# IML-DKFZ/values

Measured on AMD Instinct MI355X. Metric: uncertainty-volumes/sec (64^3, T=10 MC-dropout), higher is better.
Workload: dtype f32; 1 GPU; C2: 64^3 1-channel volumes, UNet3D(initial_filter_size=8, 2 classes), T=10 MC-dropout passes + fused softmax/entropy/MI/variance/argmax reduction; dropout=hash bit generator, new seed every step, weights=torch default init, seed 123

## Files before the change

include/values_amd.h:

```cpp
#ifndef VALUES_AMD_H
#define VALUES_AMD_H

#include <stddef.h>
#include <stdint.h>

#ifdef __cplusplus
extern "C" {
#endif

typedef void* vx_stream_t;

enum {
  VX_OK = 0,
  VX_E_NULL = -1,
  VX_E_SHAPE = -2,
  VX_E_DTYPE = -3,
  VX_E_WORKSPACE = -4,
  VX_E_ALIGN = -5
};

enum { VX_F32 = 0, VX_F64 = 1 };
enum { VX_ACT_NONE = 0, VX_ACT_LRELU = 1 , VX_ACT_RELU = 2 };
enum { VX_DROP_NONE = 0, VX_DROP_HASH = 1, VX_DROP_MASK = 2 };

// ... 30 lines not shown
                  uint8_t* argmax, uint8_t* sample_argmax, vx_stream_t stream);

typedef struct vx_unc_outputs {
  float* mean_prob; float* pred_entropy; float* exp_entropy; float* mutual_info;
  float* variance;
  uint8_t* argmax; uint8_t* sample_argmax;
  const float* in_count; const float* out_count;
} vx_unc_outputs;
int vx_unc_reduce_ex(const void* x, int dtype, int from_logits, int B, int T, int C, int64_t nvox,
                     const vx_unc_outputs* outputs, vx_stream_t stream);

int vx_unc_stats_accumulate(const float* logits, int B, int T, int C, int64_t nvox, float* stats, vx_stream_t stream);
int vx_unc_stats_finalize(const float* stats, int B, int T_total, int C, int64_t nvox, float* mean_prob,
                          float* pred_entropy, float* exp_entropy, float* mutual_info, uint8_t* argmax,
                          vx_stream_t stream);

int vx_softmax_planar(const float* logits, int64_t R, int C, int64_t nvox, float* out, vx_stream_t stream);

int vx_one_minus_msr(const void* x, int dtype, int C, int64_t nvox, void* out, vx_stream_t stream);

#define VX_MSR_MAX_ITEMS 65536
#define VX_MSR_MAX_PLANES (1 << 22)
typedef struct vx_msr_item {
  void* out;
  int64_t n;
  int32_t first_plane;
  int32_t C;
  int32_t dtype;
  int32_t reserved;
} vx_msr_item;
int64_t vx_one_minus_msr_batched_workspace_bytes(int n_items, int n_planes);
int vx_one_minus_msr_batched(const vx_msr_item* items , int n_items,
                             const void* const* planes , int n_planes, void* workspace,
                             int64_t ws_bytes, vx_stream_t stream);

int64_t vx_conv3d_k3_packed_floats(int Cin, int Cout);
int vx_pack_conv3d_k3(const float* w_torch, float* w_packed, int Cin, int Cout, vx_stream_t stream);
int64_t vx_convT_k2s2_packed_floats(int Cin, int Cout);
int vx_pack_convT_k2s2(const float* w_torch, float* w_packed, int Cin, int Cout, vx_stream_t stream);

typedef struct vx_conv3d_args {
  const float* in;
  const float* w_packed;
  const float* bias;
  float* out;
  int32_t in_pitch, out_pitch, out_coff;
  int32_t N, D, H, W, Cin, Cout;
  int32_t act;
  int32_t drop_mode;
  uint32_t drop_seed, drop_layer;
  const uint8_t* drop_mask;
  float* stats_partial;
  int32_t in_xblk;
  int32_t w_family;
  float* head_out;
  const float* head_w;
  const float* head_b;
  const int32_t* head_dst;
  const int32_t* head_flip;
  int32_t head_C;
  const float* in_mean; const float* in_rstd;
  int32_t in_drop_mode; uint32_t in_drop_seed, in_drop_layer;
  int32_t in_repeat;
  int32_t out_xblk, out_half;
  uint32_t* range_flag;
  const uint32_t* seed_dev;
  const float* up_in;
  const float* up_w;
  const float* up_b;
  int32_t up_pitch;
  float* pool_out;
  uint32_t* pool_flags;
  int32_t in_split;
  int32_t out_f16, in_f16;
  int32_t out_split, up_split;
  const float* up_fused;
  const uint32_t* in_pool_flags;
  const float* acc_in;
  int32_t acc_pitch;
  int32_t out_planar, in_planar;
  int32_t products;
} vx_conv3d_args;
int64_t vx_conv3d_upfused_packed_floats(void);
int vx_pack_conv3d_upfused(const float* w1_torch, const float* b1, const float* up_w_torch, const float* up_b, float* packed,
                           vx_stream_t stream);
int vx_conv3d_k3_prologue_ok(int D, int H, int W, int Cin, int Cout);
int vx_conv3d_k3_upfuse_ok(int D, int H, int W, int Cin, int Cout);
int64_t vx_convT_zc16_packed_floats(void);
int64_t vx_conv3d_upfused_zc16_packed_floats(void);
int vx_pack_conv3d_upfused_zc16(const float* w1_torch, const float* up_w_torch, const float* up_b, float* packed, vx_stream_t stream);
int vx_pack_convT_zc16(const float* w_torch , float* packed, vx_stream_t stream);
int vx_conv3d_k3_skip_prologue_ok(int D, int H, int W, int Cin, int Cout, int xblk);
int vx_conv3d_k3_acc_ok(int D, int H, int W, int Cin, int Cout);
int vx_conv3d_k3_planar_ok(int D, int H, int W, int Cin, int Cout);
int vx_conv3d_k3_poolfuse_ok(int D, int H, int W, int Cin, int Cout);
int vx_conv3d_k3_presplit_ok(int D, int H, int W, int Cin, int Cout);
int vx_conv3d_k3_poolfin_ok(int Cin, int Cout);
int vx_prenorm_split(float* x, const float* mean, const float* rstd, int N, int64_t nvox, float scale, vx_stream_t stream);
int vx_pool_finish(const float* pool_raw, const uint32_t* pool_flags, const float* mean, const float* rstd, float* out,
                   int out_pitch, int N, int64_t voxels_per_sample, int drop_scale2, vx_stream_t stream);
int vx_pool_finish_z(const float* pool_raw, const uint32_t* pool_flags, const float* mean, const float* rstd, float* out,
                     int out_pitch, int N, int Dp, int64_t plane_voxels, int drop_scale2, vx_stream_t stream);
int vx_conv3d_k3_pool_layout(int D, int H, int W, int Cin, int Cout);
int vx_conv3d_k3_tiles(int D, int H, int W);
int vx_conv3d_k3_tiles_for(int D, int H, int W, int Cout);
int vx_conv3d_k3(const vx_conv3d_args* a, vx_stream_t stream);
int vx_conv3d_k3_head_fusable(int Cin, int Cout);
int vx_conv3d_k3_route(const vx_conv3d_args* a, char* kernel_name, int cap);

int vx_conv3d_k3_c1_tiles(int D, int H, int W);
int vx_conv3d_k3_c1(const float* in, const float* w_torch , const float* bias, float* out,
                    int out_pitch, int N, int D, int H, int W, int Cout, int repeat, const int32_t* src,
                    const int32_t* flip, float* stats_partial, vx_stream_t stream);

int vx_pack_input_cl8(const float* in, float* out, int N, int Cin, int D, int H, int W, int repeat, const int32_t* src,
                      const int32_t* flip, vx_stream_t stream);

int vx_instnorm_finalize(const float* stats_partial, int N, int ntiles, int C, int64_t nvox, float eps,
                         float* mean, float* rstd, vx_stream_t stream);

typedef struct vx_norm_args {
  const float* x; int32_t x_pitch;
  const float* mean; const float* rstd;
  float* out; int32_t out_pitch, out_coff;
  float* pool_out; int32_t pool_pitch;
  int32_t N, D, H, W, C;
  int32_t act, drop_mode; uint32_t drop_seed, drop_layer; const uint8_t* drop_mask;
  int32_t out_xblk, out_half;
  int32_t x_xblk, x_half;
  const uint32_t* seed_dev;
  uint32_t* range_flag;
} vx_norm_args;
int vx_norm_act_drop_pool(const vx_norm_args* a, vx_stream_t stream);
typedef struct vx_stat_src {
  const float* stats_partial; int32_t tiles; float eps; int64_t count;
  float* mean_out; float* rstd_out;
} vx_stat_src;
int vx_norm_act_drop_pool_stats(const vx_norm_args* a, const vx_stat_src* st, vx_stream_t stream);
int vx_prenorm_split_stats(float* x, const vx_stat_src* st, int N, int64_t nvox, float scale, vx_stream_t stream);
int vx_zero(void* p, int64_t bytes, vx_stream_t stream);
int vx_pool_finish_z_stats(const float* pool_raw, const uint32_t* pool_flags, const vx_stat_src* st, float* out, int out_pitch,
                           int N, int Dp, int64_t plane_voxels, int drop_scale2, vx_stream_t stream);
int vx_norm_act_drop_pool_bcast(const vx_norm_args* a, int x_repeat, vx_stream_t stream);

typedef struct vx_convT_args {
  const float* in; int32_t in_pitch;
  const float* w_packed; const float* bias;
  float* out; int32_t out_pitch, out_coff;
  int32_t N, D, H, W, Cin, Cout;
  int32_t act, drop_mode; uint32_t drop_seed, drop_layer; const uint8_t* drop_mask;
  int32_t out_xblk, out_half;
  uint32_t* range_flag;
  const uint32_t* seed_dev;
} vx_convT_args;
int vx_convT_k2s2(const vx_convT_args* a, vx_stream_t stream);

int vx_conv1x1_ncdhw(const float* in, int in_pitch, const float* w, const float* bias, float* out, int N, int D,
                     int H, int W, int F, int C, const int32_t* dst, const int32_t* flip, vx_stream_t stream);

typedef struct vx_unet3d_weights {
  const float* conv_w[18];
  const float* conv_b[18];
  const float* up_w[4];
  const float* up_b[4];
  const float* final_w;
  const float* final_b;
  int32_t F;
  int32_t num_classes;
  int32_t conv_family[18];
  int32_t in_channels;
  int32_t no_instancenorm;
  const float* up_fused;
  const float* split_w[2];
  int32_t split_family;
  const float* up3_zc16;
  const float* up3_fused;
} vx_unet3d_weights;

typedef struct vx_unet3d_run {
  const float* x;
  int32_t N, D, H, W;
  int32_t repeat;
  const int32_t* src;
  const int32_t* flip;
  const int32_t* dst;
  int32_t drop_mode;
  uint32_t seed;
  const uint8_t* masks[17];
  float* logits;
  void* workspace; size_t workspace_bytes;
  uint32_t* range_flag;
  const uint32_t* seed_dev;
} vx_unet3d_run;

size_t vx_unet3d_workspace_bytes(int N, int D, int H, int W, int F);
int vx_unet3d_forward(const vx_unet3d_weights* w, const vx_unet3d_run* r, vx_stream_t stream);
int vx_unet3d_forward_profiled(const vx_unet3d_weights* w, const vx_unet3d_run* r, vx_stream_t stream,
                               int max_launches, float* ms, const char** labels, int* n_launches);

typedef struct vx_conv2d_args {
  const float* in; int32_t in_pitch;
  const float* w_packed; const float* bias;
  float* out; int32_t out_pitch, out_coff;
  int32_t N, H, W, Cin, Cout, KS, S;
  float* stats_partial;
  int32_t w_family;
  const float* in_scale; const float* in_shift;
  int32_t in_cpitch, in_group_images, in_relu;
  const float* out_scale; const float* out_shift;
  const float* out_add; int32_t out_add_pitch;
  int32_t out_act;
} vx_conv2d_args;
int64_t vx_conv2d_packed_floats(int Cin, int Cout, int KS);
int vx_pack_conv2d(const float* w_torch , float* w_packed, int Cin, int Cout, int KS, vx_stream_t stream);
int vx_conv2d_tiles(int H, int W, int KS, int S);
int vx_conv2d(const vx_conv2d_args* a, vx_stream_t stream);
typedef struct vx_conv2d_route_info {
  int32_t nchunks;
  int32_t w_all;
  int32_t lds_bytes;
  int32_t grid_x, grid_y;
} vx_conv2d_route_info;
int vx_conv2d_route(const vx_conv2d_args* a, char* kernel_name, int cap, vx_conv2d_route_info* info);

int vx_bn_finalize(const float* stats_partial, int ntiles, int C, int64_t count, float eps, const float* gamma,
                   const float* beta, float* scale, float* shift, vx_stream_t stream);
int vx_bn_finalize_groups(const float* stats_partial, int ntiles_per_group, int G, int C, int cpitch, int64_t count_per_group,
                          float eps, const float* gamma, const float* beta, float* scale, float* shift, vx_stream_t stream);

typedef struct vx_bn_affine_item {
  const float* gamma; const float* beta; const float* running_mean; const float* running_var;
  float* scale; float* shift;
  int32_t C, cpitch;
} vx_bn_affine_item;
int vx_bn_running_affine(const vx_bn_affine_item* items, int n_items, float eps, vx_stream_t stream);

typedef struct vx_affine_args {
  const float* x; int32_t x_pitch;
  const float* scale; const float* shift;
  const float* add; int32_t add_pitch;
  float* out; int32_t out_pitch, out_coff;
  int32_t N, H, W, C, OH, OW;
  int32_t act;
  int32_t drop_mode; uint32_t drop_seed, drop_layer; const uint8_t* drop_mask;
  int32_t group_images;
} vx_affine_args;
int vx_affine_gather(const vx_affine_args* a, vx_stream_t stream);

typedef struct vx_fuse_term {
  const float* x; int32_t x_pitch, H, W;
  const float* scale; const float* shift;
} vx_fuse_term;
typedef struct vx_fuse_args {
  vx_fuse_term term[4]; int32_t nterms;
  float* out; int32_t out_pitch;
  int32_t N, OH, OW, C;
  int32_t act;
  int32_t group_images;
} vx_fuse_args;
int vx_fuse_sum(const vx_fuse_args* a, vx_stream_t stream);

int vx_bilinear_nchw(const float* x, int x_pitch, int N, int H, int W, int C, int OH, int OW, float* out,
                     const int32_t* dst, const int32_t* flip, vx_stream_t stream);
int vx_bilinear_softmax_nchw(const float* x, int x_pitch, int N, int H, int W, int C, int OH, int OW, float* out,
                             const int32_t* dst, const int32_t* flip, vx_stream_t stream);

int vx_softmax_accumulate(const float* logits, int B, int T, int C, int P0, int P1, int P2, const int32_t* crop,
                          float* sum, float* count, int X, int Y, int Z, int overlap, vx_stream_t stream);

int vx_aleatoric_sample(const float* mu_s, const float* eps, uint32_t seed, int N, int T, int C, int64_t nvox,
                        float* out, float* sigma, vx_stream_t stream);

int vx_softmax_variance(const float* x, int from_logits, int B, int T, int C, int64_t nvox, float* out, vx_stream_t stream);

int vx_ssn_sample(const float* head, const float* eps_w, const float* eps_d, uint32_t seed, int N, int S, int C, int R,
                  int64_t nvox, float epsilon, float* out, vx_stream_t stream);

int vx_tta_views_2d(const void* src, int src_u8, const float* noise0, const float* noise1, const float* mean, const float* std,
                    float max_pixel_value, int B, int H, int W, int G, const int32_t* view_code, float* out, vx_stream_t stream);

int vx_tta_views_2d_gen(const void* src, int src_u8, const float* noise0, const float* noise1, const float* mean,
                        const float* std, float max_pixel_value, int B, int H, int W, int G, const int32_t* view_code,
                        uint32_t seed, const uint32_t* seed_dev, int64_t image0, const float* var_limit, float* sigma_out,
                        float* out, vx_stream_t stream);

int vx_noise_view_3d(const float* x, float* out, int V, int64_t per, uint32_t seed, const uint32_t* seed_dev, int64_t index0,
                     float var_lo, float var_hi, int sigma_law, float* sigma_out, vx_stream_t stream);

int vx_colorize_u8(const uint8_t* labels, const uint8_t* ignore, int64_t n, const uint8_t* lut, int unlabeled, uint8_t* rgb,
                   vx_stream_t stream);

#define VX_SELECT_MAX_ITEMS 65536
enum { VX_COUNT_B1 = 0, VX_COUNT_B2 = 1, VX_COUNT_B4 = 2, VX_COUNT_B8 = 3, VX_COUNT_F32 = 4, VX_COUNT_F64 = 5 };
enum { VX_SELECT_OK = 0, VX_SELECT_NAN = 1 };
typedef struct vx_count_item {
  const void* ptr;
  int64_t n;
  int32_t kind;
  int32_t reserved;
} vx_count_item;
typedef struct vx_select_item {
  const void* ptr;
  int64_t n;
  int32_t dtype;
  int32_t reserved;
} vx_select_item;
int64_t vx_count_nonzero_batched_workspace_bytes(int n_items);
int vx_count_nonzero_batched(const vx_count_item* items , int n_items, uint64_t* counts ,
                             void* workspace, int64_t ws_bytes, vx_stream_t stream);
int64_t vx_select_segments_workspace_bytes(int n_items);
int vx_select_segments(const vx_select_item* items , int n_items, int64_t k, float* out ,
                       int32_t* status , void* workspace, int64_t ws_bytes, vx_stream_t stream);

enum { VX_PREP_U8 = 0, VX_PREP_I8 = 1, VX_PREP_U16 = 2, VX_PREP_I16 = 3, VX_PREP_U32 = 4, VX_PREP_I32 = 5, VX_PREP_F32 = 6, VX_PREP_F64 = 7 };
enum { VX_PREP_ZSCORE = 0, VX_PREP_COPY = 1 };
#define VX_PREP_OWN (-1)
typedef struct vx_prep_item {
  const void* ptr;
  int64_t n;
  int32_t kind;
  int32_t reserved;
} vx_prep_item;
typedef struct vx_prep_pad_item {
  const void* src;
  void* dst;
  int32_t dims[3];
  int32_t out_dims[3];
  int32_t pad_below[3];
  int32_t kind;
// ... 269 lines not shown
```

values_amd/_lib.py:

```python
from __future__ import annotations

import ctypes as C
import os

_HERE = os.path.dirname(os.path.abspath(__file__))
LIB_PATH = os.environ.get("VX_LIB_PATH") or os.path.join(_HERE, "libvalues_amd.so")

VX_F32, VX_F64 = 0, 1
VX_ACT_NONE, VX_ACT_LRELU, VX_ACT_RELU = 0, 1, 2
VX_DROP_NONE, VX_DROP_HASH, VX_DROP_MASK = 0, 1, 2

_p = C.c_void_p
_i = C.c_int
_i32 = C.c_int32
_u32 = C.c_uint32
_i64 = C.c_int64


class ConvArgs(C.Structure):
    _fields_ = [("in_", _p), ("w_packed", _p), ("bias", _p), ("out", _p),
                ("in_pitch", _i32), ("out_pitch", _i32), ("out_coff", _i32),
                ("N", _i32), ("D", _i32), ("H", _i32), ("W", _i32), ("Cin", _i32), ("Cout", _i32),
                ("act", _i32), ("drop_mode", _i32), ("drop_seed", _u32), ("drop_layer", _u32),
                ("drop_mask", _p), ("stats_partial", _p), ("in_xblk", _i32), ("w_family", _i32),
                ("head_out", _p), ("head_w", _p), ("head_b", _p), ("head_dst", _p), ("head_flip", _p),
                ("head_C", _i32),
                ("in_mean", _p), ("in_rstd", _p), ("in_drop_mode", _i32), ("in_drop_seed", _u32), ("in_drop_layer", _u32),
                ("in_repeat", _i32), ("out_xblk", _i32), ("out_half", _i32), ("range_flag", _p), ("seed_dev", _p),
                ("up_in", _p), ("up_w", _p), ("up_b", _p), ("up_pitch", _i32), ("pool_out", _p), ("pool_flags", _p),
                ("in_split", _i32), ("out_f16", _i32), ("in_f16", _i32),
                ("out_split", _i32), ("up_split", _i32), ("up_fused", _p), ("in_pool_flags", _p),
                ("acc_in", _p), ("acc_pitch", _i32), ("out_planar", _i32), ("in_planar", _i32), ("products", _i32)]


class NormArgs(C.Structure):
    _fields_ = [("x", _p), ("x_pitch", _i32), ("mean", _p), ("rstd", _p),
                ("out", _p), ("out_pitch", _i32), ("out_coff", _i32),
                ("pool_out", _p), ("pool_pitch", _i32),
                ("N", _i32), ("D", _i32), ("H", _i32), ("W", _i32), ("C", _i32),
                ("act", _i32), ("drop_mode", _i32), ("drop_seed", _u32), ("drop_layer", _u32), ("drop_mask", _p),
                ("out_xblk", _i32), ("out_half", _i32), ("x_xblk", _i32), ("x_half", _i32), ("seed_dev", _p),
                ("range_flag", _p)]


class StatSrc(C.Structure):
    _fields_ = [("stats_partial", _p), ("tiles", _i32), ("eps", C.c_float), ("count", _i64), ("mean_out", _p), ("rstd_out", _p)]


class ConvTArgs(C.Structure):
    _fields_ = [("in_", _p), ("in_pitch", _i32), ("w_packed", _p), ("bias", _p),
                ("out", _p), ("out_pitch", _i32), ("out_coff", _i32),
                ("N", _i32), ("D", _i32), ("H", _i32), ("W", _i32), ("Cin", _i32), ("Cout", _i32),
                ("act", _i32), ("drop_mode", _i32), ("drop_seed", _u32), ("drop_layer", _u32), ("drop_mask", _p),
                ("out_xblk", _i32), ("out_half", _i32), ("range_flag", _p), ("seed_dev", _p)]


class Conv2dArgs(C.Structure):
    _fields_ = [("in_", _p), ("in_pitch", _i32), ("w_packed", _p), ("bias", _p),
                ("out", _p), ("out_pitch", _i32), ("out_coff", _i32),
                ("N", _i32), ("H", _i32), ("W", _i32), ("Cin", _i32), ("Cout", _i32), ("KS", _i32), ("S", _i32),
                ("stats_partial", _p), ("w_family", _i32),
                ("in_scale", _p), ("in_shift", _p), ("in_cpitch", _i32), ("in_group_images", _i32), ("in_relu", _i32),
                ("out_scale", _p), ("out_shift", _p), ("out_add", _p), ("out_add_pitch", _i32), ("out_act", _i32)]


class Conv2dRouteInfo(C.Structure):
    _fields_ = [("nchunks", _i32), ("w_all", _i32), ("lds_bytes", _i32), ("grid_x", _i32), ("grid_y", _i32)]


class BnAffineItem(C.Structure):
    _fields_ = [("gamma", _p), ("beta", _p), ("running_mean", _p), ("running_var", _p), ("scale", _p), ("shift", _p),
                ("C", _i32), ("cpitch", _i32)]


class AffineArgs(C.Structure):
    _fields_ = [("x", _p), ("x_pitch", _i32), ("scale", _p), ("shift", _p), ("add", _p), ("add_pitch", _i32),
                ("out", _p), ("out_pitch", _i32), ("out_coff", _i32),
                ("N", _i32), ("H", _i32), ("W", _i32), ("C", _i32), ("OH", _i32), ("OW", _i32),
                ("act", _i32), ("drop_mode", _i32), ("drop_seed", _u32), ("drop_layer", _u32), ("drop_mask", _p),
                ("group_images", _i32)]


class FuseTerm(C.Structure):
    _fields_ = [("x", _p), ("x_pitch", _i32), ("H", _i32), ("W", _i32), ("scale", _p), ("shift", _p)]


class FuseArgs(C.Structure):
    _fields_ = [("term", FuseTerm * 4), ("nterms", _i32), ("out", _p), ("out_pitch", _i32),
                ("N", _i32), ("OH", _i32), ("OW", _i32), ("C", _i32), ("act", _i32), ("group_images", _i32)]


class Config(C.Structure):
    _fields_ = [(n, _i32) for n in (
        "conv_fp32", "s16_no_prenorm", "s16_no_xp8", "s16_skip_raw", "no_head_fusion", "s16_no_upfuse", "s16_no_poolfuse",
        "storage16", "s16_generic", "s16_no_zc16", "s16_no_halves", "s16_no_deep", "s16_no_l1dma", "c2s_no_wide", "c2s_no_oct")]
    RETIRED = ("s16_no_upcompose", "s16_no_upsplit", "s16_no_poolfin", "s16_no_presplit", "s16_no_dbplain")


def _retired_field(name):
    def put(self, v):
        if v:
            raise ValueError(f"vx_config.{name} was retired in 0.7.0: the default data flow is the only one")
    return property(lambda self: 0, put)


for _n in Config.RETIRED:
    setattr(Config, _n, _retired_field(_n))


class UncOutputs(C.Structure):
    _fields_ = [("mean_prob", _p), ("pred_entropy", _p), ("exp_entropy", _p), ("mutual_info", _p), ("variance", _p),
                ("argmax", _p), ("sample_argmax", _p), ("in_count", _p), ("out_count", _p)]


class UNet3DWeights(C.Structure):
    _fields_ = [("conv_w", _p * 18), ("conv_b", _p * 18), ("up_w", _p * 4), ("up_b", _p * 4),
                ("final_w", _p), ("final_b", _p), ("F", _i32), ("num_classes", _i32), ("conv_family", _i32 * 18),
                ("in_channels", _i32), ("no_instancenorm", _i32), ("up_fused", _p), ("split_w", _p * 2), ("split_family", _i32), ("up3_zc16", _p), ("up3_fused", _p)]


class UNet3DRun(C.Structure):
    _fields_ = [("x", _p), ("N", _i32), ("D", _i32), ("H", _i32), ("W", _i32), ("repeat", _i32),
                ("src", _p), ("flip", _p), ("dst", _p), ("drop_mode", _i32), ("seed", _u32),
                ("masks", _p * 17), ("logits", _p), ("workspace", _p), ("workspace_bytes", C.c_size_t),
                ("range_flag", _p), ("seed_dev", _p)]


VX_NIFTI_COPY, VX_NIFTI_PROB, VX_NIFTI_MEAN_PROB, VX_NIFTI_ARGMAX, VX_NIFTI_ARGMAX_MEAN = 0, 1, 2, 3, 4


class NiftiItem(C.Structure):
    _fields_ = [("src", _p), ("count", _p), ("dst_off", _i64), ("kind", _i32), ("src_dtype", _i32), ("esize", _i32),
                ("T", _i32), ("C", _i32), ("t", _i32), ("c", _i32), ("X", _i32), ("Y", _i32), ("Z", _i32),
                ("header", C.c_uint8 * 352)]


class GzItem(C.Structure):
    _fields_ = [("src", _p), ("n", _i64), ("dst_off", _i64), ("stride_hint", _i32 * 3), ("pad", _i32)]


class PngItem(C.Structure):
    _fields_ = [("labels", _p), ("ignore", _p), ("H", _i32), ("W", _i32)]


class PngRgbItem(C.Structure):
    _fields_ = [("rgb", _p), ("H", _i32), ("W", _i32)]


class InflateItem(C.Structure):
    _fields_ = [("src", _p), ("src_n", _i64), ("dst_off", _i64), ("dst_cap", _i64), ("format", _i32), ("pad", _i32)]


VX_INFLATE_GZIP, VX_INFLATE_ZLIB, VX_INFLATE_RAW = 0, 1, 2
INFLATE_STATUS = ("ok", "truncated", "bad header", "bad block type", "invalid code lengths", "bad symbol",
                  "distance beyond the output start", "output capacity reached", "checksum mismatch", "ISIZE mismatch",
                  "trailing bytes", "stored block length mismatch", "preset dictionary")
VX_INFLATE_CAPACITY = 7


class NiftiDecItem(C.Structure):
    _fields_ = [("src", _p), ("src_n", _i64), ("vox_offset", _i64), ("dst", _p), ("dst_n", _i64), ("ndim", _i32),
                ("dims", _i32 * 7), ("code", _i32), ("big_endian", _i32), ("out_dtype", _i32), ("pad", _i32),
                ("slope", C.c_double), ("inter", C.c_double)]


class PngUnfilterItem(C.Structure):
    _fields_ = [("src", _p), ("src_n", _i64), ("dst", _p), ("H", _i32), ("W", _i32), ("bpp", _i32), ("pad", _i32)]


VX_PNG_OK, VX_PNG_BAD_FILTER, VX_PNG_BAD_SIZE = 0, 1, 2
PNG_STATUS = ("ok", "filter byte above 4", "stream size is not H (1 + W bpp)")


class TiffLzwItem(C.Structure):
    _fields_ = [("src", _p), ("src_n", _i64), ("dst_off", _i64), ("dst_cap", _i64)]


class TiffUnpredictItem(C.Structure):
    _fields_ = [("src", _p), ("dst", _p), ("rows", _i32), ("W", _i32), ("predictor", _i32), ("pad", _i32)]


VX_LZW_OK, VX_LZW_TRUNCATED, VX_LZW_BAD_CODE = 0, 1, 2
LZW_STATUS = ("ok", "truncated", "bad code")
VX_LZW_NO_ROOM = 3


VX_AGG_IMAGE, VX_AGG_THRESHOLD, VX_AGG_PATCH = 0, 1, 2
VX_AGG_MAX_SPECS, VX_AGG_MAX_ITEMS = 8, 4096


class AggItem(C.Structure):
    _fields_ = [("map", _p), ("dtype", _i32), ("D", _i32), ("H", _i32), ("W", _i32)]


class AggSpec(C.Structure):
    _fields_ = [("kind", _i32), ("pd", _i32), ("ph", _i32), ("pw", _i32), ("thr", C.c_double)]


VX_EM_MAX_ITEMS = 4096


class EmItem(C.Structure):
    _fields_ = [("unc", _p), ("ref", _p), ("pred", _p), ("nvox", _i64), ("dtype", _i32), ("R", _i32)]


class NccItem(C.Structure):
    _fields_ = [("gt", _p), ("pred", _p), ("n_gt", _i64), ("n_pred", _i64), ("gt_dtype", _i32), ("pred_dtype", _i32),
                ("gt_R", _i32), ("reserved", _i32)]


VX_SELECT_MAX_ITEMS = 65536
VX_COUNT_B1, VX_COUNT_B2, VX_COUNT_B4, VX_COUNT_B8, VX_COUNT_F32, VX_COUNT_F64 = range(6)
VX_SELECT_OK, VX_SELECT_NAN = 0, 1


class CountItem(C.Structure):
    _fields_ = [("ptr", _p), ("n", _i64), ("kind", _i32), ("reserved", _i32)]


class SelectItem(C.Structure):
    _fields_ = [("ptr", _p), ("n", _i64), ("dtype", _i32), ("reserved", _i32)]


VX_PREP_U8, VX_PREP_I8, VX_PREP_U16, VX_PREP_I16, VX_PREP_U32, VX_PREP_I32, VX_PREP_F32, VX_PREP_F64 = range(8)
VX_PREP_ZSCORE, VX_PREP_COPY = 0, 1
VX_PREP_OWN = -1


class PrepItem(C.Structure):
    _fields_ = [("ptr", _p), ("n", _i64), ("kind", _i32), ("reserved", _i32)]


class PrepPadItem(C.Structure):
    _fields_ = [("src", _p), ("dst", _p), ("dims", _i32 * 3), ("out_dims", _i32 * 3), ("pad_below", _i32 * 3),
                ("kind", _i32), ("out_dtype", _i32), ("mode", _i32), ("stats_row", _i32), ("reserved", _i32)]


VX_P2D_IMAGE, VX_P2D_LABEL_IDS, VX_P2D_LABEL_COLOR = 0, 1, 2


class P2dItem(C.Structure):
    _fields_ = [("src", _p), ("palette", _p), ("H", _i32), ("W", _i32), ("bpp", _i32), ("y0", _i32), ("x0", _i32),
                ("crop_h", _i32), ("crop_w", _i32), ("factor", _i32), ("mode", _i32), ("reserved", _i32), ("out_rgb", _p),
                ("out_ids", _p)]


class P2dTables(C.Structure):
    _fields_ = [("id2trainid", _p), ("trainid2color", _p), ("color2trainid", _p), ("n_color", _i32), ("default_id", _i32)]


VX_MSR_MAX_ITEMS, VX_MSR_MAX_PLANES = 65536, 1 << 22


class MsrItem(C.Structure):
    _fields_ = [("out", _p), ("n", _i64), ("first_plane", _i32), ("C", _i32), ("dtype", _i32), ("reserved", _i32)]


SIGNATURES = {
    "vx_version": (_i, []),
    "vx_last_error_string": (C.c_char_p, []),
    "vx_last_kernel_name": (C.c_char_p, []),
    "vx_drop_hash_mask": (_i, [_u32, _u32, _i, _i64, _p, _p]),
    "vx_get_config": (_i, [C.POINTER(Config)]),
    "vx_set_config": (_i, [C.POINTER(Config)]),
    "vx_conv3d_k3_family": (_i, [_i, _i]),
    "vx_conv2d_family": (_i, [_i, _i, _i]),
    "vx_unc_reduce": (_i, [_p, _i, _i, _i, _i, _i, _i64, _p, _p, _p, _p, _p, _p, _p]),
    "vx_unc_reduce_ex": (_i, [_p, _i, _i, _i, _i, _i, _i64, C.POINTER(UncOutputs), _p]),
    "vx_unc_stats_accumulate": (_i, [_p, _i, _i, _i, _i64, _p, _p]),
    "vx_unc_stats_finalize": (_i, [_p, _i, _i, _i, _i64, _p, _p, _p, _p, _p, _p]),
    "vx_softmax_planar": (_i, [_p, _i64, _i, _i64, _p, _p]),
    "vx_one_minus_msr": (_i, [_p, _i, _i, _i64, _p, _p]),
    "vx_one_minus_msr_batched_workspace_bytes": (_i64, [_i, _i]),
    "vx_one_minus_msr_batched": (_i, [C.POINTER(MsrItem), _i, C.POINTER(_p), _i, _p, _i64, _p]),
    "vx_conv3d_k3_packed_floats": (_i64, [_i, _i]),
    "vx_pack_conv3d_k3": (_i, [_p, _p, _i, _i, _p]),
    "vx_convT_k2s2_packed_floats": (_i64, [_i, _i]),
    "vx_pack_convT_k2s2": (_i, [_p, _p, _i, _i, _p]),
    "vx_conv3d_k3_tiles": (_i, [_i, _i, _i]),
    "vx_conv3d_k3_tiles_for": (_i, [_i, _i, _i, _i]),
    "vx_conv3d_k3_head_fusable": (_i, [_i, _i]),
    "vx_conv3d_k3_route": (_i, [C.POINTER(ConvArgs), C.c_char_p, _i]),
    "vx_conv3d_k3_prologue_ok": (_i, [_i, _i, _i, _i, _i]),
    "vx_conv3d_k3_upfuse_ok": (_i, [_i, _i, _i, _i, _i]),
    "vx_conv3d_k3_poolfuse_ok": (_i, [_i, _i, _i, _i, _i]),
    "vx_conv3d_k3_presplit_ok": (_i, [_i, _i, _i, _i, _i]),
    "vx_conv3d_k3_poolfin_ok": (_i, [_i, _i]),
    "vx_conv3d_upfused_packed_floats": (_i64, []),
    "vx_pack_conv3d_upfused": (_i, [_p, _p, _p, _p, _p, _p]),
    "vx_pack_conv3d_upfused_zc16": (_i, [_p, _p, _p, _p, _p]),
    "vx_conv3d_upfused_zc16_packed_floats": (_i64, []),
    "vx_pool_finish": (_i, [_p, _p, _p, _p, _p, _i, _i, _i64, _i, _p]),
    "vx_pool_finish_z": (_i, [_p, _p, _p, _p, _p, _i, _i, _i, _i64, _i, _p]),
    "vx_conv3d_k3_pool_layout": (_i, [_i, _i, _i, _i, _i]),
    "vx_conv3d_k3_skip_prologue_ok": (_i, [_i, _i, _i, _i, _i, _i]),
    "vx_conv3d_k3_acc_ok": (_i, [_i, _i, _i, _i, _i]),
    "vx_conv3d_k3_planar_ok": (_i, [_i, _i, _i, _i, _i]),
    "vx_convT_zc16_packed_floats": (_i64, []),
    "vx_pack_convT_zc16": (_i, [_p, _p, _p]),
    "vx_prenorm_split": (_i, [_p, _p, _p, _i, _i64, C.c_float, _p]),
    "vx_zero": (_i, [_p, _i64, _p]),
    "vx_conv3d_k3": (_i, [C.POINTER(ConvArgs), _p]),
    "vx_conv3d_k3_c1_tiles": (_i, [_i, _i, _i]),
    "vx_conv3d_k3_c1": (_i, [_p, _p, _p, _p, _i, _i, _i, _i, _i, _i, _i, _p, _p, _p, _p]),
    "vx_pack_input_cl8": (_i, [_p, _p, _i, _i, _i, _i, _i, _i, _p, _p, _p]),
    "vx_instnorm_finalize": (_i, [_p, _i, _i, _i, _i64, C.c_float, _p, _p, _p]),
    "vx_norm_act_drop_pool": (_i, [C.POINTER(NormArgs), _p]),
    "vx_norm_act_drop_pool_bcast": (_i, [C.POINTER(NormArgs), _i, _p]),
    "vx_norm_act_drop_pool_stats": (_i, [C.POINTER(NormArgs), C.POINTER(StatSrc), _p]),
    "vx_prenorm_split_stats": (_i, [_p, C.POINTER(StatSrc), _i, _i64, C.c_float, _p]),
    "vx_pool_finish_z_stats": (_i, [_p, _p, C.POINTER(StatSrc), _p, _i, _i, _i, _i64, _i, _p]),
    "vx_convT_k2s2": (_i, [C.POINTER(ConvTArgs), _p]),
    "vx_conv1x1_ncdhw": (_i, [_p, _i, _p, _p, _p, _i, _i, _i, _i, _i, _i, _p, _p, _p]),
    "vx_unet3d_workspace_bytes": (C.c_size_t, [_i, _i, _i, _i, _i]),
    "vx_unet3d_forward": (_i, [C.POINTER(UNet3DWeights), C.POINTER(UNet3DRun), _p]),
    "vx_unet3d_forward_profiled": (_i, [C.POINTER(UNet3DWeights), C.POINTER(UNet3DRun), _p, _i, C.POINTER(C.c_float),
                                        C.POINTER(C.c_char_p), C.POINTER(_i)]),
    "vx_softmax_accumulate": (_i, [_p, _i, _i, _i, _i, _i, _i, _p, _p, _p, _i, _i, _i, _i, _p]),
    "vx_aleatoric_sample": (_i, [_p, _p, _u32, _i, _i, _i, _i64, _p, _p, _p]),
    "vx_colorize_u8": (_i, [_p, _p, _i64, _p, _i, _p, _p]),
    "vx_fuse_sum": (_i, [C.POINTER(FuseArgs), _p]),
    "vx_tta_views_2d": (_i, [_p, _i, _p, _p, C.POINTER(C.c_float), C.POINTER(C.c_float), C.c_float, _i, _i, _i, _i,
                             C.POINTER(C.c_int32), _p, _p]),
    "vx_tta_views_2d_gen": (_i, [_p, _i, _p, _p, C.POINTER(C.c_float), C.POINTER(C.c_float), C.c_float, _i, _i, _i, _i,
                                 C.POINTER(C.c_int32), _u32, _p, _i64, C.POINTER(C.c_float), _p, _p, _p]),
    "vx_noise_view_3d": (_i, [_p, _p, _i, _i64, _u32, _p, _i64, C.c_float, C.c_float, _i, _p, _p]),
    "vx_count_nonzero_batched_workspace_bytes": (_i64, [_i]),
    "vx_count_nonzero_batched": (_i, [C.POINTER(CountItem), _i, _p, _p, _i64, _p]),
    "vx_select_segments_workspace_bytes": (_i64, [_i]),
    "vx_select_segments": (_i, [C.POINTER(SelectItem), _i, _i64, _p, _p, _p, _i64, _p]),
    "vx_volume_stats_batched_workspace_bytes": (_i64, [C.POINTER(PrepItem), _i]),
    "vx_volume_stats_batched": (_i, [C.POINTER(PrepItem), _i, _p, _p, _i64, _p]),
    "vx_zscore_pad_batched_workspace_bytes": (_i64, [C.POINTER(PrepPadItem), _i]),
    "vx_zscore_pad_batched": (_i, [C.POINTER(PrepPadItem), _i, _p, _p, _i64, _p]),
    "vx_p2d_out_size": (_i, [_i, _i]),
    "vx_crop_resize_batched_workspace_bytes": (_i64, [C.POINTER(P2dItem), _i, C.POINTER(P2dTables)]),
    "vx_crop_resize_batched": (_i, [C.POINTER(P2dItem), _i, C.POINTER(P2dTables), _p, _p, _i64, _p]),
    "vx_toy_embed": (_i, [_p, C.POINTER(_i32), C.POINTER(_i32), C.c_double, _i, _i, _p, C.POINTER(_i32), _p]),
    "vx_gauss_blur_axis_f64": (_i, [_p, _p, C.POINTER(_i32), _i, _p, _i, _p]),
    "vx_count_ge_f64": (_i, [_p, _i64, C.c_double, _p, _p]),
    "vx_order_stats_f64_workspace_bytes": (_i64, [_i]),
    "vx_order_stats_f64_reads": (_i, [_i64, C.POINTER(_i64), _i]),
    "vx_order_stats_f64": (_i, [_p, _i64, C.POINTER(_i64), _i, _p, _p, _p, _i64, _p]),
    "vx_toy_segment": (_i, [_p, _i64, C.POINTER(C.c_double), _i, _p, _p]),
    "vx_toy_noise": (_i, [_p, _i64, _u32, _u32, C.c_double, _p]),
    "vx_voxelize_meshes": (_i, [_p, C.POINTER(_i64), _i, C.POINTER(C.c_double), C.c_double, C.POINTER(_i32), _p, _p, _p]),
    "vx_mask_agreement": (_i, [_p, _i, _i, _i64, _p, _p]),
    "vx_mask_agreement_batched": (_i, [_p, _i, _i, _i, _i64, _i, _p, _p]),
    "vx_soft_metric_workspace_bytes": (_i64, [_i, _i]),
    "vx_soft_metric_sums": (_i, [_p, _p, _i, _i, _i64, _p, _p, _p]),
    "vx_soft_metric_batched_workspace_bytes": (_i64, [_i, _i, _i, _i64]),
    "vx_soft_metric_sums_batched": (_i, [_p, _p, _i, _i, _i, _i64, _p, _p, _p]),
    "vx_ssn2d_lowres": (_i, [_p, _i, _p, _i, _p, _u32, _i, _i64, _i, _i, _i, _p, _p, _p]),
    "vx_ssn2d_add_diag": (_i, [_p, _p, _p, _u32, _i, _i, _i64, C.c_float, _p]),
    "vx_softmax_variance": (_i, [_p, _i, _i, _i, _i, _i64, _p, _p]),
    "vx_ssn_sample": (_i, [_p, _p, _p, _u32, _i, _i, _i, _i, _i64, C.c_float, _p, _p]),
    "vx_conv2d_packed_floats": (_i64, [_i, _i, _i]),
    "vx_pack_conv2d": (_i, [_p, _p, _i, _i, _i, _p]),
    "vx_conv2d_tiles": (_i, [_i, _i, _i, _i]),
    "vx_conv2d": (_i, [C.POINTER(Conv2dArgs), _p]),
    "vx_conv2d_route": (_i, [C.POINTER(Conv2dArgs), C.c_char_p, _i, C.POINTER(Conv2dRouteInfo)]),
    "vx_bn_finalize": (_i, [_p, _i, _i, _i64, C.c_float, _p, _p, _p, _p, _p]),
    "vx_bn_finalize_groups": (_i, [_p, _i, _i, _i, _i, _i64, C.c_float, _p, _p, _p, _p, _p]),
    "vx_bn_running_affine": (_i, [_p, _i, C.c_float, _p]),
    "vx_affine_gather": (_i, [C.POINTER(AffineArgs), _p]),
    "vx_bilinear_nchw": (_i, [_p, _i, _i, _i, _i, _i, _i, _i, _p, _p, _p, _p]),
    "vx_bilinear_softmax_nchw": (_i, [_p, _i, _i, _i, _i, _i, _i, _i, _p, _p, _p, _p]),
    "vx_ncc_batched_workspace_bytes": (C.c_size_t, [C.POINTER(NccItem), _i]),
    "vx_ncc_batched": (_i, [C.POINTER(NccItem), _i, _p, _p, C.c_size_t, _p]),
    "vx_rater_variance": (_i, [_p, _i, _i64, _p, _p]),
    "vx_platt_batched_workspace_bytes": (C.c_size_t, [C.POINTER(EmItem), _i]),
    "vx_platt_sums_batched": (_i, [C.POINTER(EmItem), _i, C.POINTER(C.c_double), _i, _p, _p, C.c_size_t, _p]),
    "vx_calib_batched_workspace_bytes": (C.c_size_t, [C.POINTER(EmItem), _i]),
    "vx_calib_bins_batched": (_i, [C.POINTER(EmItem), _i, C.POINTER(C.c_double), C.POINTER(C.c_double), _i, _p, _p,
                                   C.c_size_t, _p]),
    "vx_aggregate_workspace_bytes": (C.c_size_t, [C.POINTER(AggItem), _i, C.POINTER(AggSpec), _i]),
    "vx_aggregate_batched": (_i, [C.POINTER(AggItem), _i, C.POINTER(AggSpec), _i, _p, _p, C.c_size_t, _p]),
    "vx_nifti_workspace_bytes": (C.c_size_t, [_i]),
    "vx_nifti_payload_bytes": (_i64, [C.POINTER(NiftiItem)]),
    "vx_nifti_payload": (_i, [C.POINTER(NiftiItem), _i, _p, _i64, _p, C.c_size_t, _p]),
    "vx_gzip_bound": (_i64, [_i64]),
    "vx_gzip_workspace_bytes": (C.c_size_t, [C.POINTER(_i64), _i]),
    "vx_gzip_encode": (_i, [C.POINTER(GzItem), _i, _p, _i64, _p, _p, C.c_size_t, _p]),
    "vx_crc32": (_i, [_p, _i64, _p, _p]),
    "vx_png_bound": (_i64, [_i, _i]),
    "vx_png_workspace_bytes": (C.c_size_t, [C.POINTER(PngItem), _i]),
    "vx_png_encode": (_i, [C.POINTER(PngItem), _i, _p, _i, _p, _i64, _p, _p, _p, C.c_size_t, _p]),
    "vx_png_encode_rgb_workspace_bytes": (C.c_size_t, [C.POINTER(PngRgbItem), _i]),
    "vx_png_encode_rgb": (_i, [C.POINTER(PngRgbItem), _i, _p, _i64, _p, _p, _p, C.c_size_t, _p]),
    "vx_inflate_workspace_bytes": (_i64, [_i]),
    "vx_inflate": (_i, [C.POINTER(InflateItem), _i, _p, _i64, _p, _p, _p, _i64, _p]),
    "vx_nifti_decode_workspace_bytes": (_i64, [_i]),
    "vx_nifti_decode": (_i, [C.POINTER(NiftiDecItem), _i, _p, _i64, _p]),
    "vx_png_unfilter_workspace_bytes": (_i64, [_i]),
    "vx_png_unfilter": (_i, [C.POINTER(PngUnfilterItem), _i, _p, _p, _i64, _p]),
    "vx_rgb_to_trainid": (_i, [_p, _i64, _p, _i, _i, _p, _p]),
    "vx_tiff_lzw_workspace_bytes": (_i64, [_i]),
    "vx_tiff_lzw": (_i, [C.POINTER(TiffLzwItem), _i, _p, _i64, _p, _p, _p, _i64, _p]),
    "vx_tiff_unpredict_workspace_bytes": (_i64, [_i]),
    "vx_tiff_unpredict": (_i, [C.POINTER(TiffUnpredictItem), _i, _p, _p, _i64, _p]),
    "vx_tiff_predict_workspace_bytes": (_i64, [_i]),
    "vx_tiff_predict": (_i, [C.POINTER(TiffUnpredictItem), _i, _p, _p, _i64, _p]),
    "vx_tiff_lzw_bound": (_i64, [_i64]),
    "vx_tiff_lzw_encode_workspace_bytes": (_i64, [_i]),
    "vx_tiff_lzw_encode": (_i, [C.POINTER(TiffLzwItem), _i, _p, _i64, _p, _p, _p, _i64, _p]),
    "vx_tiff_lzw_pack_workspace_bytes": (_i64, [_i]),
    "vx_tiff_lzw_pack": (_i, [C.POINTER(TiffLzwItem), _i, _p, _i64, _p, _p, _i64, _p, _p, _i64, _p]),
}

_lib = None


class VxError(RuntimeError):
    pass


def load():
    global _lib
    if _lib is not None:
        return _lib
    if not os.path.exists(LIB_PATH):
        raise VxError(
            f"{LIB_PATH} is missing: build it with `python -c 'import __graft_entry__ as g; g.build()'` "
            "(or `make -C values_amd/csrc`). values_amd has no CPU fallback.")
    import torch
    lib = C.CDLL(LIB_PATH, mode=C.RTLD_GLOBAL)
    for name, (res, args) in SIGNATURES.items():
        if os.environ.get("VX_LIB_PATH") and not hasattr(lib, name):
            continue
        fn = getattr(lib, name)
        fn.restype = res
        fn.argtypes = args
    _lib = lib
    return lib


def get_config() -> "Config":
    c = Config()
    check(load().vx_get_config(C.byref(c)), "vx_get_config")
    return c


class config:

# ... 73 lines not shown
```

values_amd/csrc/conv3d_deep.hip:

```cpp
#include "s16_common.h"
#include "conv3d_internal.h"

struct DeepArgs {
  vx_conv3d_args a;
  const float* w;
  int tx, ty, tz, ts;
  int ltx, lty, ltz;
  int tiles_x, tiles_y, tiles_z;
  int npos;
  int nchunks, ncg;
  int npairs;
  unsigned m_cg, m_tx, m_ty, m_tz;
  int stat_epc;
  unsigned long long* stamps;
  int abl;
};

#define DP_STAMP VX_STAMP
#define DP_WAIT_LOADS VX_STAMP_WAIT_LOADS
#define DP_ABL VX_DIAG(ka.abl)

constexpr int DEEP_PREC_B = DEEP_NPOS * 16;
constexpr int DEEP_IMG_B = 2 * DEEP_PREC_B;

// ... 176 lines not shown
      }
#pragma unroll
      for (int it = 0; it < IN_IT; ++it) {
        if (!((ibad_always >> it) & 1u)) {
          f32x4 v = ibuf[it];
          if constexpr (PRE == 1) {
            uint32_t bits = 0xFu;
            if (hashed) bits = vx_drop_bits4(p_key, p_e0 + (voff[it] >> 2));
            if ((p_bad >> it) & 1u) bits = 0u;
#pragma unroll
            for (int j = 0; j < 4; ++j) {
              const int keep = __builtin_amdgcn_sbfe((int)bits, j, 1);
              const float scj = __int_as_float(__float_as_int(sc[j]) & keep);
              const float tt = vx_mul1(vx_sub1(v[j], p_mean[j]), scj);
              v[j] = vx_max1(tt, vx_mul1(tt, 0.01f));
            }
          }
          f16x4 hi, lo;
          vx_split4_s(v, hi, lo);
          if (!(DP_ABL & 16)) {
            *reinterpret_cast<f16x4*>(img + ldst[it]) = hi;
            *reinterpret_cast<f16x4*>(img + ldst[it] + DEEP_PREC_B) = lo;
          } else {
            asm volatile("" :: "v"(hi), "v"(lo));
          }
        }
      }
    };

    Cur cx = {0, 0}, cc = {0, 0}, cp = {0, 0};
    prefetch(cp); advance(cp);
    dma_w(cc, 0);
    commit(0);    advance(cc);
    asm volatile("s_waitcnt vmcnt(0)" ::: "memory");
    prefetch(cp); advance(cp);
    int j = 0;
    while (cx.ci < npair_wg) {
      __syncthreads();
      DP_STAMP(0);
      DP_WAIT_LOADS();
      DP_STAMP(3);
      dma_w(cc, (j + 1) & 1);
      if (cc.ci < npair_wg && !(DP_ABL & 4)) commit((j + 1) & 1);
      DP_STAMP(4);
      if (!(DP_ABL & 8)) prefetch(cp);
      if constexpr (IN_IT == 9) asm volatile("s_waitcnt vmcnt(9)" ::: "memory");
      else asm volatile("s_waitcnt vmcnt(7)" ::: "memory");
      DP_STAMP(5);
#ifdef VX_CONV_STAMPS
      ++st_iters;
#endif
      advance(cx); advance(cc); advance(cp);
      ++j;
    }
    if (STATS) __syncthreads();
  } else {
    int vbase[R];
    const int out_voxf = a.out_pitch;
    const size_t out_sample = (size_t)a.D * a.H * a.W * out_voxf;
    auto vox_of = [&](int v, int& cx_, int& ly, int& lz, int& smp) {
      cx_ = v & (TX - 1); v >>= ka.ltx;
      ly = v & (TY - 1); v >>= ka.lty;
      lz = v & (TZ - 1); smp = v >> ka.ltz;
    };
#pragma unroll
    for (int r = 0; r < R; ++r) {
      int cx_, ly, lz, smp;
      vox_of((wave * R + r) * 16 + m, cx_, ly, lz, smp);
      vbase[r] = (((smp * HZ + lz) * HY + ly) * HX + cx_) * 16;
    }
    int toff[NSTEP];
#pragma unroll
    for (int s = 0; s < NSTEP; ++s) {
      int tap = 4 * s + g;
      if (DP_ABL & 64) tap = 4 * s;
      if (tap > 26) tap = 26;
      toff[s] = (((tap / 9) * HY + (tap / 3) % 3) * HX + tap % 3) * 16;
    }
    const unsigned char* wlane = s_w + lane * 16;
    const bool f_lrelu = EPI == 3 ? a.act == VX_ACT_LRELU : EPI == 1;
    const bool f_relu = EPI == 3 && a.act == VX_ACT_RELU;
    const uint32_t seed_out = EPI == 1 ? vx_seed_of(a, a.drop_seed) : 0u;

    f32x4 acc[R][NT], accx[R][NT];

    auto multiply = [&](int buf) {
      const unsigned char* img = s_img + buf * DEEP_IMG_B;
      const unsigned char* wb = wlane + buf * DEEP_W_B;
      f16x8 wh[NT], wl[NT], bh[2][R], bl[R];
      int vb_[R];
#pragma unroll
      for (int r = 0; r < R; ++r) { vb_[r] = vbase[r]; asm volatile("" : "+v"(vb_[r])); }
      auto ldA = [&](int s, int nt) {
        wh[nt] = *reinterpret_cast<const f16x8*>(wb + ((s * NT + nt) * 2) * 1024);
        wl[nt] = *reinterpret_cast<const f16x8*>(wb + ((s * NT + nt) * 2 + 1) * 1024);
      };
      auto ldBh = [&](int s, int r) { bh[s & 1][r] = *reinterpret_cast<const f16x8*>(img + vb_[r] + toff[s]); };
      auto ldBl = [&](int s, int r) { bl[r] = *reinterpret_cast<const f16x8*>(img + vb_[r] + toff[s] + DEEP_PREC_B); };
#pragma unroll
      for (int nt = 0; nt < NT; ++nt) ldA(0, nt);
#pragma unroll
      for (int r = 0; r < R; ++r) { ldBh(0, r); ldBl(0, r); }
      __builtin_amdgcn_sched_group_barrier(0x100, 2 * NT + 2 * R, 0);
#pragma unroll
      for (int s = 0; s < NSTEP; ++s) {
        const bool more = s + 1 < NSTEP;
        const int set = s & 1;
#pragma unroll
        for (int nt = 0; nt < NT; ++nt) {
#pragma unroll
          for (int r = 0; r < R; ++r) {
            acc[r][nt] = __builtin_amdgcn_mfma_f32_16x16x32_f16(wh[nt], bh[set][r], acc[r][nt], 0, 0, 0);
            accx[r][nt] = __builtin_amdgcn_mfma_f32_16x16x32_f16(wh[nt], bl[r], accx[r][nt], 0, 0, 0);
            if (more && nt == 0) ldBh(s + 1, r);
            if (more && nt == NT - 1) ldBl(s + 1, r);
          }
#pragma unroll
          for (int r = 0; r < R; ++r) accx[r][nt] = __builtin_amdgcn_mfma_f32_16x16x32_f16(wl[nt], bh[set][r], accx[r][nt], 0, 0, 0);
          if (more) ldA(s + 1, nt);
        }
#ifndef DEEP_NO_PIPE
#pragma unroll
        for (int nt = 0; nt < NT; ++nt) {
#pragma unroll
          for (int r = 0; r < R; ++r) {
            __builtin_amdgcn_sched_group_barrier(0x008, 2, 0);
            if (more) __builtin_amdgcn_sched_group_barrier(0x100, 1, 0);
          }
          __builtin_amdgcn_sched_group_barrier(0x008, R, 0);
          if (more) __builtin_amdgcn_sched_group_barrier(0x100, 2, 0);
        }
#endif
      }
    };

    auto epilogue = [&](int ci) {
      float* red = s_red + (ci & 1) * (NW * 32 * 2);
      int n0, tzi, tyi, txi, cg;
      pair_of(ci, n0, tzi, tyi, txi, cg);
      const auto kp = kernarg();
      const unsigned vox0 = (unsigned)(((tzi * TZ) * a.H + tyi * TY) * a.W + txi * TX);
      const unsigned osoff = (vox0 * (unsigned)out_voxf + (unsigned)(cg * 32)) * 4u;
      const __amdgpu_buffer_rsrc_t osrd = __builtin_amdgcn_make_buffer_rsrc(
          (void*)(reinterpret_cast<char*>(kp->a.out) + (size_t)n0 * out_sample * 4), 0, VX_NUMREC, 0x00020000);
      float ssum[NT][4], ssq[NT][4];
      if (STATS) {
#pragma unroll
        for (int nt = 0; nt < NT; ++nt)
#pragma unroll
          for (int j = 0; j < 4; ++j) { ssum[nt][j] = 0.f; ssq[nt][j] = 0.f; }
      }
      int m_ = m;
      asm volatile("" : "+v"(m_));
#pragma unroll
      for (int r = 0; r < R; ++r) {
        int cx_, ly, lz, smp;
        vox_of((wave * R + r) * 16 + m_, cx_, ly, lz, smp);
        const int ovox = (lz * a.H + ly) * a.W + cx_;
        unsigned ovoff_r = ((unsigned)smp * (unsigned)out_sample + (unsigned)ovox * (unsigned)out_voxf + (unsigned)kp->a.out_coff + 4u * g) * 4u;
        if constexpr (R == 2) {
          if (n0 + smp >= a.N) ovoff_r = VX_OOB;
        }
        uint32_t hword = 0;
        if (EPI == 1) {
          const vx_dkey key = vx_drop_key(seed_out, kp->a.drop_layer, (uint32_t)(n0 + smp));
          hword = vx_drop_word(key, (vox0 + (unsigned)ovox) * (unsigned)ka.ncg + (unsigned)cg) >> (4 * g);
        }
#pragma unroll
        for (int nt = 0; nt < NT; ++nt) {
          f32x4 v;
#pragma unroll
          for (int j = 0; j < 4; ++j) v[j] = fmaf(accx[r][nt][j], 1.0f / 2048.f, acc[r][nt][j]);
          if (STATS) {
#pragma unroll
            for (int j = 0; j < 4; ++j) { ssum[nt][j] += v[j]; ssq[nt][j] = fmaf(v[j], v[j], ssq[nt][j]); }
          }
          if (f_lrelu) {
#pragma unroll
            for (int j = 0; j < 4; ++j) v[j] = fmaxf(v[j], 0.01f * v[j]);
          } else if (f_relu) {
#pragma unroll
            for (int j = 0; j < 4; ++j) v[j] = fmaxf(v[j], 0.f);
          }
          if (EPI == 1) {
            const uint32_t bits = hword >> (16 * nt);
#pragma unroll
            for (int j = 0; j < 4; ++j) v[j] *= __uint_as_float((bits << (30 - j)) & 0x40000000u);
          }
          if (!STATS) rmax = vx_max3abs(vx_max3abs(rmax, v[0], v[1]), v[2], v[3]);
          u32x4 sv = __builtin_bit_cast(u32x4, v);
          if (EPI == 1 || EPI == 3) {
            if (a.out_split) {
              typedef unsigned u32x2 __attribute__((ext_vector_type(2)));
              f16x4 hi, lo;
              vx_split4_s(v, hi, lo);
              const u32x2 h2 = __builtin_bit_cast(u32x2, hi), l2 = __builtin_bit_cast(u32x2, lo);
              sv = (u32x4){h2[0], h2[1], l2[0], l2[1]};
            }
          }
          __builtin_amdgcn_raw_buffer_store_b128(sv, osrd, (int)ovoff_r, (int)(osoff + (unsigned)(nt * 64)), 0);
          __builtin_amdgcn_sched_barrier(0);
          asm volatile("s_nop 3" ::: "memory");
          __builtin_amdgcn_sched_barrier(0);
        }
      }
      if (STATS) {
#pragma unroll
        for (int nt = 0; nt < NT; ++nt)
#pragma unroll
          for (int j = 0; j < 4; ++j) {
            float s = ssum[nt][j], qq = ssq[nt][j];
#pragma unroll
            for (int rot = 8; rot >= 1; rot >>= 1) { s += vx_row_ror(s, rot); qq += vx_row_ror(qq, rot); }
            if (m == 0) {
              red[(wave * 32 + nt * 16 + g * 4 + j) * 2 + 0] = s;
              red[(wave * 32 + nt * 16 + g * 4 + j) * 2 + 1] = qq;
            }
          }
      }
    };

    auto flush_tile = [&](int ci) {
      const float* red = s_red + (ci & 1) * (NW * 32 * 2);
      int n0, tzi, tyi, txi, cg;
      pair_of(ci, n0, tzi, tyi, txi, cg);
      const auto kp = kernarg();
      const int epc = kp->stat_epc;
      const int tps = ka.tiles_x * ka.tiles_y * ka.tiles_z;
      const int tile = (tzi * ka.tiles_y + tyi) * ka.tiles_x + txi;
      float* dst = kp->a.stats_partial + (((size_t)n0 * tps + tile) * epc * a.Cout + cg * 32) * 2;
      if (tid < 32) {
        float s = 0.f, qq = 0.f;
#pragma unroll
        for (int w = 0; w < NW; ++w) {
          s += red[(w * 32 + tid) * 2 + 0];
          qq += red[(w * 32 + tid) * 2 + 1];
        }
        dst[tid * 2 + 0] = s;
        dst[tid * 2 + 1] = qq;
      }
      for (int e = 1; e < epc; ++e)
        if (tid < 64) dst[(size_t)e * a.Cout * 2 + tid] = 0.f;
    };

    const bool late = wave >= NW / 2;
    Cur cx = {0, 0};
    int j = 0;
    int prev_ci = -1;
    int fl_ci = -1, fl_at = 0;
    while (cx.ci < npair_wg) {
      __syncthreads();
      DP_STAMP(0);
      if (STATS && fl_ci >= 0 && j >= fl_at && !late) { flush_tile(fl_ci); fl_ci = -1; }
      if (late && prev_ci >= 0) {
        if (!(DP_ABL & 2)) epilogue(prev_ci);
        prev_ci = -1;
      }
      DP_STAMP(2);
      if (cx.c == 0) {
        int n0, tzi, tyi, txi, cg;
        pair_of(cx.ci, n0, tzi, tyi, txi, cg);
        const f32x4 zero = {0.f, 0.f, 0.f, 0.f};
#pragma unroll
        for (int nt = 0; nt < NT; ++nt) {
          const f32x4 b4 = *reinterpret_cast<const f32x4*>(s_bias + cg * 32 + nt * 16 + 4 * g);
#pragma unroll
          for (int r = 0; r < R; ++r) { acc[r][nt] = b4; accx[r][nt] = zero; }
        }
      }
      if (!(DP_ABL & 1)) multiply(j & 1);
      DP_STAMP(1);
      if (cx.c == NCH - 1) {
        if (late) prev_ci = cx.ci;
        else if (!(DP_ABL & 2)) epilogue(cx.ci);
        if (STATS) { fl_ci = cx.ci; fl_at = j + 2; }
      }
      DP_STAMP(2);
#ifdef VX_CONV_STAMPS
      ++st_iters;
#endif
      advance(cx);
      ++j;
    }
    if (late && prev_ci >= 0) epilogue(prev_ci);
    if (STATS) {
      __syncthreads();
      if (fl_ci >= 0 && !late) flush_tile(fl_ci);
    }
  }
  if (!STATS && a.range_flag) {
    float mx = rmax;
#pragma unroll
    for (int off = 32; off >= 1; off >>= 1) mx = fmaxf(mx, __shfl_xor(mx, off, 64));
    if (lane == 0 && !(mx < 32768.f)) atomicMax(a.range_flag, __float_as_uint(mx));
  }
#ifdef VX_CONV_STAMPS
  if (ka.stamps && lane == 0) {
    unsigned long long* d = ka.stamps + ((size_t)blockIdx.x * 16 + wave) * 8;
    for (int i = 0; i < 6; ++i) d[i] = st_sum[i];
    d[6] = st_iters;
  }
#endif
}

__global__ void pack_conv3d_deep_kernel(const float* __restrict__ w, _Float16* __restrict__ out, int Cin, int64_t total) {
  const int nch = Cin / 8;
  for (int64_t i = (int64_t)blockIdx.x * blockDim.x + threadIdx.x; i < total; i += (int64_t)gridDim.x * blockDim.x) {
    const int j = (int)(i & 7), lane = (int)((i >> 3) & 63), hl = (int)((i >> 9) & 1), nt = (int)((i >> 10) & 1);
    const int64_t sb = i >> 11;
    const int step = (int)(sb % 7);
    const int64_t blk = sb / 7;
    const int chunk = (int)(blk % nch), cg = (int)(blk / nch);
    const int row = cg * 32 + nt * 16 + (lane & 15), tap = 4 * step + (lane >> 4);
    const float v = tap > 26 ? 0.f : w[((size_t)row * Cin + 8 * chunk + j) * 27 + tap];
    const float c = fminf(fmaxf(v, -65504.f), 65504.f);
    const _Float16 h = (_Float16)c;
    out[i] = hl == 0 ? h : (_Float16)((v - (float)h) * 2048.f);
  }
}

int vx_pack_conv3d_deep(const float* w_torch, float* w_packed, int Cin, int Cout, hipStream_t s) {
  const int64_t total = conv3d_deep_packed_floats(Cin, Cout) * 2;
  if (total <= 0) return VX_OK;
  int blocks = (int)((total + 255) / 256);
  if (blocks > 4096) blocks = 4096;
  hipLaunchKernelGGL(pack_conv3d_deep_kernel, dim3(blocks), dim3(256), 0, s, w_torch, reinterpret_cast<_Float16*>(w_packed), Cin, total);
  VX_CHECK_LAUNCH("vx_pack_conv3d_k3(deep)");
  return VX_OK;
// ... 44 lines not shown
```

values_amd/csrc/conv3d_k3.hip:

```cpp
#include <string.h>

#include "conv3d_internal.h"

extern "C" int vx_conv3d_k3_route(const vx_conv3d_args* ap, char* kernel_name, int cap) {
  if (!ap) VX_FAIL(VX_E_NULL, "vx_conv3d_k3: null args");
  Conv3dRoute r;
  const int rc = conv3d_route(*ap, vx_cfg(), &r);
  if (rc != VX_OK) VX_FAIL(rc, "%s", r.err);
  if (kernel_name && cap > 0) conv3d_route_name(r, kernel_name, cap);
  return VX_OK;
}

extern "C" int vx_conv3d_k3(const vx_conv3d_args* ap, vx_stream_t stream) {
  if (!ap) VX_FAIL(VX_E_NULL, "vx_conv3d_k3: null args");
  const vx_conv3d_args& a = *ap;
  Conv3dRoute r;
  const int rc = conv3d_route(a, vx_cfg(), &r);
  if (rc != VX_OK) VX_FAIL(rc, "%s", r.err);
  hipStream_t s = (hipStream_t)stream;
  switch (r.kernel) {
    case CONV3D_C8: return vx_conv3d_c8_launch(r, a, s);
    case CONV3D_XP8W: return vx_conv3d_xp8w_launch(r, a, s);
    case CONV3D_ZC16: return vx_conv3d_zc16_launch(r, a, a.w_packed + r.w_off, s);
    case CONV3D_DEEP: return vx_conv3d_deep_launch(r, a, a.w_packed + r.w_off, s);
    case CONV3D_S16: return vx_conv3d_s16_launch(r, a, s);
    default: return vx_conv3d_mfma_launch(r, a, s);
  }
}

extern "C" int vx_conv3d_k3_family(int Cin, int Cout) { return conv3d_family(Cin, Cout, vx_cfg()); }
extern "C" int64_t vx_conv3d_k3_packed_floats(int Cin, int Cout) { return conv3d_packed_floats(Cin, Cout, vx_cfg()); }

extern "C" int vx_pack_conv3d_k3(const float* w_torch, float* w_packed, int Cin, int Cout, vx_stream_t stream) {
  if (!w_torch || !w_packed) VX_FAIL(VX_E_NULL, "vx_pack_conv3d_k3: null pointer");
  const int64_t total = vx_conv3d_k3_packed_floats(Cin, Cout);
  if (total < 0) VX_FAIL(VX_E_SHAPE, "vx_pack_conv3d_k3: Cin=%d Cout=%d must be positive multiples of 8", Cin, Cout);
  const ConvCfg c = conv_config(Cin, Cout, vx_cfg());
  hipStream_t s = (hipStream_t)stream;
  if (c.C8) return vx_pack_conv3d_k3_c8(w_torch, w_packed, Cin, s);
  if (!c.S16) return vx_pack_conv3d_k3_mfma(w_torch, w_packed, Cin, Cout, total, s);
  const int rc = vx_pack_conv3d_k3_s16(w_torch, w_packed, Cin, Cout, s);
  if (rc != VX_OK) return rc;
  float* w_block = w_packed + conv3d_s16_packed_floats(Cin, Cout);
  if (conv3d_deep_packs(Cin, Cout)) return vx_pack_conv3d_deep(w_torch, w_block, Cin, Cout, s);
  return vx_pack_conv3d_zc16(w_torch, w_block, Cin, Cout, s);
}

extern "C" int vx_conv3d_k3_tiles(int D, int H, int W) { return conv3d_tiles_max(D, H, W); }
extern "C" int vx_conv3d_k3_tiles_for(int D, int H, int W, int Cout) { return conv3d_tiles_for(D, H, W, Cout, vx_cfg()); }
extern "C" int vx_conv3d_k3_head_fusable(int Cin, int Cout) { return conv3d_head_fusable(Cin, Cout, vx_cfg()); }
extern "C" int vx_conv3d_k3_prologue_ok(int D, int H, int W, int Cin, int Cout) { return conv3d_prologue_ok(D, H, W, Cin, Cout, vx_cfg()); }
extern "C" int vx_conv3d_k3_skip_prologue_ok(int D, int H, int W, int Cin, int Cout, int xblk) {
  return conv3d_skip_prologue_ok(D, H, W, Cin, Cout, xblk, vx_cfg());
}
extern "C" int vx_conv3d_k3_acc_ok(int D, int H, int W, int Cin, int Cout) { return conv3d_zc16_16to16(D, H, W, Cin, Cout, vx_cfg()) ? 1 : 0; }
extern "C" int vx_conv3d_k3_planar_ok(int D, int H, int W, int Cin, int Cout) { return conv3d_zc16_16to16(D, H, W, Cin, Cout, vx_cfg()) ? 1 : 0; }
extern "C" int vx_conv3d_k3_upfuse_ok(int D, int H, int W, int Cin, int Cout) { return conv3d_upfuse_ok(D, H, W, Cin, Cout, vx_cfg()); }
extern "C" int vx_conv3d_k3_pool_layout(int D, int H, int W, int Cin, int Cout) { return conv3d_pool_layout(D, H, W, Cin, Cout, vx_cfg()); }
extern "C" int vx_conv3d_k3_poolfuse_ok(int D, int H, int W, int Cin, int Cout) { return conv3d_pool_layout(D, H, W, Cin, Cout, vx_cfg()) != 0 ? 1 : 0; }
extern "C" int vx_conv3d_k3_presplit_ok(int D, int H, int W, int Cin, int Cout) { return conv3d_presplit_ok(D, H, W, Cin, Cout, vx_cfg()); }
extern "C" int vx_conv3d_k3_poolfin_ok(int Cin, int Cout) { return conv3d_poolfin_ok(Cin, Cout, vx_cfg()); }
```

values_amd/csrc/conv3d_route.h:

```cpp
#pragma once
#include <stdint.h>
#include <stdio.h>

#include "../../include/values_amd.h"

constexpr int DEEP_NPOS = 1080;
constexpr int DEEP_NPOS_R2 = 896;
constexpr int DEEP_W_B = 7 * 2 * 2 * 1024;
constexpr int DEEP_MAXC = 512;
constexpr int DEEP_MAXDIM = 32;
constexpr int S16_HEAD_MAXC = 4;

enum Conv3dKernel { CONV3D_MFMA = 0, CONV3D_C8, CONV3D_S16, CONV3D_XP8W, CONV3D_ZC16, CONV3D_DEEP, CONV3D_NKERNELS };

#define MFMA_TILES(X, CB, NT, XP) X(CB, NT, 16, 4, 4, 8, XP) X(CB, NT, 8, 8, 4, 8, XP) X(CB, NT, 4, 4, 4, 4, XP)
#define MFMA_INSTANCES(X) MFMA_TILES(X, 8, 1, 1) MFMA_TILES(X, 16, 1, 0) MFMA_TILES(X, 16, 2, 0) MFMA_TILES(X, 8, 1, 0) MFMA_TILES(X, 8, 2, 0)
#define C8_INSTANCES(X) X(1, 32, 4, 4) X(2, 32, 4, 4) X(1, 16, 8, 4) X(2, 16, 8, 4) X(1, 8, 4, 4) X(2, 8, 4, 4)
#define S16_SMALL(X, CB, NT, XP)                                                                                       \
  X(CB, NT, 16, 4, 4, 8, XP, 0, 0) X(CB, NT, 16, 4, 4, 8, XP, 0, 1) X(CB, NT, 16, 4, 4, 8, XP, 0, 3)                     \
  X(CB, NT, 8, 8, 4, 8, XP, 0, 0) X(CB, NT, 8, 8, 4, 8, XP, 0, 1) X(CB, NT, 8, 8, 4, 8, XP, 0, 3) X(CB, NT, 4, 4, 4, 4, XP, 0, 3)
#define S16_LARGE(X, CB, XP) X(CB, 1, 16, 8, 4, 8, XP, 0, 0) X(CB, 1, 16, 8, 4, 8, XP, 0, 1) X(CB, 1, 16, 8, 4, 8, XP, 0, 3)
#define S16_DB_PLAIN(X, CB, NT) X(CB, NT, 16, 4, 4, 8, 0, 2, 0) X(CB, NT, 16, 4, 4, 8, 0, 2, 1) X(CB, NT, 16, 4, 4, 8, 0, 2, 3)
#define S16_DB_XP(X)                                                                                                   \
  X(8, 1, 16, 8, 4, 8, 1, 2, 0) X(8, 1, 16, 8, 4, 8, 1, 2, 1) X(8, 1, 16, 8, 4, 8, 1, 2, 2) X(8, 1, 16, 8, 4, 8, 1, 2, 3) \
// ... 226 lines not shown
}
static inline bool conv3d_tile_prologue(int Cin, int Cout, const vx_config& cfg) {
  return conv_config(Cin, Cout, cfg).S16 && conv3d_s16_prologue_ok(Cin, Cout);
}
static inline bool conv3d_tile_xblk_prologue(int Cin, int Cout, int xblk) {
  const int csrc = Cin / 2;
  return s16_config(Cin, Cout).CB == 16 && csrc % 16 == 0 && conv3d_pow2((int64_t)xblk * csrc);
}
static inline int conv3d_prologue_ok(int D, int H, int W, int Cin, int Cout, const vx_config& cfg) {
  if (!conv3d_channels_ok(Cin, Cout)) return 0;
  return conv3d_xp8_applies(D, H, W, Cin, Cout, cfg) || conv3d_tile_prologue(Cin, Cout, cfg) ? 1 : 0;
}
static inline int conv3d_skip_prologue_ok(int D, int H, int W, int Cin, int Cout, int xblk, const vx_config& cfg) {
  if (Cin <= 0 || Cout <= 0 || Cin % 16 || Cout % 8 || (xblk != 1 && xblk != 2 && xblk != 4)) return 0;
  if (Cin == 16 && conv3d_xp8_applies(D, H, W, Cin, Cout, cfg)) return 1;
  return conv3d_tile_prologue(Cin, Cout, cfg) && conv3d_tile_xblk_prologue(Cin, Cout, xblk) ? 1 : 0;
}
static inline int conv3d_upfuse_ok(int D, int H, int W, int Cin, int Cout, const vx_config& cfg) {
  if (cfg.s16_no_upfuse) return 0;
  if (Cin == 16 && conv3d_xp8_applies(D, H, W, Cin, Cout, cfg)) return 1;
  return conv3d_zc16_16to16(D, H, W, Cin, Cout, cfg) ? 2 : 0;
}
static inline int conv3d_pool_layout(int D, int H, int W, int Cin, int Cout, const vx_config& cfg) {
  if (cfg.s16_no_poolfuse) return 0;
  if (Cin == 8 && conv3d_xp8_applies(D, H, W, Cin, Cout, cfg)) return 1;
  return conv3d_zc16_16to16(D, H, W, Cin, Cout, cfg) ? 2 : 0;
}
static inline int conv3d_presplit_ok(int D, int H, int W, int Cin, int Cout, const vx_config& cfg) {
  return Cin == 8 && conv3d_xp8_applies(D, H, W, Cin, Cout, cfg) ? 1 : 0;
}
static inline int conv3d_poolfin_ok(int Cin, int Cout, const vx_config& cfg) {
  if (Cin != 8 || Cout <= 0 || Cout % 8 || Cout % 32 == 0) return 0;
  return conv3d_tile_prologue(Cin, Cout, cfg) ? 1 : 0;
}

#define ROUTE_FAIL(code, ...)                          \
  do {                                                 \
    snprintf(r->err, sizeof(r->err), __VA_ARGS__);     \
    return (code);                                     \
  } while (0)
constexpr int ROUTE_DECLINED = 1;

static inline void route_instance(Conv3dRoute* r, int kernel, int np, int a = 0, int b = 0, int c = 0, int d = 0, int e = 0, int f = 0,
                                  int g = 0, int h = 0, int i = 0) {
  const int p[9] = {a, b, c, d, e, f, g, h, i};
  r->kernel = kernel; r->np = np;
  for (int k = 0; k < 9; ++k) r->p[k] = p[k];
}
static inline void route_tiles(Conv3dRoute* r, const vx_conv3d_args& a, int txv, int ty, int tz) {
  r->tiles_x = conv3d_tiles_along(a.W, txv); r->tiles_y = conv3d_tiles_along(a.H, ty); r->tiles_z = conv3d_tiles_along(a.D, tz);
  r->mx = conv3d_magic(r->tiles_x); r->my = conv3d_magic(r->tiles_y); r->mz = conv3d_magic(r->tiles_z);
}
static inline void route_columns(Conv3dRoute* r, const vx_conv3d_args& a, int tz, int stat_tiles) {
  r->tiles_x = a.W / 32; r->tiles_y = a.H / 8; r->tiles_z = 1; r->kz = a.D / tz;
  const int cps = r->tiles_x * r->tiles_y;
  r->nitems = (int)((int64_t)a.N * cps);
  r->mcps = conv3d_magic(cps); r->mx = conv3d_magic(r->tiles_x);
  r->stat_epc = stat_tiles / cps;
}

static inline int route_xp8w(const vx_conv3d_args& a, int stat_tiles, Conv3dRoute* r) {
  const int nch = a.Cin / 8;
  route_columns(r, a, 4 / nch, stat_tiles);
  const int cps = r->tiles_x * r->tiles_y;
  r->rep = (a.in_mean && a.in_repeat > 1 && a.N % a.in_repeat == 0) ? a.in_repeat : 1;
  r->mrep = conv3d_magic(r->rep);
  if ((int64_t)a.N * cps >= (1ll << 31)) ROUTE_FAIL(VX_E_SHAPE, "vx_conv3d_k3(xp8w): too many columns");
  if (a.stats_partial && (stat_tiles % cps || a.act != VX_ACT_NONE || (a.drop_mode != VX_DROP_NONE && !a.pool_out) || a.head_out))
    ROUTE_FAIL(VX_E_SHAPE, "vx_conv3d_k3(xp8w): statistics go with a plain epilogue");
  const int pre = a.in_split ? 2 : (a.in_mean ? 1 : 0);
  if (a.in_split && (a.Cin != 8 || a.in_xblk || a.in_pitch != 8 || a.up_in || !a.stats_partial))
    ROUTE_FAIL(VX_E_SHAPE, "vx_conv3d_k3(xp8w): a pre-split input (vx_prenorm_split) goes with a dense 8-channel tensor and the "
               "statistics epilogue (contr_1_2)");
  int epi;
  if (a.stats_partial) epi = a.pool_out ? 4 : 0;
  else if (a.head_out) epi = 2;
  else if (a.drop_mode == VX_DROP_HASH) epi = 1;
  else epi = 3;
  if (epi == 2 && a.act == VX_ACT_LRELU && a.drop_mode == VX_DROP_NONE) epi = 5;
  if (epi == 2 && !(a.act == VX_ACT_LRELU && a.drop_mode == VX_DROP_HASH)) return ROUTE_DECLINED;
  if (epi == 1 && a.act != VX_ACT_LRELU) return ROUTE_DECLINED;
  const int up = a.up_in ? (a.up_fused ? 2 : 1) : 0;
  if (a.pool_out && nch != 1) ROUTE_FAIL(VX_E_SHAPE, "vx_conv3d_k3(xp8w): the pooled output goes with Cin = 8");
  if (a.out_split) ROUTE_FAIL(VX_E_SHAPE, "vx_conv3d_k3(xp8w): out_split is an epilogue of the tile kernel");
  if (a.up_split && !up) ROUTE_FAIL(VX_E_SHAPE, "vx_conv3d_k3(xp8w): up_split without up_in");
  if (a.out_f16 && (epi != 1 || a.out_xblk || a.out_coff))
    ROUTE_FAIL(VX_E_SHAPE, "vx_conv3d_k3(xp8w): fp16 output goes with the LeakyReLU + dropout epilogue and a dense output tensor");
  if (a.in_f16 && !(nch == 1 && epi == 2 && pre == 0 && !up && !a.in_xblk))
    ROUTE_FAIL(VX_E_SHAPE, "vx_conv3d_k3(xp8w): fp16 input goes with the dense 8-channel layer that carries the fused head");
  const int in16 = (a.in_f16 ? 1 : 0) | (a.products == 1 ? 2 : 0);
  route_instance(r, CONV3D_XP8W, 6, nch, epi, pre, up, nch == 2 ? 8 : 4, in16);
  if (conv3d_instance_exists(CONV3D_XP8W, r->p, 6)) return VX_OK;
  if (a.products == 1 && !a.in_f16)
    ROUTE_FAIL(VX_E_SHAPE, "vx_conv3d_k3(xp8w): products = 1 exists for the MC-dropout forward's contr_1_2, upscale2 + expand_1_1 and "
               "expand_1_2 + head (nch %d, epilogue %d, prologue %d, up %d)", nch, epi, pre, up);
  if (up) ROUTE_FAIL(VX_E_SHAPE, "vx_conv3d_k3(xp8w): no fused up-convolution for this epilogue (act=%d, drop_mode=%d, statistics=%d)",
                     a.act, a.drop_mode, a.stats_partial ? 1 : 0);
  if (a.pool_out) ROUTE_FAIL(VX_E_SHAPE, "vx_conv3d_k3(xp8w): no pooled output for this epilogue");
  return ROUTE_DECLINED;
}

static inline int route_zc16(const vx_conv3d_args& a, int stat_tiles, Conv3dRoute* r) {
  if (a.in_xblk || a.head_out || a.in_split || a.in_f16 || a.out_f16 || (a.in_repeat > 1)) return ROUTE_DECLINED;
  if ((a.in_planar || a.out_planar) && (a.drop_mode == VX_DROP_MASK || !a.out || a.in_pitch != a.Cin || a.Cout != 16))
    ROUTE_FAIL(VX_E_SHAPE, "vx_conv3d_k3(zc16): the planar pre-split hand-over needs hash or no dropout and dense 16-channel tensors");
  if (a.up_in && (a.Cin != 16 || a.in_mean || a.stats_partial || a.up_pitch < 32 || a.up_pitch % 4 || (a.up_fused && (!a.acc_in || a.out_xblk || a.out_split))))
    ROUTE_FAIL(VX_E_SHAPE, "vx_conv3d_k3(zc16): the fused up-convolution (32 coarse channels -> the conv's 16 input channels) goes with an "
               "activation epilogue, no prologue, up_pitch >= 32 (got %d), up_w packed by vx_pack_convT_zc16; composed weights "
               "(up_fused: vx_pack_conv3d_upfused_zc16) only together with partial sums (acc_in) and a dense float or planar output", a.up_pitch);
  if (a.drop_mode == VX_DROP_MASK || !a.out) return ROUTE_DECLINED;
  route_columns(r, a, 2, stat_tiles);
  const int cps = r->tiles_x * r->tiles_y;
  if ((int64_t)a.N * cps >= (1ll << 31)) ROUTE_FAIL(VX_E_SHAPE, "vx_conv3d_k3(zc16): too many columns");
  if (a.in_pitch != a.Cin) return ROUTE_DECLINED;
  if (a.stats_partial && (stat_tiles % cps || a.act != VX_ACT_NONE || (a.drop_mode != VX_DROP_NONE && !a.pool_out)))
    ROUTE_FAIL(VX_E_SHAPE, "vx_conv3d_k3(zc16): statistics go with a plain epilogue");
  if (a.pool_out && (!a.stats_partial || a.Cin != 16)) ROUTE_FAIL(VX_E_SHAPE, "vx_conv3d_k3(zc16): the pooled output goes with statistics, 16 -> 16");
  int pre = 0;
  if (a.in_pool_flags) pre = 3;
  else if (a.in_mean) pre = 1;
  if ((pre == 1 && a.Cin != 16) || (pre == 3 && a.Cin != 8)) return ROUTE_DECLINED;
  if (a.in_planar) {
    if (a.Cin != 16 || pre != 0 || a.up_in || a.acc_in || a.stats_partial || !conv3d_aligned16(a.in) ||
        (conv3d_bytes)a.D * a.H * a.W * 64 >= CONV3D_2GIB)
      ROUTE_FAIL(VX_E_SHAPE, "vx_conv3d_k3(zc16): a planar pre-split input (in_planar) goes with 16 -> 16, an activation epilogue, no "
                 "prologue / up-convolution / partial sums, a 16-byte aligned tensor, one sample below 2 GiB");
    pre = 4;
  }
  if (a.out_planar && (a.stats_partial || a.out_pitch != 16 || a.out_coff != 0 || a.out_xblk || a.out_split || a.out == a.acc_in ||
                       (conv3d_bytes)a.D * a.H * a.W * 64 >= CONV3D_2GIB))
    ROUTE_FAIL(VX_E_SHAPE, "vx_conv3d_k3(zc16): a planar pre-split output (out_planar) goes with an activation epilogue into a dense "
               "16-channel tensor that is not the partial sums' (another layout), one sample below 2 GiB");
  int epi;
  if (a.stats_partial) epi = a.pool_out ? 4 : 0;
  else if (a.drop_mode == VX_DROP_HASH) { if (a.act != VX_ACT_LRELU) return ROUTE_DECLINED; epi = 1; }
  else epi = 3;
  if (a.out_split && a.stats_partial) ROUTE_FAIL(VX_E_SHAPE, "vx_conv3d_k3(zc16): out_split goes with the activation epilogues");
  if (a.out_planar) {
    if (a.Cin != 16 || pre != 0 || (epi != 1 && epi != 3) || ((a.acc_in != nullptr) != (a.up_in != nullptr)))
      ROUTE_FAIL(VX_E_SHAPE, "vx_conv3d_k3(zc16): out_planar goes with 16 -> 16, an activation epilogue, no prologue, and either partial "
                 "sums + the fused up-convolution together or neither");
    epi = epi == 1 ? 5 : 6;
  }
  if (a.acc_in && (a.Cin != 16 || pre != 0 || a.stats_partial || a.acc_pitch < 16 || a.acc_pitch % 4 || !conv3d_aligned16(a.acc_in) ||
                   (conv3d_bytes)a.D * a.H * a.W * a.acc_pitch * 4 >= CONV3D_2GIB))
    ROUTE_FAIL(VX_E_SHAPE, "vx_conv3d_k3(zc16): partial sums (acc_in) go with 16 -> 16, no prologue, an activation epilogue, a "
               "16-byte aligned tensor of pitch >= 16 (pitch %d), one sample below 2 GiB", a.acc_pitch);
  route_instance(r, CONV3D_ZC16, 5, a.Cin, epi, pre, a.acc_in ? 1 : 0, a.up_in ? 1 : 0);
  if (conv3d_instance_exists(CONV3D_ZC16, r->p, 5)) return VX_OK;
  if (a.up_in && !a.acc_in) ROUTE_FAIL(VX_E_SHAPE, "vx_conv3d_k3(zc16): no fused up-convolution for this epilogue");
  return ROUTE_DECLINED;
}

static inline int route_deep(const vx_conv3d_args& a, int stat_tiles, Conv3dRoute* r) {
  if (a.head_out || a.in_split || a.in_f16 || a.out_f16 || (a.in_repeat > 1) || a.out_xblk || a.up_in || a.pool_out ||
      a.in_pool_flags || a.acc_in)
    return ROUTE_DECLINED;
  if (a.drop_mode == VX_DROP_MASK || !a.out) return ROUTE_DECLINED;
  DeepGeo g;
  const int R = deep_pick(a.D, a.H, a.W, &g);
  if (!R) return ROUTE_DECLINED;
  if (a.in_xblk) {
    const int csrc = a.Cin / 2;
    if (a.in_mean || csrc % 8 || a.W % a.in_xblk) return ROUTE_DECLINED;
  } else if (a.in_pitch % 4) {
    return ROUTE_DECLINED;
  }
  if (a.in_mean && (a.in_pitch != a.Cin || g.ts != 1)) return ROUTE_DECLINED;
  if (a.stats_partial && g.ts != 1) return ROUTE_DECLINED;
  r->tx = g.tx; r->ty = g.ty; r->tz = g.tz; r->ts = g.ts; r->npos = g.npos;
  r->tiles_x = g.tiles_x; r->tiles_y = g.tiles_y; r->tiles_z = g.tiles_z;
  r->nchunks = a.Cin / 8;
  r->ncg = a.Cout / 32;
  const int tps = g.tiles_x * g.tiles_y * g.tiles_z;
  const int64_t npairs = (((int64_t)a.N + g.ts - 1) / g.ts) * tps * r->ncg;
  if (npairs >= (1ll << 31)) ROUTE_FAIL(VX_E_SHAPE, "vx_conv3d_k3(deep): too many tiles");
  r->nitems = (int)npairs;
  r->m_cg = conv3d_magic(r->ncg); r->mx = conv3d_magic(g.tiles_x); r->my = conv3d_magic(g.tiles_y); r->mz = conv3d_magic(g.tiles_z);
  r->stat_epc = 0;
  if (a.stats_partial) {
    if (stat_tiles % tps) return ROUTE_DECLINED;
    if (a.act != VX_ACT_NONE || a.drop_mode != VX_DROP_NONE) ROUTE_FAIL(VX_E_SHAPE, "vx_conv3d_k3(deep): statistics go with a plain epilogue");
    r->stat_epc = stat_tiles / tps;
  }
  if ((conv3d_bytes)g.ts * a.D * a.H * a.W * a.out_pitch * 4 >= CONV3D_2GIB)
    ROUTE_FAIL(VX_E_SHAPE, "vx_conv3d_k3(deep): one tile's samples must stay below 2 GiB");
  int epi;
  if (a.stats_partial) epi = 0;
  else if (a.drop_mode == VX_DROP_HASH) { if (a.act != VX_ACT_LRELU) return ROUTE_DECLINED; epi = 1; }
  else epi = 3;
  if (a.out_split && a.stats_partial) ROUTE_FAIL(VX_E_SHAPE, "vx_conv3d_k3(deep): out_split goes with the activation epilogues");
  route_instance(r, CONV3D_DEEP, 3, R, epi, a.in_mean ? 1 : 0);
  return conv3d_instance_exists(CONV3D_DEEP, r->p, 3) ? VX_OK : ROUTE_DECLINED;
}

static inline int route_s16(const vx_conv3d_args& a, const vx_config& cfg, Conv3dRoute* r) {
  const S16Cfg c = s16_config(a.Cin, a.Cout);
  int txv, ty, tz;
  vx_conv3d_s16_tile(a.H, a.W, a.Cout, &txv, &ty, &tz);
  const int tx = c.XP ? txv / 2 : txv;
  route_tiles(r, a, txv, ty, tz);
  r->nchunks = a.Cin / c.CB;
  r->ty8 = (tx == 16 && ty == 8) ? 1 : 0;
  const bool generic = cfg.s16_generic != 0;
  int epi = 3;
  if (generic) epi = 3;
  else if (a.act == VX_ACT_NONE && a.drop_mode == VX_DROP_NONE && !a.head_out && a.out) epi = 0;
  else if (a.act == VX_ACT_LRELU && a.drop_mode == VX_DROP_HASH && !a.head_out && a.out) epi = 1;
  else if (a.act == VX_ACT_LRELU && a.drop_mode == VX_DROP_HASH && a.head_out && c.XP) epi = 2;
  int db = 0;
  if (!generic && tx == 16 && c.XP && r->ty8 && r->nchunks <= 2) db = r->nchunks == 1 ? 2 : 3;
  if (!generic && tx == 16 && !c.XP && !r->ty8 && r->nchunks == 1) db = 2;
  if (epi == 2 && db != 2) epi = 3;
  if (db == 3 && epi == 0) epi = 3;
  if (tx == 4) epi = 3;
  route_instance(r, CONV3D_S16, 9, c.CB, c.NT, tx, ty, tz, tx == 4 ? 4 : 8, c.XP, db, epi);
  if (!conv3d_instance_exists(CONV3D_S16, r->p, 9)) ROUTE_FAIL(VX_E_SHAPE, "vx_conv3d_k3(s16): no instance for this tile");
  return VX_OK;
}

static inline int conv3d_route(const vx_conv3d_args& a, const vx_config& cfg, Conv3dRoute* r) {
  r->err[0] = 0;
  r->w_off = 0;
  if (!a.in || !a.w_packed || !a.bias || (!a.out && !a.head_out)) ROUTE_FAIL(VX_E_NULL, "vx_conv3d_k3: null tensor pointer");
  const ConvCfg c = conv_config(a.Cin, a.Cout, cfg);
  if (a.head_out) {
    if (!a.head_w || !a.head_b) ROUTE_FAIL(VX_E_NULL, "vx_conv3d_k3: fused head without weights");
    if (a.head_C < 1 || a.head_C > 8) ROUTE_FAIL(VX_E_SHAPE, "vx_conv3d_k3: fused head takes 1..8 classes, got %d", a.head_C);
    if (c.S16 && a.head_C > S16_HEAD_MAXC)
      ROUTE_FAIL(VX_E_SHAPE, "vx_conv3d_k3: the split-fp16 kernel fuses heads of up to 4 classes, got %d", a.head_C);
    if (!conv3d_head_fusable(a.Cin, a.Cout, cfg))
      ROUTE_FAIL(VX_E_SHAPE, "vx_conv3d_k3: no fused head for Cin=%d Cout=%d (see vx_conv3d_k3_head_fusable)", a.Cin, a.Cout);
    if (a.stats_partial) ROUTE_FAIL(VX_E_SHAPE, "vx_conv3d_k3: fused head on a layer with InstanceNorm statistics");
  }
  if (!conv3d_channels_ok(a.Cin, a.Cout))
    ROUTE_FAIL(VX_E_SHAPE, "vx_conv3d_k3: Cin=%d Cout=%d must be positive multiples of 8", a.Cin, a.Cout);
  if (a.N <= 0 || a.D <= 0 || a.H <= 0 || a.W <= 0) ROUTE_FAIL(VX_E_SHAPE, "vx_conv3d_k3: empty tensor");
  if (a.w_family != conv3d_family(a.Cin, a.Cout, cfg))
    ROUTE_FAIL(VX_E_DTYPE, "vx_conv3d_k3: weights packed for kernel family %d, the library is configured for family %d "
               "(vx_conv3d_k3_family(%d, %d)): re-pack them", a.w_family, conv3d_family(a.Cin, a.Cout, cfg), a.Cin, a.Cout);
  if (a.out_xblk && ((a.out_xblk != 1 && a.out_xblk != 2 && a.out_xblk != 4) || a.W % a.out_xblk || (a.out_half != 0 && a.out_half != 1)))
    ROUTE_FAIL(VX_E_SHAPE, "vx_conv3d_k3: bad concat output (xblk=%d, half=%d, W=%d)", a.out_xblk, a.out_half, a.W);
  if ((a.in_mean == nullptr) != (a.in_rstd == nullptr)) ROUTE_FAIL(VX_E_NULL, "vx_conv3d_k3: in_mean / in_rstd must come together");
  if (a.products != 0 && a.products != 1 && a.products != 3)
    ROUTE_FAIL(VX_E_SHAPE, "vx_conv3d_k3: products = %d (0 / 3: the default split scheme, 1: one fp16 product)", a.products);
  const bool xp8 = c.S16 && conv3d_xp8_applies(a.D, a.H, a.W, a.Cin, a.Cout, cfg) && a.drop_mode != VX_DROP_MASK;
  if (a.products == 1 && !(xp8 && a.in_drop_mode != VX_DROP_MASK))
    ROUTE_FAIL(VX_E_SHAPE, "vx_conv3d_k3: products = 1 is taken by the full-resolution z-column kernel only (got %dx%dx%d, %d -> %d)",
               a.D, a.H, a.W, a.Cin, a.Cout);
  if ((a.in_planar || a.out_planar) && !conv3d_zc16_16to16(a.D, a.H, a.W, a.Cin, a.Cout, cfg))
    ROUTE_FAIL(VX_E_SHAPE, "vx_conv3d_k3: the planar pre-split hand-over (in_planar / out_planar) is taken where vx_conv3d_k3_planar_ok "
               "(got %dx%dx%d, %d -> %d)", a.D, a.H, a.W, a.Cin, a.Cout);
  if (a.up_in) {
    if (!a.up_w || !a.up_b) ROUTE_FAIL(VX_E_NULL, "vx_conv3d_k3: fused up-convolution without weights");
    if (!conv3d_upfuse_ok(a.D, a.H, a.W, a.Cin, a.Cout, cfg) || a.drop_mode == VX_DROP_MASK || a.stats_partial || a.head_out)
      ROUTE_FAIL(VX_E_SHAPE, "vx_conv3d_k3: no fused up-convolution for this layer (see vx_conv3d_k3_upfuse_ok; hash or no "
                 "dropout, no statistics, no head): %dx%dx%d, %d -> %d", a.D, a.H, a.W, a.Cin, a.Cout);
    if (a.up_pitch < 16 || a.up_pitch % 4 || !conv3d_aligned16(a.up_in) || !conv3d_aligned16(a.up_b))
      ROUTE_FAIL(VX_E_ALIGN, "vx_conv3d_k3: up_in pitch %d (>= 16, multiple of 4 floats) / alignment", a.up_pitch);
    if ((conv3d_bytes)(a.D / 2 + 2) * (a.H / 2) * (a.W / 2) * a.up_pitch * 4 >= CONV3D_2GIB)
      ROUTE_FAIL(VX_E_SHAPE, "vx_conv3d_k3: one coarse sample must stay below 2 GiB");
    if (a.up_fused && !conv3d_aligned16(a.up_fused)) ROUTE_FAIL(VX_E_ALIGN, "vx_conv3d_k3: up_fused alignment");
  } else if (a.up_fused) {
    ROUTE_FAIL(VX_E_SHAPE, "vx_conv3d_k3: up_fused (composed up-convolution weights) without up_in");
  }
  if (a.pool_out) {
    if (!a.pool_flags || !a.stats_partial) ROUTE_FAIL(VX_E_NULL, "vx_conv3d_k3: pool_out goes with pool_flags and stats_partial");
    if (!conv3d_pool_layout(a.D, a.H, a.W, a.Cin, a.Cout, cfg) || a.drop_mode == VX_DROP_MASK || a.act != VX_ACT_NONE || a.head_out)
      ROUTE_FAIL(VX_E_SHAPE, "vx_conv3d_k3: no pooled output for this layer (see vx_conv3d_k3_poolfuse_ok; hash or no dropout, "
                 "no activation): %dx%dx%d, %d -> %d", a.D, a.H, a.W, a.Cin, a.Cout);
    if (!conv3d_aligned16(a.pool_out)) ROUTE_FAIL(VX_E_ALIGN, "vx_conv3d_k3: pool_out alignment");
  }
  if (a.in_drop_mode != VX_DROP_NONE && a.in_drop_mode != VX_DROP_HASH) ROUTE_FAIL(VX_E_DTYPE, "vx_conv3d_k3: in_drop_mode %d", a.in_drop_mode);
  if (a.in_pool_flags) {
    if (!a.in_mean) ROUTE_FAIL(VX_E_NULL, "vx_conv3d_k3: in_pool_flags goes with in_mean / in_rstd");
    if (!conv3d_poolfin_ok(a.Cin, a.Cout, cfg) || a.in_xblk || a.in_pitch != 8 || a.in_split || a.up_in || a.in_repeat > 1)
      ROUTE_FAIL(VX_E_SHAPE, "vx_conv3d_k3: pool-finish on load takes a dense 8-channel tensor of window maxima (see "
                 "vx_conv3d_k3_poolfin_ok): %d -> %d, pitch %d", a.Cin, a.Cout, a.in_pitch);
    if (a.act != VX_ACT_NONE || a.drop_mode != VX_DROP_NONE || a.head_out || !a.out)
      ROUTE_FAIL(VX_E_SHAPE, "vx_conv3d_k3: pool-finish on load goes with the plain epilogue (no activation, no dropout, no head): "
                 "act=%d drop_mode=%d", a.act, a.drop_mode);
  }
  if (a.out && !a.out_xblk && (a.out_pitch < (int64_t)a.out_coff + a.Cout || a.out_pitch % 4 || a.out_coff % 4))
    ROUTE_FAIL(VX_E_ALIGN, "vx_conv3d_k3: output pitch/offset must be multiples of 4 floats and cover the channels");
  if (a.in_xblk) {
    if (a.in_xblk != 1 && a.in_xblk != 2 && a.in_xblk != 4) ROUTE_FAIL(VX_E_SHAPE, "vx_conv3d_k3: in_xblk must be 0, 1, 2 or 4");
    if (a.W % a.in_xblk) ROUTE_FAIL(VX_E_SHAPE, "vx_conv3d_k3: W=%d not a multiple of in_xblk=%d", a.W, a.in_xblk);
    if (a.Cin % 16) ROUTE_FAIL(VX_E_SHAPE, "vx_conv3d_k3: concat input needs Cin %% 16 == 0 (two halves of Cin/2)");
  } else if (a.in_pitch < (a.up_in ? a.Cin / 2 : a.Cin) || a.in_pitch % 4) {
    ROUTE_FAIL(VX_E_ALIGN, "vx_conv3d_k3: input pitch must be a multiple of 4 floats and cover the channels");
  }
  if (!conv3d_aligned16(a.in) || !conv3d_aligned16(a.out) || !conv3d_aligned16(a.w_packed) || !conv3d_aligned16(a.bias))
    ROUTE_FAIL(VX_E_ALIGN, "vx_conv3d_k3: pointers must be 16-byte aligned");
  if (a.act < 0 || a.act > 2 || a.drop_mode < 0 || a.drop_mode > 2) ROUTE_FAIL(VX_E_DTYPE, "vx_conv3d_k3: bad act/drop enum");
  if (a.drop_mode == VX_DROP_MASK && !a.drop_mask) ROUTE_FAIL(VX_E_NULL, "vx_conv3d_k3: VX_DROP_MASK without mask");
  const int64_t inrow = a.in_xblk ? (int64_t)a.Cin : (int64_t)a.in_pitch;
  if ((conv3d_bytes)a.D * a.H * a.W * a.out_pitch * 4 >= CONV3D_2GIB || ((conv3d_bytes)a.D + 2) * a.H * a.W * inrow * 4 >= CONV3D_2GIB)
    ROUTE_FAIL(VX_E_SHAPE, "vx_conv3d_k3: one sample must stay below 2 GiB (32-bit buffer offsets)");

  const TileCfg t = tile_config(a.W, c.XP);
  if (c.C8 && !a.in_mean && !a.out_xblk) {
    route_tiles(r, a, t.TXV, t.TY, t.TZ);
    route_instance(r, CONV3D_C8, 4, a.Cin / 8, t.TXV, t.TY, t.TZ);
    return VX_OK;
  }
  const int stat_tiles = conv3d_tiles_for(a.D, a.H, a.W, a.Cout, cfg);
  r->w_off = conv3d_s16_packed_floats(a.Cin, a.Cout);
  if (xp8) {
    r->w_off = 0;
    const int rc = route_xp8w(a, stat_tiles, r);
    if (rc != ROUTE_DECLINED) return rc;
// ... 40 lines not shown
```

values_amd/csrc/convtranspose.hip:

```cpp
#include "common.h"
#include <stdlib.h>

constexpr int CT_CO = 8;

__device__ __forceinline__ float* convT_out_ptr(const vx_convT_args& a, size_t orow, int ox, int OW, int c) {
  if (a.out_xblk) {
    const int xb = a.out_xblk;
    return a.out + orow * (2 * (size_t)OW * a.Cout) + ((ox / xb) * 2 + a.out_half) * xb * a.Cout + (ox % xb) * a.Cout + c;
  }
  return a.out + (orow * OW + ox) * a.out_pitch + a.out_coff + c;
}

__global__ __launch_bounds__(256) void convT_k2s2_kernel(vx_convT_args a, int64_t nvox_in) {
  const int ngroups = a.Cout / CT_CO;
  const int cgp = blockIdx.y % ngroups;
  const int dzy = blockIdx.y / ngroups;
  const int dz = dzy >> 1, dy = dzy & 1;
  const int co0 = cgp * CT_CO;
  const float* __restrict__ wp = a.w_packed + (size_t)dzy * a.Cin * 2 * a.Cout;
  const int OD = a.D * 2, OH = a.H * 2, OW = a.W * 2;

  for (int64_t i = blockIdx.x * (int64_t)blockDim.x + threadIdx.x; i < nvox_in; i += (int64_t)gridDim.x * blockDim.x) {
    int64_t r = i;
    const int x = r % a.W; r /= a.W;
// ... 68 lines not shown
    const int n = (int)r;
    const int ox = p / C4, x = ox >> 1;
    const float* __restrict__ xin = a.in + (((size_t)(n * a.D + z) * a.H + y) * a.W + x) * a.in_pitch;
    f32x4 xv[CIN / 4];
#pragma unroll
    for (int k = 0; k < CIN / 4; ++k) xv[k] = *reinterpret_cast<const f32x4*>(xin + 4 * k);
    f32x4 acc = b4;
#pragma unroll
    for (int ci = 0; ci < CIN; ++ci) {
      const float xs = xv[ci >> 2][ci & 3];
#pragma unroll
      for (int j = 0; j < 4; ++j) acc[j] = fmaf(wreg[ci][j], xs, acc[j]);
    }
    const int oz = 2 * z + dz, oy = 2 * y + dy;
    const size_t ovox = ((size_t)(n * OD + oz) * OH + oy) * OW + ox;
    if (a.act == VX_ACT_RELU) {
#pragma unroll
      for (int j = 0; j < 4; ++j) acc[j] = fmaxf(acc[j], 0.f);
    } else if (a.act == VX_ACT_LRELU) {
#pragma unroll
      for (int j = 0; j < 4; ++j) acc[j] = fmaxf(acc[j], 0.01f * acc[j]);
    }
    if (a.drop_mode == VX_DROP_HASH) {
      const uint32_t e = (uint32_t)(((oz * OH + oy) * OW + ox) * a.Cout + cq * 4);
      const uint32_t bits = vx_drop_bits4(vx_drop_key(vx_seed_of(a, a.drop_seed), a.drop_layer, (uint32_t)n), e);
#pragma unroll
      for (int j = 0; j < 4; ++j) acc[j] *= __uint_as_float((bits << (30 - j)) & 0x40000000u);
    } else if (a.drop_mode == VX_DROP_MASK) {
      const uint32_t mk = *reinterpret_cast<const uint32_t*>(a.drop_mask + ovox * a.Cout + cq * 4);
#pragma unroll
      for (int j = 0; j < 4; ++j) acc[j] = ((mk >> (8 * j)) & 0xFFu) ? 2.f * acc[j] : 0.f;
    }
    *reinterpret_cast<f32x4*>(convT_out_ptr(a, (size_t)(n * OD + oz) * OH + oy, ox, OW, cq * 4)) = acc;
  }
}

struct ConvTDecode { unsigned mW, mH, mD; };
__device__ __forceinline__ unsigned ct_div(unsigned n, unsigned m) { return m ? __umulhi(n, m) : n; }

template <int CIN, int RT, bool MASK = false>
__global__ __launch_bounds__(256) void convT_k2s2_mfma_kernel(vx_convT_args a, int ncoltiles, int nvox_in, ConvTDecode dc) {
  constexpr int Q = CIN / 16;
  const int tid = threadIdx.x, lane = tid & 63, wave = tid >> 6;
  const int m = lane & 15, g = lane >> 4;
  const int OW = a.W * 2, OH = a.H * 2, OD = a.D * 2;
  const int rt0 = blockIdx.y * RT;
  f32x4 wreg[RT][Q];
#pragma unroll
  for (int rt = 0; rt < RT; ++rt) {
    const int row = 16 * (rt0 + rt) + m;
    const int pos = row / a.Cout, co = row % a.Cout;
    const float* wp = a.w_packed + (size_t)(pos >> 1) * CIN * 2 * a.Cout + (pos & 1) * a.Cout + co;
#pragma unroll
    for (int q = 0; q < Q; ++q)
#pragma unroll
      for (int j = 0; j < 4; ++j) wreg[rt][q][j] = wp[(size_t)(16 * q + 4 * g + j) * 2 * a.Cout];
  }
  int opos[RT], oco[RT];
#pragma unroll
  for (int rt = 0; rt < RT; ++rt) {
    const int row = 16 * (rt0 + rt) + 4 * g;
    opos[rt] = row / a.Cout;
    oco[rt] = row % a.Cout;
  }
  const int xs = a.out_xblk ? __builtin_ctz((unsigned)a.out_xblk) : 0;
  const int wstride = (int)gridDim.x * 4;
  float rmax = 0.f;
  auto load_x = [&](int ct, f32x4* dst) {
    int v = ct * 16 + m;
    if (v >= nvox_in) v = nvox_in - 1;
    const float* __restrict__ xin = a.in + (size_t)v * a.in_pitch + 4 * g;
#pragma unroll
    for (int q = 0; q < Q; ++q) dst[q] = *reinterpret_cast<const f32x4*>(xin + 16 * q);
  };
  constexpr bool PF = CIN <= 32;
  constexpr bool HB = PF || RT <= 4;
  f32x4 biasr[HB ? RT : 1];
  if constexpr (HB) {
#pragma unroll
    for (int rt = 0; rt < RT; ++rt) biasr[rt] = *reinterpret_cast<const f32x4*>(a.bias + oco[rt]);
  }
  f32x4 xnext[Q];
  if constexpr (PF) {
    const int ct0 = blockIdx.x * 4 + wave;
    load_x(ct0 < ncoltiles ? ct0 : ncoltiles - 1, xnext);
  }
  const uint32_t seed0 = vx_seed_of(a, a.drop_seed);
  for (int ct = blockIdx.x * 4 + wave; ct < ncoltiles; ct += wstride) {
    const int v = ct * 16 + m;
    const bool ok = v < nvox_in;
    const int vc = ok ? v : nvox_in - 1;
    f32x4 xv[Q];
    if constexpr (PF) {
#pragma unroll
      for (int q = 0; q < Q; ++q) xv[q] = xnext[q];
      const int ctn = ct + wstride;
      load_x(ctn < ncoltiles ? ctn : ncoltiles - 1, xnext);
    } else {
      load_x(ct, xv);
    }
    unsigned r = (unsigned)vc, q;
    q = ct_div(r, dc.mW); const int x = (int)(r - q * (unsigned)a.W); r = q;
    q = ct_div(r, dc.mH); const int y = (int)(r - q * (unsigned)a.H); r = q;
    q = ct_div(r, dc.mD); const int z = (int)(r - q * (unsigned)a.D);
    const int n = (int)q;
    const vx_dkey dkey = vx_drop_key(seed0, a.drop_layer, (uint32_t)n);
#pragma unroll
    for (int rt = 0; rt < RT; ++rt) {
      f32x4 acc;
      if constexpr (HB) acc = biasr[rt];
      else acc = *reinterpret_cast<const f32x4*>(a.bias + oco[rt]);
#pragma unroll
      for (int q = 0; q < Q; ++q)
#pragma unroll
        for (int j = 0; j < 4; ++j) acc = __builtin_amdgcn_mfma_f32_16x16x4f32(wreg[rt][q][j], xv[q][j], acc, 0, 0, 0);
      const int pos = opos[rt];
      const int oz = 2 * z + (pos >> 2), oy = 2 * y + ((pos >> 1) & 1), ox = 2 * x + (pos & 1);
      const size_t orow = ((size_t)n * OD + oz) * OH + oy;
      if (a.act == VX_ACT_RELU) {
#pragma unroll
        for (int j = 0; j < 4; ++j) acc[j] = fmaxf(acc[j], 0.f);
      } else if (a.act == VX_ACT_LRELU) {
#pragma unroll
        for (int j = 0; j < 4; ++j) acc[j] = fmaxf(acc[j], 0.01f * acc[j]);
      }
      if (a.drop_mode == VX_DROP_HASH) {
        const uint32_t bits = vx_drop_bits4(dkey, (uint32_t)(((oz * OH + oy) * OW + ox) * a.Cout + oco[rt]));
#pragma unroll
        for (int j = 0; j < 4; ++j) acc[j] *= __uint_as_float((bits << (30 - j)) & 0x40000000u);
      }
      if constexpr (MASK) {
        const uint32_t mk = *reinterpret_cast<const uint32_t*>(a.drop_mask + (orow * OW + ox) * a.Cout + oco[rt]);
#pragma unroll
        for (int j = 0; j < 4; ++j) acc[j] = ((mk >> (8 * j)) & 0xFFu) ? 2.f * acc[j] : 0.f;
      }
      float* op;
      if (a.out_xblk)
        op = a.out + orow * (2 * (size_t)OW * a.Cout) +
             ((((ox >> xs) * 2 + a.out_half) << xs) + (ox & (a.out_xblk - 1))) * a.Cout + oco[rt];
      else
        op = a.out + (orow * OW + ox) * a.out_pitch + a.out_coff + oco[rt];
      *reinterpret_cast<f32x4*>(op) = acc;
      rmax = fmaxf(fmaxf(rmax, fmaxf(fabsf(acc[0]), fabsf(acc[1]))), fmaxf(fabsf(acc[2]), fabsf(acc[3])));
    }
  }
  if (a.range_flag) {
#pragma unroll
    for (int off = 32; off >= 1; off >>= 1) rmax = fmaxf(rmax, __shfl_xor(rmax, off, 64));
    if (lane == 0 && !(rmax < 32768.f)) atomicMax(a.range_flag, __float_as_uint(rmax));
  }
}

#include "s16_common.h"
template <int CIN, int RT, bool MASK = false>
__global__ __launch_bounds__(256) void convT_k2s2_s16_kernel(vx_convT_args a, int ncoltiles, int nvox_in, ConvTDecode dc) {
  constexpr int Q = CIN / 32;
  const int tid = threadIdx.x, lane = tid & 63, wave = tid >> 6;
  const int m = lane & 15, g = lane >> 4;
  const int OW = a.W * 2, OH = a.H * 2, OD = a.D * 2;
  const int rt0 = blockIdx.y * RT;
  f16x8 wh[RT][Q], wl[RT][Q];
  float rmax = 0.f;
#pragma unroll
  for (int rt = 0; rt < RT; ++rt) {
    const int row = 16 * (rt0 + rt) + m;
    const int pos = row / a.Cout, co = row % a.Cout;
    const float* wp = a.w_packed + (size_t)(pos >> 1) * CIN * 2 * a.Cout + (pos & 1) * a.Cout + co;
#pragma unroll
    for (int q = 0; q < Q; ++q)
#pragma unroll
      for (int j = 0; j < 8; ++j) {
        const float w = wp[(size_t)(32 * q + 8 * g + j) * 2 * a.Cout];
        const float c = fminf(fmaxf(w, -65504.f), 65504.f);
        if (!(fabsf(w) <= 65504.f)) rmax = __builtin_inff();
        const _Float16 h = (_Float16)c;
        wh[rt][q][j] = h;
        wl[rt][q][j] = (_Float16)((c - (float)h) * 2048.f);
      }
  }
  int opos[RT], oco[RT];
#pragma unroll
  for (int rt = 0; rt < RT; ++rt) {
    const int row = 16 * (rt0 + rt) + 4 * g;
    opos[rt] = row / a.Cout;
    oco[rt] = row % a.Cout;
  }
  const int xs = a.out_xblk ? __builtin_ctz((unsigned)a.out_xblk) : 0;
  const int wstride = (int)gridDim.x * 4;
  auto load_x = [&](int ct, f32x4* dst) {
    int v = ct * 16 + m;
    if (v >= nvox_in) v = nvox_in - 1;
    const float* __restrict__ xin = a.in + (size_t)v * a.in_pitch + 8 * g;
#pragma unroll
    for (int q = 0; q < Q; ++q) {
      dst[2 * q] = *reinterpret_cast<const f32x4*>(xin + 32 * q);
      dst[2 * q + 1] = *reinterpret_cast<const f32x4*>(xin + 32 * q + 4);
    }
  };
  f32x4 xnext[2 * Q];
  {
    const int ct0 = blockIdx.x * 4 + wave;
    load_x(ct0 < ncoltiles ? ct0 : ncoltiles - 1, xnext);
  }
  const uint32_t seed0 = vx_seed_of(a, a.drop_seed);
  const f32x4 zero = {0.f, 0.f, 0.f, 0.f};
  for (int ct = blockIdx.x * 4 + wave; ct < ncoltiles; ct += wstride) {
    const int v = ct * 16 + m;
    const int vc = v < nvox_in ? v : nvox_in - 1;
    f16x8 bh[Q], bl[Q];
#pragma unroll
    for (int q = 0; q < Q; ++q) {
      typedef unsigned u32x2 __attribute__((ext_vector_type(2)));
      f16x4 h0, l0, h1, l1;
      vx_split4(xnext[2 * q], h0, l0);
      vx_split4(xnext[2 * q + 1], h1, l1);
      const u32x2 a0 = __builtin_bit_cast(u32x2, h0), a1 = __builtin_bit_cast(u32x2, h1);
      const u32x2 c0 = __builtin_bit_cast(u32x2, l0), c1 = __builtin_bit_cast(u32x2, l1);
      bh[q] = __builtin_bit_cast(f16x8, (u32x4){a0[0], a0[1], a1[0], a1[1]});
      bl[q] = __builtin_bit_cast(f16x8, (u32x4){c0[0], c0[1], c1[0], c1[1]});
    }
    {
      const int ctn = ct + wstride;
      load_x(ctn < ncoltiles ? ctn : ncoltiles - 1, xnext);
    }
    __builtin_amdgcn_sched_barrier(0);
    asm volatile("s_nop 7" ::: "memory");
    __builtin_amdgcn_sched_barrier(0);
    unsigned r = (unsigned)vc, qq;
    qq = ct_div(r, dc.mW); const int x = (int)(r - qq * (unsigned)a.W); r = qq;
    qq = ct_div(r, dc.mH); const int y = (int)(r - qq * (unsigned)a.H); r = qq;
    qq = ct_div(r, dc.mD); const int z = (int)(r - qq * (unsigned)a.D);
    const int n = (int)qq;
    const vx_dkey dkey = vx_drop_key(seed0, a.drop_layer, (uint32_t)n);
#pragma unroll
    for (int rt = 0; rt < RT; ++rt) {
      f32x4 acc = *reinterpret_cast<const f32x4*>(a.bias + oco[rt]);
      f32x4 accx = zero;
#pragma unroll
      for (int q = 0; q < Q; ++q) {
        acc = __builtin_amdgcn_mfma_f32_16x16x32_f16(wh[rt][q], bh[q], acc, 0, 0, 0);
        accx = __builtin_amdgcn_mfma_f32_16x16x32_f16(wh[rt][q], bl[q], accx, 0, 0, 0);
        accx = __builtin_amdgcn_mfma_f32_16x16x32_f16(wl[rt][q], bh[q], accx, 0, 0, 0);
      }
#pragma unroll
      for (int j = 0; j < 4; ++j) acc[j] = fmaf(accx[j], 1.0f / 2048.f, acc[j]);
      const int pos = opos[rt];
      const int oz = 2 * z + (pos >> 2), oy = 2 * y + ((pos >> 1) & 1), ox = 2 * x + (pos & 1);
      const size_t orow = ((size_t)n * OD + oz) * OH + oy;
      if (a.act == VX_ACT_RELU) {
#pragma unroll
        for (int j = 0; j < 4; ++j) acc[j] = fmaxf(acc[j], 0.f);
      } else if (a.act == VX_ACT_LRELU) {
#pragma unroll
        for (int j = 0; j < 4; ++j) acc[j] = fmaxf(acc[j], 0.01f * acc[j]);
      }
      if (a.drop_mode == VX_DROP_HASH) {
        const uint32_t bits = vx_drop_bits4(dkey, (uint32_t)(((oz * OH + oy) * OW + ox) * a.Cout + oco[rt]));
#pragma unroll
        for (int j = 0; j < 4; ++j) acc[j] *= __uint_as_float((bits << (30 - j)) & 0x40000000u);
      }
      if constexpr (MASK) {
        const uint32_t mk = *reinterpret_cast<const uint32_t*>(a.drop_mask + (orow * OW + ox) * a.Cout + oco[rt]);
#pragma unroll
        for (int j = 0; j < 4; ++j) acc[j] = ((mk >> (8 * j)) & 0xFFu) ? 2.f * acc[j] : 0.f;
      }
      float* op;
      if (a.out_xblk)
        op = a.out + orow * (2 * (size_t)OW * a.Cout) +
             ((((ox >> xs) * 2 + a.out_half) << xs) + (ox & (a.out_xblk - 1))) * a.Cout + oco[rt];
      else
        op = a.out + (orow * OW + ox) * a.out_pitch + a.out_coff + oco[rt];
      *reinterpret_cast<f32x4*>(op) = acc;
      rmax = fmaxf(fmaxf(rmax, fmaxf(fabsf(acc[0]), fabsf(acc[1]))), fmaxf(fabsf(acc[2]), fabsf(acc[3])));
    }
  }
  if (a.range_flag) {
#pragma unroll
    for (int off = 32; off >= 1; off >>= 1) rmax = fmaxf(rmax, __shfl_xor(rmax, off, 64));
    if (lane == 0 && !(rmax < 32768.f)) atomicMax(a.range_flag, __float_as_uint(rmax));
  }
}

template <int CIN, int RT>
static int launch_convT_s16(const vx_convT_args& a, hipStream_t s) {
  const int64_t nvox = (int64_t)a.N * a.D * a.H * a.W;
  const int ncoltiles = (int)((nvox + 15) / 16);
  const int groups = (a.Cout / 2) / RT;
  int bx = (ncoltiles + 3) / 4;
  const int cap = (512 + groups - 1) / groups;
  if (bx > cap) bx = cap;
  auto magic = [](int d) { return d == 1 ? 0u : (unsigned)((1ull << 32) / (unsigned)d) + 1u; };
  ConvTDecode dc;
  dc.mW = magic(a.W); dc.mH = magic(a.H); dc.mD = magic(a.D);
  static const char* kname = vx_kname("convT_k2s2_s16_kernel<%d,%d,false>", CIN, RT);
  static const char* kname_m = vx_kname("convT_k2s2_s16_kernel<%d,%d,true>", CIN, RT);
  vx_note_kernel(a.drop_mode == VX_DROP_MASK ? kname_m : kname);
  if (a.drop_mode == VX_DROP_MASK)
    hipLaunchKernelGGL((convT_k2s2_s16_kernel<CIN, RT, true>), dim3((unsigned)bx, (unsigned)groups), dim3(256), 0, s, a, ncoltiles,
                       (int)nvox, dc);
  else
    hipLaunchKernelGGL((convT_k2s2_s16_kernel<CIN, RT, false>), dim3((unsigned)bx, (unsigned)groups), dim3(256), 0, s, a, ncoltiles,
                       (int)nvox, dc);
  VX_CHECK_LAUNCH("vx_convT_k2s2(s16)");
  return VX_OK;
}

template <int CIN, int RT>
static int launch_convT_mfma(const vx_convT_args& a, hipStream_t s) {
  const int64_t nvox = (int64_t)a.N * a.D * a.H * a.W;
  const int ncoltiles = (int)((nvox + 15) / 16);
  const int groups = (a.Cout / 2) / RT;
  int bx = (ncoltiles + 3) / 4;
  int per = 32;
  const int cap = (256 * per + groups - 1) / groups;
  if (bx > cap) bx = cap;
  auto magic = [](int d) { return d == 1 ? 0u : (unsigned)((1ull << 32) / (unsigned)d) + 1u; };
  ConvTDecode dc;
  dc.mW = magic(a.W); dc.mH = magic(a.H); dc.mD = magic(a.D);
  static const char* kname = vx_kname("convT_k2s2_mfma_kernel<%d,%d,false>", CIN, RT);
  static const char* kname_m = vx_kname("convT_k2s2_mfma_kernel<%d,%d,true>", CIN, RT);
  vx_note_kernel(a.drop_mode == VX_DROP_MASK ? kname_m : kname);
  if (a.drop_mode == VX_DROP_MASK)
    hipLaunchKernelGGL((convT_k2s2_mfma_kernel<CIN, RT, true>), dim3((unsigned)bx, (unsigned)groups), dim3(256), 0, s, a,
                       ncoltiles, (int)nvox, dc);
  else
    hipLaunchKernelGGL((convT_k2s2_mfma_kernel<CIN, RT, false>), dim3((unsigned)bx, (unsigned)groups), dim3(256), 0, s, a,
                       ncoltiles, (int)nvox, dc);
  VX_CHECK_LAUNCH("vx_convT_k2s2(mfma)");
  return VX_OK;
}

__global__ void pack_convT_kernel(const float* __restrict__ w, float* __restrict__ out, int Cin, int Cout, int64_t total) {
  for (int64_t i = blockIdx.x * (int64_t)blockDim.x + threadIdx.x; i < total; i += (int64_t)gridDim.x * blockDim.x) {
    int64_t r = i;
    const int co = r % Cout; r /= Cout;
    const int dx = r % 2; r /= 2;
    const int ci = r % Cin; r /= Cin;
    const int dy = r % 2; r /= 2;
    const int dz = (int)r;
    out[i] = w[(((size_t)ci * Cout + co) * 2 + dz) * 4 + dy * 2 + dx];
  }
}

extern "C" int64_t vx_convT_k2s2_packed_floats(int Cin, int Cout) {
  if (Cin <= 0 || Cout <= 0 || Cin % 4 || Cout % 8) return -1;
  return (int64_t)Cin * Cout * 8;
}

extern "C" int vx_pack_convT_k2s2(const float* w_torch, float* w_packed, int Cin, int Cout, vx_stream_t stream) {
  if (!w_torch || !w_packed) VX_FAIL(VX_E_NULL, "vx_pack_convT_k2s2: null pointer");
  const int64_t total = vx_convT_k2s2_packed_floats(Cin, Cout);
  if (total < 0) VX_FAIL(VX_E_SHAPE, "vx_pack_convT_k2s2: Cin=%d (mult of 4) Cout=%d (mult of 8)", Cin, Cout);
  int blocks = (int)((total + 255) / 256);
  if (blocks > 4096) blocks = 4096;
  hipLaunchKernelGGL(pack_convT_kernel, dim3(blocks), dim3(256), 0, (hipStream_t)stream, w_torch, w_packed, Cin, Cout,
                     total);
  VX_CHECK_LAUNCH("vx_pack_convT_k2s2");
  return VX_OK;
}

extern "C" int vx_convT_k2s2(const vx_convT_args* ap, vx_stream_t stream) {
  if (!ap) VX_FAIL(VX_E_NULL, "vx_convT_k2s2: null args");
  const vx_convT_args& a = *ap;
  if (!a.in || !a.w_packed || !a.bias || !a.out) VX_FAIL(VX_E_NULL, "vx_convT_k2s2: null tensor");
  if (a.Cin <= 0 || a.Cout <= 0 || a.Cin % 4 || a.Cout % 8)
    VX_FAIL(VX_E_SHAPE, "vx_convT_k2s2: Cin=%d (mult of 4) Cout=%d (mult of 8)", a.Cin, a.Cout);
  if (a.N <= 0 || a.D <= 0 || a.H <= 0 || a.W <= 0) VX_FAIL(VX_E_SHAPE, "vx_convT_k2s2: empty tensor");
  if (a.in_pitch % 4 || a.in_pitch < a.Cin) VX_FAIL(VX_E_ALIGN, "vx_convT_k2s2: input pitch");
  if (a.out_xblk) {
    if ((a.out_xblk != 1 && a.out_xblk != 2 && a.out_xblk != 4) || (2 * a.W) % a.out_xblk || (a.out_half != 0 && a.out_half != 1))
      VX_FAIL(VX_E_SHAPE, "vx_convT_k2s2: bad concat layout (xblk=%d, half=%d)", a.out_xblk, a.out_half);
  } else if (a.out_pitch % 4 || a.out_coff % 4 || a.out_pitch < a.out_coff + a.Cout) {
    VX_FAIL(VX_E_ALIGN, "vx_convT_k2s2: pitches/offsets must be multiples of 4 floats");
  }
  if (a.drop_mode == VX_DROP_MASK && !a.drop_mask) VX_FAIL(VX_E_NULL, "vx_convT_k2s2: mask mode without mask");
  if ((int64_t)a.D * a.H * a.W * 8 * a.Cout >= (1ll << 32)) VX_FAIL(VX_E_SHAPE, "vx_convT_k2s2: sample too large");
  const int64_t dmax = a.W > a.H ? (a.W > a.D ? a.W : a.D) : (a.H > a.D ? a.H : a.D);
  if ((int64_t)a.N * a.D * a.H * a.W < (1ll << 27) && (int64_t)a.N * a.D * a.H * a.W * dmax < (1ll << 32)) {
    hipStream_t s = (hipStream_t)stream;
    const int tiles = a.Cout / 2;
    if (a.Cin == 16 && tiles % 4 == 0) return tiles % 8 ? launch_convT_mfma<16, 4>(a, s) : launch_convT_mfma<16, 8>(a, s);
    if (a.Cin == 32 && tiles % 4 == 0) return tiles % 8 ? launch_convT_mfma<32, 4>(a, s) : launch_convT_mfma<32, 8>(a, s);
    if (vx_cfg().conv_fp32 == 0) {
      if (a.Cin == 64 && tiles % 4 == 0) return launch_convT_s16<64, 4>(a, s);
      if (a.Cin == 128 && tiles % 2 == 0) return launch_convT_s16<128, 2>(a, s);
    }
    if (a.Cin == 64 && tiles % 4 == 0) return tiles % 8 ? launch_convT_mfma<64, 4>(a, s) : launch_convT_mfma<64, 8>(a, s);
    if (a.Cin == 128 && tiles % 4 == 0) return launch_convT_mfma<128, 4>(a, s);
  }
  if ((a.Cin == 16 || a.Cin == 32) && a.Cout <= 128 && 256 % (2 * (a.Cout / 4)) == 0) {
    const int64_t total = (int64_t)a.N * a.D * a.H * (2 * a.W) * (a.Cout / 4);
    int bx = (int)((total + 255) / 256);
    if (bx > 4096) bx = 4096;
    dim3 grid((unsigned)bx, 4);
    vx_note_kernel("convT_k2s2_rows_kernel");
    if (a.Cin == 16)
      hipLaunchKernelGGL(convT_k2s2_rows_kernel<16>, grid, dim3(256), 0, (hipStream_t)stream, a, total);
    else
      hipLaunchKernelGGL(convT_k2s2_rows_kernel<32>, grid, dim3(256), 0, (hipStream_t)stream, a, total);
    VX_CHECK_LAUNCH("vx_convT_k2s2");
    return VX_OK;
  }
  const int64_t nvox = (int64_t)a.N * a.D * a.H * a.W;
  int bx = (int)((nvox + 255) / 256);
  if (bx > 8192) bx = 8192;
  dim3 grid((unsigned)bx, (unsigned)(4 * (a.Cout / CT_CO)));
  vx_note_kernel("convT_k2s2_kernel");
  hipLaunchKernelGGL(convT_k2s2_kernel, grid, dim3(256), 0, (hipStream_t)stream, a, nvox);
  VX_CHECK_LAUNCH("vx_convT_k2s2");
  return VX_OK;
}
```

values_amd/csrc/lib.cpp:

```cpp
#include <stdarg.h>
#include <stdio.h>
#include <stdlib.h>
#include <string.h>

#include "../../include/values_amd.h"

static thread_local char g_err[512] = "";

void vx_set_error(const char* fmt, ...) {
  va_list ap;
  va_start(ap, fmt);
  vsnprintf(g_err, sizeof(g_err), fmt, ap);
  va_end(ap);
}

static thread_local const char* g_last_kernel = nullptr;
void vx_note_kernel(const char* name) { g_last_kernel = name; }
const char* vx_last_kernel() { return g_last_kernel; }
const char* vx_kname(const char* fmt, ...) {
  char buf[256];
  va_list ap;
  va_start(ap, fmt);
  vsnprintf(buf, sizeof(buf), fmt, ap);
  va_end(ap);
  char* p = (char*)malloc(strlen(buf) + 1);
  strcpy(p, buf);
  return p;
}

#include <mutex>
#include <stdlib.h>
#include <string.h>

static vx_config g_cfg;
static std::once_flag g_cfg_once;

static int env_int(const char* name, int dflt) {
  const char* e = getenv(name);
  if (!e || !*e) return dflt;
  char* end = nullptr;
  const long v = strtol(e, &end, 0);
  return end == e ? 1 : (int)v;
}

static void cfg_from_env() {
  memset(&g_cfg, 0, sizeof(g_cfg));
  g_cfg.conv_fp32 = env_int("VX_CONV_FP32", 0);
  g_cfg.s16_no_prenorm = env_int("VX_S16_NO_PRENORM", 0);
  g_cfg.s16_no_xp8 = env_int("VX_S16_NO_XP8", 0);
  g_cfg.s16_skip_raw = env_int("VX_S16_SKIP_RAW", 1);
  g_cfg.no_head_fusion = env_int("VX_NO_HEAD_FUSION", 0);
  g_cfg.s16_no_upfuse = env_int("VX_S16_NO_UPFUSE", 0);
  g_cfg.s16_no_poolfuse = env_int("VX_S16_NO_POOLFUSE", 0);
  g_cfg.storage16 = env_int("VX_STORAGE16", 0);
  g_cfg.s16_generic = env_int("VX_S16_GENERIC", 0);
  g_cfg.s16_no_zc16 = env_int("VX_S16_NO_ZC16", 0);
  g_cfg.s16_no_halves = env_int("VX_S16_NO_HALVES", 0);
  g_cfg.s16_no_deep = env_int("VX_S16_NO_DEEP", 0);
  g_cfg.s16_no_l1dma = env_int("VX_S16_NO_L1DMA", 0);
  g_cfg.c2s_no_wide = env_int("VX_C2S_NO_WIDE", 0);
  g_cfg.c2s_no_oct = env_int("VX_C2S_NO_OCT", 0);
}

const vx_config& vx_cfg() {
  std::call_once(g_cfg_once, cfg_from_env);
  return g_cfg;
}

extern "C" int vx_get_config(vx_config* out) {
  if (!out) { vx_set_error("vx_get_config: null"); return VX_E_NULL; }
  *out = vx_cfg();
  return VX_OK;
}

extern "C" int vx_set_config(const vx_config* cfg) {
  if (!cfg) { vx_set_error("vx_set_config: null"); return VX_E_NULL; }
  if (cfg->conv_fp32 < 0 || cfg->conv_fp32 > 2) { vx_set_error("vx_set_config: conv_fp32 %d", cfg->conv_fp32); return VX_E_DTYPE; }
  (void)vx_cfg();
  g_cfg = *cfg;
  return VX_OK;
}

extern "C" const char* vx_last_kernel_name(void) { return g_last_kernel ? g_last_kernel : ""; }
extern "C" int vx_version(void) { return 903;  }
extern "C" const char* vx_last_error_string(void) { return g_err; }
```

values_amd/csrc/unet3d_forward.hip:

```cpp
#include "conv3d_internal.h"

namespace {
struct Level { int D, H, W, C; int64_t nvox; };

struct Plan {
  Level lv[5];
  float *A[4], *B[4], *CAT[4], *P[5], *C0, *C1;
  float *stats, *mean, *rstd;
  float *mean0, *rstd0;
  float *meanS[4], *rstdS[4];
  size_t bytes;
};

static size_t align_up(size_t v) { return (v + 255) & ~(size_t)255; }

static void make_plan(Plan& p, int N, int D, int H, int W, int F, char* base) {
  size_t off = 0;
  auto carve = [&](size_t floats) {
    float* q = base ? (float*)(base + off) : nullptr;
    off += align_up(floats * sizeof(float));
    return q;
  };
  for (int l = 0; l < 5; ++l) {
    p.lv[l].D = D >> l; p.lv[l].H = H >> l; p.lv[l].W = W >> l; p.lv[l].C = F << l;
    p.lv[l].nvox = (int64_t)p.lv[l].D * p.lv[l].H * p.lv[l].W;
  }
  for (int l = 0; l < 4; ++l) {
    const size_t e = (size_t)N * p.lv[l].nvox * p.lv[l].C;
    p.A[l] = carve(e);
    p.B[l] = carve(e);
    p.CAT[l] = carve(2 * e);
  }
  p.P[0] = nullptr;
  for (int l = 1; l < 5; ++l) p.P[l] = carve((size_t)N * p.lv[l].nvox * p.lv[l - 1].C);
  p.C0 = carve((size_t)N * p.lv[4].nvox * p.lv[4].C);
  p.C1 = carve((size_t)N * p.lv[4].nvox * p.lv[4].C);
  size_t smax = 0;
  for (int l = 0; l < 4; ++l) {
    size_t t = (size_t)vx_conv3d_k3_tiles(p.lv[l].D, p.lv[l].H, p.lv[l].W);
    if (l == 0) {
      size_t t1 = (size_t)vx_conv3d_k3_c1_tiles(p.lv[0].D, p.lv[0].H, p.lv[0].W);
      if (t1 > t) t = t1;
    }
    const size_t e = (size_t)N * t * p.lv[l].C * 2;
    if (e > smax) smax = e;
  }
  p.stats = carve(smax);
  p.mean = carve((size_t)N * p.lv[3].C);
  p.rstd = carve((size_t)N * p.lv[3].C);
  p.mean0 = carve((size_t)N * p.lv[0].C);
  p.rstd0 = carve((size_t)N * p.lv[0].C);
  for (int l = 0; l < 4; ++l) {
    p.meanS[l] = l == 0 ? p.mean0 : carve((size_t)N * p.lv[l].C);
    p.rstdS[l] = l == 0 ? p.rstd0 : carve((size_t)N * p.lv[l].C);
  }
  p.bytes = off;
}
}

extern "C" size_t vx_unet3d_workspace_bytes(int N, int D, int H, int W, int F) {
  if (N <= 0 || D <= 0 || H <= 0 || W <= 0 || F <= 0) return 0;
  Plan p;
  make_plan(p, N, D, H, W, F, nullptr);
  return p.bytes;
}

namespace {
struct Prof {
  static constexpr int MAXL = 96;
  hipEvent_t ev[2 * MAXL];
  const char* name[MAXL];
  const char* kernel[MAXL];
  int n = 0;
  hipStream_t s;
};
thread_local Prof* g_prof = nullptr;
thread_local char g_prof_labels[Prof::MAXL][192];
}

#define VX_TRY(expr)            \
  do {                          \
    int rc_ = (expr);           \
    if (rc_ != VX_OK) return rc_; \
  } while (0)

#define VX_STEP(label, expr)                                                       \
  do {                                                                             \
    Prof* pf_ = g_prof;                                                            \
    if (pf_ && pf_->n < Prof::MAXL) { vx_note_kernel(nullptr); (void)hipEventRecord(pf_->ev[2 * pf_->n], pf_->s); }  \
    int rc_ = (expr);                                                              \
    if (rc_ != VX_OK) return rc_;                                                  \
    if (pf_ && pf_->n < Prof::MAXL) {                                              \
      (void)hipEventRecord(pf_->ev[2 * pf_->n + 1], pf_->s);                             \
      pf_->kernel[pf_->n] = vx_last_kernel();                                      \
      pf_->name[pf_->n++] = (label);                                               \
    }                                                                              \
  } while (0)

namespace {
int xblk_of(int W) { return W % 4 == 0 ? 4 : (W % 2 == 0 ? 2 : 1); }

struct Flow {
  bool inorm;
  int ich;
  int rep;
  bool shared;
  bool fuse_head;
  bool pre[4];
  bool presplit;
  bool skip_raw[4];
  bool pooled[4];
  bool poolfin1;
  bool halves[4];
  bool fuse_up;
  bool fuse_up1;
  bool split_out[4];
  bool planar1;
  bool st16;
  int products_c12, products_e11, products_e12;
};

Flow decide_flow(const vx_unet3d_weights* w, const vx_unet3d_run* r, const Plan& p) {
  const vx_config& cfg = vx_cfg();
  const int F = w->F, dm = r->drop_mode;
  const Level* lv = p.lv;
  const bool hashed = dm != VX_DROP_MASK;
  Flow f = {};
  f.inorm = !w->no_instancenorm;
  f.ich = w->in_channels > 1 ? w->in_channels : 1;
  f.rep = r->repeat > 0 ? r->repeat : 1;
  f.shared = !r->src && !r->flip && f.rep > 1 && r->N % f.rep == 0;
  f.fuse_head = w->num_classes <= 4 && vx_conv3d_k3_head_fusable(F, F) && !cfg.no_head_fusion;
  f.pre[0] = hashed && !cfg.s16_no_prenorm && F == 8 && f.inorm && vx_conv3d_k3_prologue_ok(lv[0].D, lv[0].H, lv[0].W, F, F);
  for (int l = 1; l < 4; ++l)
    f.pre[l] = f.inorm && hashed && !cfg.s16_no_prenorm && vx_conv3d_k3_prologue_ok(lv[l].D, lv[l].H, lv[l].W, lv[l].C, lv[l].C);
  f.presplit = f.shared && f.pre[0] && vx_conv3d_k3_presplit_ok(lv[0].D, lv[0].H, lv[0].W, F, F);
  f.skip_raw[0] = f.pre[0] && cfg.s16_skip_raw && vx_conv3d_k3_prologue_ok(lv[0].D, lv[0].H, lv[0].W, 2 * F, F);
  f.pooled[0] = f.skip_raw[0] && vx_conv3d_k3_poolfuse_ok(lv[0].D, lv[0].H, lv[0].W, F, F);
  f.poolfin1 = f.pooled[0] && vx_conv3d_k3_poolfin_ok(F, 2 * F);
  for (int l = 1; l < 4; ++l) {
    const Level& L = lv[l];
    f.skip_raw[l] = f.pooled[l] = f.inorm && hashed && !cfg.s16_no_prenorm && cfg.s16_skip_raw &&
                                  vx_conv3d_k3_pool_layout(L.D, L.H, L.W, L.C, L.C) == 2 &&
                                  vx_conv3d_k3_skip_prologue_ok(L.D, L.H, L.W, 2 * L.C, L.C, xblk_of(L.W));
  }
  f.halves[1] = f.skip_raw[1] && lv[1].C == 16 && w->split_w[0] && w->split_w[1] && !cfg.s16_no_halves &&
                w->split_family == vx_conv3d_k3_family(16, 16) && vx_conv3d_k3_acc_ok(lv[1].D, lv[1].H, lv[1].W, 16, 16);
  f.fuse_up = hashed && F == 8 && vx_conv3d_k3_upfuse_ok(lv[0].D, lv[0].H, lv[0].W, 2 * F, F);
  f.fuse_up1 = f.halves[1] && w->up3_zc16 && hashed && vx_conv3d_k3_upfuse_ok(lv[1].D, lv[1].H, lv[1].W, 16, 16) == 2;
  f.split_out[1] = f.fuse_up;
  f.split_out[2] = f.fuse_up1;
  f.planar1 = f.fuse_up1 && !cfg.s16_no_l1dma && vx_conv3d_k3_planar_ok(lv[1].D, lv[1].H, lv[1].W, 16, 16);
  f.st16 = cfg.storage16 && dm == VX_DROP_HASH && F == 8 && f.fuse_head && cfg.conv_fp32 == 0 &&
           vx_conv3d_k3_prologue_ok(lv[0].D, lv[0].H, lv[0].W, F, F);
  const bool one = f.st16 && cfg.storage16 == 2;
  f.products_c12 = one && f.presplit && f.pooled[0];
  f.products_e11 = one && f.skip_raw[0] && f.fuse_up && w->up_fused;
  f.products_e12 = one;
  return f;
}
}

extern "C" int vx_unet3d_forward(const vx_unet3d_weights* w, const vx_unet3d_run* r, vx_stream_t stream) {
  if (!w || !r) VX_FAIL(VX_E_NULL, "vx_unet3d_forward: null argument");
  if (!r->x || !r->logits || !r->workspace) VX_FAIL(VX_E_NULL, "vx_unet3d_forward: null tensor/workspace");
  const int N = r->N, D = r->D, H = r->H, W = r->W, F = w->F, NC = w->num_classes;
  if (N <= 0 || D <= 0 || H <= 0 || W <= 0) VX_FAIL(VX_E_SHAPE, "vx_unet3d_forward: empty batch");
  if (D % 16 || H % 16 || W % 16)
    VX_FAIL(VX_E_SHAPE, "vx_unet3d_forward: spatial size (%d,%d,%d) must be divisible by 16 (4 poolings; InstanceNorm "
            "needs > 1 voxel at the 8x level)", D, H, W);
  if (F != 8 && F != 16 && F != 32) VX_FAIL(VX_E_SHAPE, "vx_unet3d_forward: initial_filter_size %d unsupported (8,16,32)", F);
  if (NC <= 0) VX_FAIL(VX_E_SHAPE, "vx_unet3d_forward: num_classes %d", NC);
  if (r->drop_mode < 0 || r->drop_mode > 2) VX_FAIL(VX_E_DTYPE, "vx_unet3d_forward: drop_mode %d", r->drop_mode);
  if ((((uintptr_t)r->workspace) & 255u) != 0) VX_FAIL(VX_E_ALIGN, "vx_unet3d_forward: workspace must be 256-byte aligned");
  for (int i = 0; i < 18; ++i)
    if (!w->conv_w[i] || !w->conv_b[i]) VX_FAIL(VX_E_NULL, "vx_unet3d_forward: conv weight %d missing", i);
  if (w->in_channels < 0 || w->in_channels > 8) VX_FAIL(VX_E_SHAPE, "vx_unet3d_forward: in_channels %d (1 .. 8)", w->in_channels);
  for (int i = 0; i < 4; ++i)
    if (!w->up_w[i] || !w->up_b[i]) VX_FAIL(VX_E_NULL, "vx_unet3d_forward: transposed-conv weight %d missing", i);
  if (!w->final_w || !w->final_b) VX_FAIL(VX_E_NULL, "vx_unet3d_forward: final weights missing");
  if (r->drop_mode == VX_DROP_MASK)
    for (int i = 0; i < 17; ++i)
      if (!r->masks[i]) VX_FAIL(VX_E_NULL, "vx_unet3d_forward: mask %d missing", i);

  Plan p;
  make_plan(p, N, D, H, W, F, (char*)r->workspace);
  if (p.bytes > r->workspace_bytes)
    VX_FAIL(VX_E_WORKSPACE, "vx_unet3d_forward: workspace %zu B < required %zu B", r->workspace_bytes, p.bytes);
  const Flow f = decide_flow(w, r, p);

  const int dm = r->drop_mode;
  auto mask = [&](int i) { return dm == VX_DROP_MASK ? r->masks[i] : (const uint8_t*)nullptr; };
  auto conv_args = [&](int wi, const Level& L, int Cin, int Cout, float* stats) {
    vx_conv3d_args a = {};
    a.w_packed = w->conv_w[wi]; a.bias = w->conv_b[wi]; a.w_family = w->conv_family[wi];
    a.N = N; a.D = L.D; a.H = L.H; a.W = L.W; a.Cin = Cin; a.Cout = Cout;
    a.drop_seed = r->seed; a.seed_dev = r->seed_dev;
    a.stats_partial = stats; a.range_flag = stats ? nullptr : r->range_flag;
    a.out_half = 1;
    return a;
  };
  auto set_drop = [&](vx_conv3d_args& a, int act, int layer) {
    a.act = act; a.drop_mode = dm; a.drop_layer = (uint32_t)layer; a.drop_mask = mask(layer);
  };
  auto set_pre = [&](vx_conv3d_args& a, int layer, int rep, const float* mean, const float* rstd) {
    a.in_mean = mean; a.in_rstd = rstd; a.in_repeat = rep;
    a.in_drop_mode = dm; a.in_drop_seed = r->seed; a.in_drop_layer = (uint32_t)layer;
  };
  auto norm_args = [&](const float* x, int C, const Level& L, int drop_layer, bool normalise) {
    vx_norm_args a = {};
    a.x = x; a.x_pitch = C; a.x_half = 1; a.out_half = 1; a.pool_pitch = C;
    a.mean = normalise ? p.mean : nullptr; a.rstd = normalise ? p.rstd : nullptr;
    a.range_flag = normalise ? nullptr : r->range_flag;
    a.N = N; a.D = L.D; a.H = L.H; a.W = L.W; a.C = C;
    a.act = VX_ACT_LRELU;
    a.drop_mode = drop_layer >= 0 ? dm : VX_DROP_NONE; a.drop_seed = r->seed; a.drop_layer = (uint32_t)(drop_layer >= 0 ? drop_layer : 0);
    a.drop_mask = drop_layer >= 0 ? mask(drop_layer) : nullptr;
    a.seed_dev = r->seed_dev;
    return a;
  };
  auto convT = [&](const float* in, int ui, float* out, int out_pitch, const Level& Lin, int Cin, int Cout, int act,
                   int drop_layer, bool dense) {
    vx_convT_args a = {};
    a.range_flag = r->range_flag;
    a.seed_dev = r->seed_dev;
    a.out_xblk = dense ? 0 : xblk_of(2 * Lin.W); a.out_half = 0;
    a.in = in; a.in_pitch = Cin; a.w_packed = w->up_w[ui]; a.bias = w->up_b[ui];
    a.out = out; a.out_pitch = out_pitch; a.out_coff = 0;
    a.N = N; a.D = Lin.D; a.H = Lin.H; a.W = Lin.W; a.Cin = Cin; a.Cout = Cout;
    a.act = act;
    a.drop_mode = drop_layer >= 0 ? dm : VX_DROP_NONE;
    a.drop_seed = r->seed; a.drop_layer = (uint32_t)(drop_layer >= 0 ? drop_layer : 0);
    a.drop_mask = drop_layer >= 0 ? mask(drop_layer) : nullptr;
    return vx_convT_k2s2(&a, stream);
  };
  auto pool_flags = [&](int l) {
    const size_t maxima = l == 0 ? (size_t)N * p.lv[1].nvox * 8 : (size_t)N * (p.lv[l].nvox / 4) * p.lv[l].C;
    return reinterpret_cast<uint32_t*>(p.B[l] + maxima);
  };
  auto first_conv = [&](float* out, int n_out, int rep, float* stats) -> int {
    const Level& L = p.lv[0];
    if (f.ich == 1)
      return vx_conv3d_k3_c1(r->x, w->conv_w[0], w->conv_b[0], out, L.C, n_out, L.D, L.H, L.W, L.C, rep, r->src, r->flip, stats, stream);
    VX_TRY(vx_pack_input_cl8(r->x, p.B[0], n_out, f.ich, L.D, L.H, L.W, rep, r->src, r->flip, stream));
    vx_conv3d_args a = conv_args(0, L, 8, L.C, stats);
    a.N = n_out; a.in = p.B[0]; a.in_pitch = 8; a.out = out; a.out_pitch = L.C;
    return vx_conv3d_k3(&a, stream);
  };

  static const char* kConv[18] = {"contr_1_1", "contr_1_2", "contr_2_1", "contr_2_2", "contr_3_1", "contr_3_2",
                                  "contr_4_1", "contr_4_2", "center.0", "center.2", "expand_4_1", "expand_4_2",
                                  "expand_3_1", "expand_3_2", "expand_2_1", "expand_2_2", "expand_1_1", "expand_1_2"};
  static const char* kNorm[8] = {"norm:contr_1_1", "norm:contr_1_2", "norm:contr_2_1", "norm:contr_2_2",
                                 "norm:contr_3_1", "norm:contr_3_2", "norm:contr_4_1", "norm:contr_4_2"};
  static const char* kFin[8] = {"finalize:contr_1_1", "finalize:contr_1_2", "finalize:contr_2_1", "finalize:contr_2_2",
                                "finalize:contr_3_1", "finalize:contr_3_2", "finalize:contr_4_1", "finalize:contr_4_2"};
  static const char* kPoolFin[4] = {"poolfin:contr_1_2", "poolfin:contr_2_2", "poolfin:contr_3_2", "poolfin:contr_4_2"};
  static const char* kUp[4] = {"center.4", "upscale4", "upscale3", "upscale2"};
  float* const out1 = f.shared && !f.skip_raw[0] ? p.CAT[0] : p.A[0];
  const int fan = f.shared ? f.rep : 1;
  for (int l = 0; l < 4; ++l) {
    const Level& L = p.lv[l];
    const int C = L.C;
    const int ntiles = vx_conv3d_k3_tiles_for(L.D, L.H, L.W, C);
    if (l == 0) {
      const int n1 = N / fan;
      const int ntiles1 = f.ich == 1 ? vx_conv3d_k3_c1_tiles(L.D, L.H, L.W) : ntiles;
      VX_STEP(kConv[0], first_conv(out1, n1, f.shared ? 1 : f.rep, f.inorm ? p.stats : nullptr));
      if (f.inorm) VX_STEP(kFin[0], vx_instnorm_finalize(p.stats, n1, ntiles1, C, L.nvox, 1e-5f, p.mean, p.rstd, stream));
      if (f.presplit)
        VX_STEP("presplit:contr_1_1", vx_prenorm_split(out1, p.mean, p.rstd, n1, L.nvox, dm == VX_DROP_HASH ? 2.f : 1.f, stream));
      if (!f.pre[0]) {
        vx_norm_args n = norm_args(out1, C, L, 0, f.inorm);
        n.out = p.A[0]; n.out_pitch = C;
        VX_STEP(kNorm[0], vx_norm_act_drop_pool_bcast(&n, fan, stream));
      }
    } else {
      vx_conv3d_args a = conv_args(2 * l, L, C / 2, C, f.inorm ? p.stats : nullptr);
      a.in = p.P[l]; a.in_pitch = C / 2; a.out = p.A[l]; a.out_pitch = C;
      if (!f.inorm) set_drop(a, VX_ACT_LRELU, 2 * l);
      if (l == 1 && f.poolfin1) {
        a.in = p.B[0]; a.in_pool_flags = pool_flags(0);
        set_pre(a, 1, 1, p.mean0, p.rstd0);
      }
      VX_STEP(l == 1 && f.poolfin1 ? "poolfin+contr_2_1" : kConv[2 * l], vx_conv3d_k3(&a, stream));
      if (f.inorm) {
        VX_STEP(kFin[2 * l], vx_instnorm_finalize(p.stats, N, ntiles, C, L.nvox, 1e-5f, p.mean, p.rstd, stream));
        if (!f.pre[l]) {
          vx_norm_args n = norm_args(p.A[l], C, L, 2 * l, true);
          n.out = p.A[l]; n.out_pitch = C;
          VX_STEP(kNorm[2 * l], vx_norm_act_drop_pool_bcast(&n, 1, stream));
        }
      }
    }
    if (!f.inorm) {
      vx_conv3d_args a = conv_args(2 * l + 1, L, C, C, nullptr);
      a.in = p.A[l]; a.in_pitch = C; a.out = p.B[l]; a.out_pitch = C;
      set_drop(a, VX_ACT_LRELU, 2 * l + 1);
      VX_STEP(kConv[2 * l + 1], vx_conv3d_k3(&a, stream));
      vx_norm_args n = norm_args(p.B[l], C, L, -1, false);
      n.act = VX_ACT_NONE;
      n.out = p.CAT[l]; n.out_pitch = 2 * C; n.out_coff = C; n.out_xblk = xblk_of(L.W); n.pool_out = p.P[l + 1];
      VX_STEP(kNorm[2 * l + 1], vx_norm_act_drop_pool_bcast(&n, 1, stream));
      continue;
    }
    vx_conv3d_args a = conv_args(2 * l + 1, L, C, C, p.stats);
    a.in = p.A[l]; a.in_pitch = C; a.out = p.B[l]; a.out_pitch = C;
    if (f.pre[l]) {
      if (l == 0) a.in = out1;
      set_pre(a, 2 * l, l == 0 ? fan : 1, p.mean, p.rstd);
    }
    a.in_split = l == 0 && f.presplit;
    if (l == 0) a.products = f.products_c12;
    if (f.skip_raw[l]) {
      if (f.halves[l]) a.out = p.CAT[l] + (size_t)N * L.nvox * C;
      else { a.out = p.CAT[l]; a.out_xblk = xblk_of(L.W); }
    }
    if (f.pooled[l]) {
      a.pool_out = p.B[l]; a.pool_flags = pool_flags(l);
      set_drop(a, VX_ACT_NONE, 2 * l + 1);
    }
    VX_STEP(kConv[2 * l + 1], vx_conv3d_k3(&a, stream));
    if (l == 0 && f.skip_raw[0]) {
      VX_STEP(kFin[1], vx_instnorm_finalize(p.stats, N, ntiles, C, L.nvox, 1e-5f, p.mean0, p.rstd0, stream));
      if (!f.pooled[0]) {
        vx_norm_args n = norm_args(p.CAT[0], C, L, 1, true);
        n.mean = p.mean0; n.rstd = p.rstd0; n.x_xblk = xblk_of(L.W); n.pool_out = p.P[1];
        VX_STEP("pool:contr_1_2", vx_norm_act_drop_pool_bcast(&n, 1, stream));
      } else if (!f.poolfin1) {
        VX_STEP(kPoolFin[0], vx_pool_finish(p.B[0], pool_flags(0), p.mean0, p.rstd0, p.P[1], C, N, p.lv[1].nvox, dm == VX_DROP_HASH, stream));
      }
    } else if (f.skip_raw[l]) {
      const vx_stat_src st = {p.stats, ntiles, 1e-5f, (int64_t)L.nvox, p.meanS[l], p.rstdS[l]};
      VX_STEP(kPoolFin[l], vx_pool_finish_z_stats(p.B[l], pool_flags(l), &st, p.P[l + 1], C, N, L.D / 2, (int64_t)(L.H / 2) * (L.W / 2),
                                                  dm == VX_DROP_HASH, stream));
    } else {
      vx_norm_args n = norm_args(p.B[l], C, L, 2 * l + 1, true);
      n.out = p.CAT[l]; n.out_pitch = 2 * C; n.out_coff = C; n.out_xblk = xblk_of(L.W); n.pool_out = p.P[l + 1];
      if (C <= 512) {
        n.mean = nullptr; n.rstd = nullptr;
        const vx_stat_src st = {p.stats, ntiles, 1e-5f, (int64_t)L.nvox, p.mean, p.rstd};
        VX_STEP(kNorm[2 * l + 1], vx_norm_act_drop_pool_stats(&n, &st, stream));
      } else {
        VX_STEP(kFin[2 * l + 1], vx_instnorm_finalize(p.stats, N, ntiles, C, L.nvox, 1e-5f, p.mean, p.rstd, stream));
        VX_STEP(kNorm[2 * l + 1], vx_norm_act_drop_pool_bcast(&n, 1, stream));
      }
    }
  }
  {
    const Level& L4 = p.lv[4];
    const int C3 = p.lv[3].C, C4 = L4.C;
    vx_conv3d_args a = conv_args(8, L4, C3, C4, nullptr);
    a.in = p.P[4]; a.in_pitch = C3; a.out = p.C0; a.out_pitch = C4; a.act = VX_ACT_RELU;
    VX_STEP(kConv[8], vx_conv3d_k3(&a, stream));
    vx_conv3d_args b = conv_args(9, L4, C4, C4, nullptr);
    b.in = p.C0; b.in_pitch = C4; b.out = p.C1; b.out_pitch = C4; b.act = VX_ACT_RELU;
    VX_STEP(kConv[9], vx_conv3d_k3(&b, stream));
    VX_STEP(kUp[0], convT(p.C1, 0, p.CAT[3], 2 * C3, L4, C4, C3, VX_ACT_RELU, 8, false));
  }
  for (int l = 3; l >= 0; --l) {
    const Level& L = p.lv[l];
    const int C = L.C;
    const int wi = 10 + 2 * (3 - l);
    const int dl = 9 + 2 * (3 - l);
    if (f.halves[l]) {
      vx_conv3d_args a = conv_args(wi, L, C, C, nullptr);
      a.w_packed = w->split_w[1]; a.w_family = w->split_family;
      a.in = p.CAT[l] + (size_t)N * L.nvox * C; a.in_pitch = C; a.out = p.A[l]; a.out_pitch = C;
      set_pre(a, 2 * l + 1, 1, p.meanS[l], p.rstdS[l]);
      a.range_flag = nullptr;
      VX_STEP("expand_2_1(skip half)", vx_conv3d_k3(&a, stream));
      vx_conv3d_args b = conv_args(wi, L, C, C, nullptr);
      b.w_packed = w->split_w[0]; b.w_family = w->split_family;
      b.in = p.CAT[l]; b.in_pitch = C; b.out = p.A[l]; b.out_pitch = C; b.acc_in = p.A[l]; b.acc_pitch = C;
      set_drop(b, VX_ACT_LRELU, dl);
      if (f.fuse_up1) {
        b.in = p.B[l + 1]; b.up_in = p.B[l + 1]; b.up_pitch = 2 * C; b.up_w = w->up3_zc16; b.up_b = w->up_b[2];
        b.up_split = 1;
        b.up_fused = w->up3_fused;
      }
      if (f.planar1) { b.out = p.CAT[l]; b.out_planar = 1; }
      VX_STEP(f.fuse_up1 ? "upscale3+expand_2_1(up half)" : "expand_2_1(up half)", vx_conv3d_k3(&b, stream));
    } else {
      vx_conv3d_args a = conv_args(wi, L, 2 * C, C, nullptr);
      a.in = p.CAT[l]; a.in_pitch = 2 * C; a.in_xblk = xblk_of(L.W); a.out = p.A[l]; a.out_pitch = C;
      set_drop(a, VX_ACT_LRELU, dl);
      if (f.skip_raw[l]) set_pre(a, 2 * l + 1, 1, p.meanS[l], p.rstdS[l]);
      if (l == 0 && f.fuse_up) {
        a.up_in = p.B[1]; a.up_w = w->up_w[3]; a.up_b = w->up_b[3]; a.up_pitch = 2 * C;
        a.up_fused = w->up_fused;
        a.up_split = 1;
      }
      if (l == 0) { a.out_f16 = f.st16; a.products = f.products_e11; }
      VX_STEP(l == 0 && f.fuse_up ? "upscale2+expand_1_1" : kConv[wi], vx_conv3d_k3(&a, stream));
    }
    vx_conv3d_args a = conv_args(wi + 1, L, C, C, nullptr);
    a.in = p.A[l]; a.in_pitch = C; a.out = p.B[l]; a.out_pitch = C;
    set_drop(a, VX_ACT_LRELU, dl + 1);
    if (l == 1 && f.planar1) { a.in = p.CAT[l]; a.in_planar = 1; }
    a.out_split = f.split_out[l];
    if (l == 0) { a.in_f16 = f.st16; a.products = f.products_e12; }
    if (l == 0 && f.fuse_head) {
      a.out = nullptr;
      a.head_out = r->logits; a.head_w = w->final_w; a.head_b = w->final_b; a.head_C = NC; a.head_dst = r->dst; a.head_flip = r->flip;
    }
    VX_STEP(l == 0 && f.fuse_head ? "expand_1_2+final" : kConv[wi + 1], vx_conv3d_k3(&a, stream));
    if (l > 0 && !(l == 1 && f.fuse_up) && !(l == 2 && f.fuse_up1))
      VX_STEP(kUp[4 - l], convT(p.B[l], 4 - l, p.CAT[l - 1], f.halves[l - 1] ? C / 2 : C, L, C, C / 2, VX_ACT_NONE, -1, f.halves[l - 1]));
  }
  if (!f.fuse_head)
    VX_STEP("final", vx_conv1x1_ncdhw(p.B[0], F, w->final_w, w->final_b, r->logits, N, D, H, W, F, NC, r->dst, r->flip, stream));
  return VX_OK;
}

extern "C" int vx_unet3d_forward_profiled(const vx_unet3d_weights* w, const vx_unet3d_run* r, vx_stream_t stream,
                                          int max_launches, float* ms, const char** labels, int* n_launches) {
  if (!ms || !labels || !n_launches) VX_FAIL(VX_E_NULL, "vx_unet3d_forward_profiled: null output");
  Prof pf;
  pf.s = (hipStream_t)stream;
  for (int i = 0; i < 2 * Prof::MAXL; ++i) {
    hipError_t e = hipEventCreate(&pf.ev[i]);
    if (e != hipSuccess) VX_FAIL((int)e, "hipEventCreate: %s", hipGetErrorString(e));
  }
  g_prof = &pf;
  int rc = vx_unet3d_forward(w, r, stream);
  g_prof = nullptr;
  if (rc == VX_OK) {
    hipError_t e = hipStreamSynchronize(pf.s);
    if (e != hipSuccess) { vx_set_error("hipStreamSynchronize: %s", hipGetErrorString(e)); rc = (int)e; }
  }
  int n = 0;
  if (rc == VX_OK) {
    for (; n < pf.n && n < max_launches; ++n) {
      float t = 0.f;
      (void)hipEventElapsedTime(&t, pf.ev[2 * n], pf.ev[2 * n + 1]);
      ms[n] = t;
      snprintf(g_prof_labels[n], sizeof(g_prof_labels[n]), "%s|%s", pf.name[n], pf.kernel[n] ? pf.kernel[n] : "?");
      labels[n] = g_prof_labels[n];
    }
  }
  *n_launches = n;
  for (int i = 0; i < 2 * Prof::MAXL; ++i) (void)hipEventDestroy(pf.ev[i]);
  return rc;
}
```

values_amd/unet3d.py:

```python
from __future__ import annotations

import ctypes as C
from typing import List, Optional, Sequence

import torch
import torch.nn as nn

from . import _lib

CONV_ORDER = ["contr_1_1.0", "contr_1_2.0", "contr_2_1.0", "contr_2_2.0", "contr_3_1.0", "contr_3_2.0",
              "contr_4_1.0", "contr_4_2.0", "center.0", "center.2", "expand_4_1.0", "expand_4_2.0",
              "expand_3_1.0", "expand_3_2.0", "expand_2_1.0", "expand_2_2.0", "expand_1_1.0", "expand_1_2.0"]
UP_ORDER = ["center.4", "upscale4", "upscale3", "upscale2"]
DROPOUT_ORDER = ["contr_1_1", "contr_1_2", "contr_2_1", "contr_2_2", "contr_3_1", "contr_3_2", "contr_4_1",
                 "contr_4_2", "center", "expand_4_1", "expand_4_2", "expand_3_1", "expand_3_2", "expand_2_1",
                 "expand_2_2", "expand_1_1", "expand_1_2"]


def _block(cin, cout, k, norm, p):
    layers = [nn.Conv3d(cin, cout, k, padding=1)]
    if norm:
        layers.append(nn.InstanceNorm3d(cout))
    layers += [nn.LeakyReLU(inplace=True), nn.Dropout(p=p)]
    return nn.Sequential(*layers)


class UNet3D(nn.Module):
    def __init__(self, num_classes: int, in_channels: int = 1, initial_filter_size: int = 8, kernel_size: int = 3,
                 do_instancenorm: bool = True, do_dropout: bool = False, aleatoric_loss: bool = False):
        super().__init__()
        if kernel_size != 3:
            raise NotImplementedError("values_amd.UNet3D: only kernel_size=3 (every shipped config) has a HIP kernel")
        if not 1 <= in_channels <= 8:
            raise NotImplementedError("values_amd.UNet3D: in_channels must be 1 .. 8")
        if initial_filter_size not in (8, 16, 32):
            raise NotImplementedError("values_amd.UNet3D: initial_filter_size must be 8, 16 or 32")
        self.num_classes = num_classes
        self.aleatoric_loss = aleatoric_loss
        self.in_channels = in_channels
        self.do_instancenorm = bool(do_instancenorm)
        self.initial_filter_size = initial_filter_size
        self.dropout_prob = 0.5 if do_dropout else 0.0
        f, p = initial_filter_size, self.dropout_prob
        chans = [f, 2 * f, 4 * f, 8 * f]
        prev = in_channels
        for lvl, c in enumerate(chans, start=1):
            setattr(self, f"contr_{lvl}_1", _block(prev, c, 3, do_instancenorm, p))
            setattr(self, f"contr_{lvl}_2", _block(c, c, 3, do_instancenorm, p))
            prev = c
        center = [nn.Conv3d(8 * f, 16 * f, 3, padding=1), nn.ReLU(inplace=True),
                  nn.Conv3d(16 * f, 16 * f, 3, padding=1), nn.ReLU(inplace=True),
                  nn.ConvTranspose3d(16 * f, 8 * f, 2, stride=2), nn.ReLU(inplace=True)]
        if do_dropout:
            center.append(nn.Dropout(p=p))
        self.center = nn.Sequential(*center)
        for lvl in (4, 3, 2, 1):
            c = chans[lvl - 1]
            setattr(self, f"expand_{lvl}_1", _block(2 * c, c, 3, False, p))
            setattr(self, f"expand_{lvl}_2", _block(c, c, 3, False, p))
            if lvl > 1:
                setattr(self, f"upscale{lvl}", nn.ConvTranspose3d(c, c // 2, kernel_size=2, stride=2))
        self.final = nn.Conv3d(f, num_classes, kernel_size=1)
        if aleatoric_loss:
            self.final_aleatoric = nn.Conv3d(f, num_classes * 2, kernel_size=1)
        self.output_reconstruction_map = nn.Conv3d(f, out_channels=1, kernel_size=1)
        self._packed = None
        self._packed_key = None
        self._packed_by_mode = {}
        self._range = {}
        self._ws = {}
        self._calls = 0
        self.seed = 123

    def _param_key(self):
        return tuple((p.data_ptr(), p._version, p.dtype, str(p.device)) for p in self.parameters()) + (_lib.pack_mode(),)

    def _ensure_packed(self, device):
        key = self._param_key()
        mode = (key[-1], str(device))
        hit = self._packed_by_mode.get(mode)
        if hit is not None and hit[0] == key:
            self._packed, self._packed_key = hit[1], key
            return self._packed
        lib = _lib.load()
        sd = {k: v.detach().to(device=device, dtype=torch.float32).contiguous() for k, v in self.state_dict().items()}
        keep = []
        w = _lib.UNet3DWeights()
        st = _lib.stream_ptr()
        for i, name in enumerate(CONV_ORDER):
            wt, b = sd[name + ".weight"], sd[name + ".bias"]
            cout, cin = wt.shape[0], wt.shape[1]
            if i == 0 and cin > 1:
                wt8 = torch.zeros((cout, 8) + tuple(wt.shape[2:]), dtype=torch.float32, device=device)
                wt8[:, :cin] = wt
                wt, cin = wt8.contiguous(), 8
                n = lib.vx_conv3d_k3_packed_floats(cin, cout)
                packed = torch.empty(n, dtype=torch.float32, device=device)
                _lib.check(lib.vx_pack_conv3d_k3(_lib.ptr(wt), _lib.ptr(packed), cin, cout, st), "vx_pack_conv3d_k3")
            elif i == 0:
                packed = wt
            else:
                n = lib.vx_conv3d_k3_packed_floats(cin, cout)
                if n < 0:
                    raise _lib.VxError(f"conv {name}: Cin={cin} Cout={cout} unsupported")
                packed = torch.empty(n, dtype=torch.float32, device=device)
                _lib.check(lib.vx_pack_conv3d_k3(_lib.ptr(wt), _lib.ptr(packed), cin, cout, st), "vx_pack_conv3d_k3")
            keep += [packed, b, wt]
            w.conv_w[i] = packed.data_ptr()
            w.conv_b[i] = b.data_ptr()
            w.conv_family[i] = 0 if (i == 0 and cin == 1) else lib.vx_conv3d_k3_family(cin, cout)
        for i, name in enumerate(UP_ORDER):
            wt, b = sd[name + ".weight"], sd[name + ".bias"]
            cin, cout = wt.shape[0], wt.shape[1]
            n = lib.vx_convT_k2s2_packed_floats(cin, cout)
            packed = torch.empty(n, dtype=torch.float32, device=device)
            _lib.check(lib.vx_pack_convT_k2s2(_lib.ptr(wt), _lib.ptr(packed), cin, cout, st), "vx_pack_convT_k2s2")
            keep += [packed, b, wt]
            w.up_w[i] = packed.data_ptr()
            w.up_b[i] = b.data_ptr()
        if self.initial_filter_size == 8 and _lib.get_config().conv_fp32 == 0:
            uf = torch.empty(lib.vx_conv3d_upfused_packed_floats(), dtype=torch.float32, device=device)
            _lib.check(lib.vx_pack_conv3d_upfused(_lib.ptr(sd["expand_1_1.0.weight"]), _lib.ptr(sd["expand_1_1.0.bias"]),
                                                  _lib.ptr(sd["upscale2.weight"]), _lib.ptr(sd["upscale2.bias"]), _lib.ptr(uf), st),
                       "vx_pack_conv3d_upfused")
            keep.append(uf)
            w.up_fused = uf.data_ptr()
            w2 = sd["expand_2_1.0.weight"]
            for hidx in range(2):
                part = w2[:, 16 * hidx:16 * (hidx + 1)].contiguous()
                pk = torch.empty(lib.vx_conv3d_k3_packed_floats(16, 16), dtype=torch.float32, device=device)
                _lib.check(lib.vx_pack_conv3d_k3(_lib.ptr(part), _lib.ptr(pk), 16, 16, st), "vx_pack_conv3d_k3 (expand_2_1 half)")
                keep += [part, pk]
                w.split_w[hidx] = pk.data_ptr()
            w.split_family = lib.vx_conv3d_k3_family(16, 16)
            u3 = torch.empty(lib.vx_convT_zc16_packed_floats(), dtype=torch.float32, device=device)
            _lib.check(lib.vx_pack_convT_zc16(_lib.ptr(sd["upscale3.weight"]), _lib.ptr(u3), st), "vx_pack_convT_zc16")
            keep.append(u3)
            w.up3_zc16 = u3.data_ptr()
            if hasattr(lib, "vx_pack_conv3d_upfused_zc16"):
                u3f = torch.empty(lib.vx_conv3d_upfused_zc16_packed_floats(), dtype=torch.float32, device=device)
                _lib.check(lib.vx_pack_conv3d_upfused_zc16(_lib.ptr(w2), _lib.ptr(sd["upscale3.weight"]), _lib.ptr(sd["upscale3.bias"]),
                                                           _lib.ptr(u3f), st), "vx_pack_conv3d_upfused_zc16")
                keep.append(u3f)
                w.up3_fused = u3f.data_ptr()
        fw, fb = self._head_params(sd)
        keep += [fw, fb]
        w.final_w = fw.data_ptr()
        w.final_b = fb.data_ptr()
        w.F = self.initial_filter_size
        w.num_classes = fw.shape[0]
        w.in_channels = self.in_channels
        w.no_instancenorm = 0 if self.do_instancenorm else 1
        self._packed = (w, keep)
        self._packed_key = key
        self._packed_by_mode[mode] = (key, self._packed)
        return self._packed

    def _head_params(self, sd):
        head = "final_aleatoric" if self.aleatoric_loss else "final"
        return sd[head + ".weight"].reshape(sd[head + ".weight"].shape[0], -1).contiguous(), sd[head + ".bias"]

    def _workspace(self, N, D, H, W, device):
        geo = (N, D, H, W, str(device))
        sid = torch.cuda.current_stream(device).cuda_stream
        ent = self._ws.get(sid)
        if ent is None or ent[0] != geo:
            nbytes = _lib.load().vx_unet3d_workspace_bytes(N, D, H, W, self.initial_filter_size)
            self._ws.pop(sid, None)
            ent = (geo, torch.empty(nbytes + 256, dtype=torch.uint8, device=device))
            self._ws[sid] = ent
        ws = ent[1]
        off = (-ws.data_ptr()) % 256
        return ws, off, ws.numel() - 256

    FP16_MAX = 65504.0

    def range_max(self, reset: bool = False) -> float:
        worst = 0.0
        for flag in self._range.values():
            worst = max(worst, float(flag.view(torch.float32).item()))
            if reset:
                flag.zero_()
        return worst

    def range_reset(self):
        for flag in self._range.values():
            flag.zero_()

    def next_seed(self) -> int:
        seed = (self.seed * 1000003 + self._calls) & 0xFFFFFFFF
        self._calls += 1
        return seed

    def check_range(self, reset: bool = True):
        m = self.range_max(reset=reset)
        if not m < self.FP16_MAX:
            raise _lib.VxError(f"values_amd.UNet3D: an activation of magnitude {m:.4g} reached a split-fp16 convolution "
                               f"(limit {self.FP16_MAX}); re-run under _lib.config(conv_fp32=1)")

    def dropout_layer_shapes(self, D, H, W):
        f = self.initial_filter_size
        enc = [(f << l, (D >> l, H >> l, W >> l)) for l in range(4) for _ in range(2)]
        dec = [(f << l, (D >> l, H >> l, W >> l)) for l in (3, 2, 1, 0) for _ in range(2)]
        return enc + [(8 * f, (D >> 3, H >> 3, W >> 3))] + dec

    def hash_dropout_masks(self, seed: int, N: int, D: int, H: int, W: int, device=None):
        _lib.require_gpu()
        lib = _lib.load()
        dev = torch.device("cuda", torch.cuda.current_device()) if device is None else torch.device(device)
        out = []
        for layer, (c, (d, h, w)) in enumerate(self.dropout_layer_shapes(D, H, W)):
            m = torch.empty((N, d, h, w, c), dtype=torch.uint8, device=dev)
            _lib.check(lib.vx_drop_hash_mask(int(seed) & 0xFFFFFFFF, layer, N, d * h * w * c, _lib.ptr(m),
                                             _lib.stream_ptr()), "vx_drop_hash_mask")
            out.append(m.permute(0, 4, 1, 2, 3).bool())
        return out

    def forward(self, x: torch.Tensor, enable_concat: bool = True, last_layer: bool = True, *,
                n_samples: int = 1, src: Optional[torch.Tensor] = None, flip: Optional[torch.Tensor] = None,
                dst: Optional[torch.Tensor] = None, out: Optional[torch.Tensor] = None,
                dropout_masks: Optional[Sequence[torch.Tensor]] = None, seed: Optional[int] = None,
                seed_dev: Optional[torch.Tensor] = None):
        if not enable_concat or not last_layer:
            raise NotImplementedError("values_amd.UNet3D: autoencoder / feature modes are training-only and not on the HIP path")
        res = self._run(x, n_samples=n_samples, src=src, flip=flip, dst=dst, out=out, dropout_masks=dropout_masks, seed=seed,
                        seed_dev=seed_dev)
        if self.aleatoric_loss:
            mu, s = res.split(self.num_classes, 1)
            return mu, s
        return res

    def _run(self, x, *, n_samples=1, src=None, flip=None, dst=None, out=None, dropout_masks=None, seed=None, seed_dev=None):
        _lib.require_gpu()
        lib = _lib.load()
        if x.dim() != 5 or x.shape[1] != self.in_channels:
            raise ValueError(f"expected (N,{self.in_channels},D,H,W) input, got {tuple(x.shape)}")
        in_dtype = x.dtype
        dev = x.device if x.is_cuda else torch.device("cuda", torch.cuda.current_device())
        xf = x.detach().to(device=dev, dtype=torch.float32).contiguous()
        V, _, D, H, W = xf.shape
        if src is not None:
            N = int(src.numel())
        else:
            N = V * int(n_samples)
        w, _keep = self._ensure_packed(dev)
        NC = w.num_classes
        ws, off, ws_bytes = self._workspace(N, D, H, W, dev)
        if out is None:
            out = torch.empty((N, NC, D, H, W), dtype=torch.float32, device=dev)
        run = _lib.UNet3DRun()
        run.x = xf.data_ptr()
        run.N, run.D, run.H, run.W = N, D, H, W
        run.repeat = int(n_samples)
        hold = [xf, out, ws]
        for name, t in (("src", src), ("flip", flip), ("dst", dst)):
            if t is not None:
                t = t.to(device=dev, dtype=torch.int32).contiguous()
                hold.append(t)
                setattr(run, name, t.data_ptr())
        if dropout_masks is not None:
            if len(dropout_masks) != 17:
                raise ValueError("dropout_masks: need 17 masks in DROPOUT_ORDER")
            run.drop_mode = _lib.VX_DROP_MASK
            for i, m in enumerate(dropout_masks):
                m = m.to(device=dev).permute(0, 2, 3, 4, 1).contiguous().to(torch.uint8)
                hold.append(m)
                run.masks[i] = m.data_ptr()
        elif self.training and self.dropout_prob > 0:
            run.drop_mode = _lib.VX_DROP_HASH
            if seed is None:
                seed = self.next_seed()
            run.seed = int(seed) & 0xFFFFFFFF
            if seed_dev is not None:
                if seed_dev.dtype != torch.int32 or not seed_dev.is_cuda:
                    raise ValueError("seed_dev: an int32 device tensor of one element")
                hold.append(seed_dev)
                run.seed_dev = seed_dev.data_ptr()
        else:
            run.drop_mode = _lib.VX_DROP_NONE
        flag = self._range.get(str(dev))
        if flag is None:
            flag = self._range[str(dev)] = torch.zeros(1, dtype=torch.int32, device=dev)
        run.range_flag = flag.data_ptr()
        run.logits = out.data_ptr()
        run.workspace = ws.data_ptr() + off
        run.workspace_bytes = ws_bytes
        _lib.check(lib.vx_unet3d_forward(C.byref(w), C.byref(run), _lib.stream_ptr()), "vx_unet3d_forward")
        self._hold = hold
        return out if in_dtype == torch.float32 else out.to(in_dtype)
```

Measured before the change: 3932 volumes/s.

## Compose upscale4 transposed conv with expand_3_1 up-half and accumulate skip half

Precomposes the upscale4 k2s2 transposed convolution with the up-channel half of expand_3_1 into per-parity effective weights, stored as split f16 hi/lo pairs. A new MFMA kernel applies these composed weights straight to the 8^3 bottleneck features, writing partial expand_3_1 sums. The skip half then runs as a 32->32 deep conv that adds those partials through a new acc_in path. This removes the materialised upsampled tensor and the 64-channel concat read at level 2. In exchange it adds extra MFMA passes for split precision, a boundary-dependent bias table and a new routing branch.

```diff
diff --git a/include/values_amd.h b/include/values_amd.h
--- a/include/values_amd.h
+++ b/include/values_amd.h
@@ -206,8 +206,12 @@
   int32_t out_xblk, out_half;
   uint32_t* range_flag;
   const uint32_t* seed_dev;
+  const float* up_fused;
 } vx_convT_args;
 int vx_convT_k2s2(const vx_convT_args* a, vx_stream_t stream);
+int64_t vx_convT_upfused32_packed_floats(void);
+int vx_pack_convT_upfused32(const float* w1_torch, int w1_cin, const float* up_w_torch, const float* up_b, float* packed, vx_stream_t stream);
+int vx_convT_k2s2_upfused_ok(int D, int H, int W, int Cin, int Cout);
 
 int vx_conv1x1_ncdhw(const float* in, int in_pitch, const float* w, const float* bias, float* out, int N, int D,
                      int H, int W, int F, int C, const int32_t* dst, const int32_t* flip, vx_stream_t stream);
@@ -229,6 +233,9 @@
   int32_t split_family;
   const float* up3_zc16;
   const float* up3_fused;
+  const float* up4_fused;
+  const float* split3_w;
+  int32_t split3_family;
 } vx_unet3d_weights;
 
 typedef struct vx_unet3d_run {
diff --git a/values_amd/_lib.py b/values_amd/_lib.py
--- a/values_amd/_lib.py
+++ b/values_amd/_lib.py
@@ -52,7 +52,7 @@
                 ("out", _p), ("out_pitch", _i32), ("out_coff", _i32),
                 ("N", _i32), ("D", _i32), ("H", _i32), ("W", _i32), ("Cin", _i32), ("Cout", _i32),
                 ("act", _i32), ("drop_mode", _i32), ("drop_seed", _u32), ("drop_layer", _u32), ("drop_mask", _p),
-                ("out_xblk", _i32), ("out_half", _i32), ("range_flag", _p), ("seed_dev", _p)]
+                ("out_xblk", _i32), ("out_half", _i32), ("range_flag", _p), ("seed_dev", _p), ("up_fused", _p)]
 
 
 class Conv2dArgs(C.Structure):
@@ -116,7 +116,8 @@
 class UNet3DWeights(C.Structure):
     _fields_ = [("conv_w", _p * 18), ("conv_b", _p * 18), ("up_w", _p * 4), ("up_b", _p * 4),
                 ("final_w", _p), ("final_b", _p), ("F", _i32), ("num_classes", _i32), ("conv_family", _i32 * 18),
-                ("in_channels", _i32), ("no_instancenorm", _i32), ("up_fused", _p), ("split_w", _p * 2), ("split_family", _i32), ("up3_zc16", _p), ("up3_fused", _p)]
+                ("in_channels", _i32), ("no_instancenorm", _i32), ("up_fused", _p), ("split_w", _p * 2), ("split_family", _i32), ("up3_zc16", _p), ("up3_fused", _p),
+                ("up4_fused", _p), ("split3_w", _p), ("split3_family", _i32)]
 
 
 class UNet3DRun(C.Structure):
@@ -290,6 +291,9 @@
     "vx_pack_conv3d_upfused": (_i, [_p, _p, _p, _p, _p, _p]),
     "vx_pack_conv3d_upfused_zc16": (_i, [_p, _p, _p, _p, _p]),
     "vx_conv3d_upfused_zc16_packed_floats": (_i64, []),
+    "vx_convT_upfused32_packed_floats": (_i64, []),
+    "vx_pack_convT_upfused32": (_i, [_p, _i, _p, _p, _p, _p]),
+    "vx_convT_k2s2_upfused_ok": (_i, [_i, _i, _i, _i, _i]),
     "vx_pool_finish": (_i, [_p, _p, _p, _p, _p, _i, _i, _i64, _i, _p]),
     "vx_pool_finish_z": (_i, [_p, _p, _p, _p, _p, _i, _i, _i, _i64, _i, _p]),
     "vx_conv3d_k3_pool_layout": (_i, [_i, _i, _i, _i, _i]),
diff --git a/values_amd/csrc/conv3d_deep.hip b/values_amd/csrc/conv3d_deep.hip
--- a/values_amd/csrc/conv3d_deep.hip
+++ b/values_amd/csrc/conv3d_deep.hip
@@ -352,6 +352,28 @@
       }
       int m_ = m;
       asm volatile("" : "+v"(m_));
+      f32x4 part[R][NT];
+      bool has_acc = false;
+      if constexpr (!STATS) has_acc = kp->a.acc_in != nullptr;
+      if constexpr (!STATS) {
+        if (has_acc) {
+          const __amdgpu_buffer_rsrc_t asrd = __builtin_amdgcn_make_buffer_rsrc(
+              (void*)(const_cast<float*>(kp->a.acc_in) + (size_t)n0 * out_sample), 0, VX_NUMREC, 0x00020000);
+#pragma unroll
+          for (int r = 0; r < R; ++r) {
+            int cx_, ly, lz, smp;
+            vox_of((wave * R + r) * 16 + m_, cx_, ly, lz, smp);
+            const int ovox = (lz * a.H + ly) * a.W + cx_;
+            unsigned aoff = ((unsigned)smp * (unsigned)out_sample + (unsigned)ovox * (unsigned)out_voxf + (unsigned)kp->a.out_coff + 4u * g) * 4u;
+            if constexpr (R == 2) {
+              if (n0 + smp >= a.N) aoff = VX_OOB;
+            }
+#pragma unroll
+            for (int nt = 0; nt < NT; ++nt)
+              part[r][nt] = __builtin_bit_cast(f32x4, __builtin_amdgcn_raw_buffer_load_b128(asrd, (int)aoff, (int)(osoff + (unsigned)(nt * 64)), 0));
+          }
+        }
+      }
 #pragma unroll
       for (int r = 0; r < R; ++r) {
         int cx_, ly, lz, smp;
@@ -374,6 +396,12 @@
           if (STATS) {
 #pragma unroll
             for (int j = 0; j < 4; ++j) { ssum[nt][j] += v[j]; ssq[nt][j] = fmaf(v[j], v[j], ssq[nt][j]); }
+          }
+          if constexpr (!STATS) {
+            if (has_acc) {
+#pragma unroll
+              for (int j = 0; j < 4; ++j) v[j] += part[r][nt][j];
+            }
           }
           if (f_lrelu) {
 #pragma unroll
diff --git a/values_amd/csrc/conv3d_k3.hip b/values_amd/csrc/conv3d_k3.hip
--- a/values_amd/csrc/conv3d_k3.hip
+++ b/values_amd/csrc/conv3d_k3.hip
@@ -53,7 +53,11 @@
 extern "C" int vx_conv3d_k3_skip_prologue_ok(int D, int H, int W, int Cin, int Cout, int xblk) {
   return conv3d_skip_prologue_ok(D, H, W, Cin, Cout, xblk, vx_cfg());
 }
-extern "C" int vx_conv3d_k3_acc_ok(int D, int H, int W, int Cin, int Cout) { return conv3d_zc16_16to16(D, H, W, Cin, Cout, vx_cfg()) ? 1 : 0; }
+extern "C" int vx_conv3d_k3_acc_ok(int D, int H, int W, int Cin, int Cout) {
+  const vx_config& cfg = vx_cfg();
+  if (conv3d_zc16_16to16(D, H, W, Cin, Cout, cfg)) return 1;
+  return conv3d_channels_ok(Cin, Cout) && conv_config(Cin, Cout, cfg).S16 && conv3d_deep_applies(D, H, W, Cin, Cout, cfg) ? 1 : 0;
+}
 extern "C" int vx_conv3d_k3_planar_ok(int D, int H, int W, int Cin, int Cout) { return conv3d_zc16_16to16(D, H, W, Cin, Cout, vx_cfg()) ? 1 : 0; }
 extern "C" int vx_conv3d_k3_upfuse_ok(int D, int H, int W, int Cin, int Cout) { return conv3d_upfuse_ok(D, H, W, Cin, Cout, vx_cfg()); }
 extern "C" int vx_conv3d_k3_pool_layout(int D, int H, int W, int Cin, int Cout) { return conv3d_pool_layout(D, H, W, Cin, Cout, vx_cfg()); }
diff --git a/values_amd/csrc/conv3d_route.h b/values_amd/csrc/conv3d_route.h
--- a/values_amd/csrc/conv3d_route.h
+++ b/values_amd/csrc/conv3d_route.h
@@ -402,11 +402,15 @@
   return ROUTE_DECLINED;
 }
 
+static inline bool conv3d_deep_acc(const vx_conv3d_args& a) {
+  return !a.stats_partial && !a.in_mean && !a.in_xblk && !a.out_split && a.acc_pitch == a.out_pitch && conv3d_aligned16(a.acc_in);
+}
 static inline int route_deep(const vx_conv3d_args& a, int stat_tiles, Conv3dRoute* r) {
   if (a.head_out || a.in_split || a.in_f16 || a.out_f16 || (a.in_repeat > 1) || a.out_xblk || a.up_in || a.pool_out ||
-      a.in_pool_flags || a.acc_in)
+      a.in_pool_flags)
     return ROUTE_DECLINED;
   if (a.drop_mode == VX_DROP_MASK || !a.out) return ROUTE_DECLINED;
+  if (a.acc_in && !conv3d_deep_acc(a)) return ROUTE_DECLINED;
   DeepGeo g;
   const int R = deep_pick(a.D, a.H, a.W, &g);
   if (!R) return ROUTE_DECLINED;
diff --git a/values_amd/csrc/convtranspose.hip b/values_amd/csrc/convtranspose.hip
--- a/values_amd/csrc/convtranspose.hip
+++ b/values_amd/csrc/convtranspose.hip
@@ -244,8 +244,141 @@
 }
 
 #include "s16_common.h"
+#include "upcompose32.h"
+
+constexpr int UPC32_PREC_B = 513 * 16;
+constexpr int UPC32_IMG_B = 2 * UPC32_PREC_B;
+constexpr int UPC32_W_B = 8 * 2 * 2 * 2 * 1024;
+constexpr int UPC32_LDS = UPC32_W_B + 2 * UPC32_IMG_B;
+
+__device__ __forceinline__ void convT_upc32_body(const vx_convT_args& a) {
+  extern __shared__ __attribute__((aligned(16))) unsigned char upc_smem[];
+  unsigned char* s_w = upc_smem;
+  unsigned char* s_img = upc_smem + UPC32_W_B;
+  const int tid = threadIdx.x, lane = tid & 63;
+  const int wave = __builtin_amdgcn_readfirstlane(tid >> 6);
+  const int m = lane & 15, g = lane >> 4;
+  const int b = blockIdx.x, S = (int)gridDim.x >> 3;
+  const bool xcd = (S & 7) == 0;
+  const int cls = xcd ? (b >> 3) & 7 : b & 7, slot = xcd ? (b & 7) + 8 * (b >> 6) : b >> 3;
+  const int pz = cls >> 2, py = (cls >> 1) & 1, px = cls & 1;
+  const int nitems = slot < a.N ? (a.N - slot + S - 1) / S : 0;
+  const int total = nitems * 8;
+  if (total == 0) return;
+
+  f32x4 ibuf[2];
+  auto prefetch = [&](int j) {
+    if (j >= total) j = total - 1;
+    const int n = slot + (j >> 3) * S, chunk = j & 7;
+    const float* src = a.in + (size_t)n * 512 * a.in_pitch + chunk * 8;
+#pragma unroll
+    for (int k = 0; k < 2; ++k) {
+      const int p = tid + 512 * k;
+      ibuf[k] = *reinterpret_cast<const f32x4*>(src + (size_t)(p >> 1) * a.in_pitch + (p & 1) * 4);
+    }
+  };
+  auto commit = [&](int buf) {
+    unsigned char* img = s_img + buf * UPC32_IMG_B;
+#pragma unroll
+    for (int k = 0; k < 2; ++k) {
+      const int p = tid + 512 * k;
+      f16x4 hi, lo;
+      vx_split4_s(ibuf[k], hi, lo);
+      *reinterpret_cast<f16x4*>(img + p * 8) = hi;
+      *reinterpret_cast<f16x4*>(img + p * 8 + UPC32_PREC_B) = lo;
+    }
+  };
+  prefetch(0);
+  {
+    const u32x4* wsrc = reinterpret_cast<const u32x4*>(a.up_fused) + (size_t)cls * (UPC32_W_B / 16);
+#pragma unroll
+    for (int i = 0; i < UPC32_W_B / 16 / 512; ++i) reinterpret_cast<u32x4*>(s_w)[tid + 512 * i] = wsrc[tid + 512 * i];
+    if (tid < 4) *reinterpret_cast<u32x4*>(s_img + (tid >> 1) * UPC32_IMG_B + (tid & 1) * UPC32_PREC_B + 512 * 16) = (u32x4){0u, 0u, 0u, 0u};
+  }
+  int boff[4][2], ooff[4], bcls[4];
+#pragma unroll
+  for (int r = 0; r < 4; ++r) {
+    const int v = (wave * 4 + r) * 16 + m;
+    const int X = v & 7, Y = (v >> 3) & 7, Z = v >> 6;
+#pragma unroll
+    for (int s = 0; s < 2; ++s) {
+      const int cz = Z + pz - 1 + s, cy = Y + py - 1 + (g >> 1), cx = X + px - 1 + (g & 1);
+      const bool ok = (unsigned)cz < 8u && (unsigned)cy < 8u && (unsigned)cx < 8u;
+      boff[r][s] = ok ? ((cz * 8 + cy) * 8 + cx) * 16 : 512 * 16;
+    }
+    const int oz = 2 * Z + pz, oy = 2 * Y + py, ox = 2 * X + px;
+    ooff[r] = ((oz * 16 + oy) * 16 + ox) * a.out_pitch + a.out_coff + 4 * g;
+    bcls[r] = (((oz == 0 ? 0 : (oz == 15 ? 2 : 1)) * 3 + (oy == 0 ? 0 : (oy == 15 ? 2 : 1))) * 3 + (ox == 0 ? 0 : (ox == 15 ? 2 : 1))) * 32 + 4 * g;
+  }
+  const float* btab = a.up_fused + VX_UPC32_WHALVES / 2;
+  const size_t out_sample = (size_t)4096 * a.out_pitch;
+  const unsigned char* wlane = s_w + lane * 16;
+  commit(0);
+  prefetch(1);
+  f32x4 acc[4][2], accx[4][2];
+  for (int j = 0; j < total; ++j) {
+    __syncthreads();
+    if (j + 1 < total) commit((j + 1) & 1);
+    prefetch(j + 2);
+    const int chunk = j & 7;
+    if (chunk == 0) {
+      const f32x4 zero = {0.f, 0.f, 0.f, 0.f};
+#pragma unroll
+      for (int r = 0; r < 4; ++r)
+#pragma unroll
+        for (int nt = 0; nt < 2; ++nt) {
+          acc[r][nt] = *reinterpret_cast<const f32x4*>(btab + bcls[r] + 16 * nt);
+          accx[r][nt] = zero;
+        }
+    }
+    const unsigned char* img = s_img + (j & 1) * UPC32_IMG_B;
+#pragma unroll
+    for (int s = 0; s < 2; ++s) {
+      f16x8 wh[2], wl[2], bh[4], bl[4];
+#pragma unroll
+      for (int nt = 0; nt < 2; ++nt) {
+        wh[nt] = *reinterpret_cast<const f16x8*>(wlane + (((chunk * 2 + s) * 2 + nt) * 2) * 1024);
+        wl[nt] = *reinterpret_cast<const f16x8*>(wlane + (((chunk * 2 + s) * 2 + nt) * 2 + 1) * 1024);
+      }
+#pragma unroll
+      for (int r = 0; r < 4; ++r) {
+        bh[r] = *reinterpret_cast<const f16x8*>(img + boff[r][s]);
+        bl[r] = *reinterpret_cast<const f16x8*>(img + boff[r][s] + UPC32_PREC_B);
+      }
+#pragma unroll
+      for (int nt = 0; nt < 2; ++nt) {
+#pragma unroll
+        for (int r = 0; r < 4; ++r) {
+          acc[r][nt] = __builtin_amdgcn_mfma_f32_16x16x32_f16(wh[nt], bh[r], acc[r][nt], 0, 0, 0);
+          accx[r][nt] = __builtin_amdgcn_mfma_f32_16x16x32_f16(wh[nt], bl[r], accx[r][nt], 0, 0, 0);
+        }
+#pragma unroll
+        for (int r = 0; r < 4; ++r) accx[r][nt] = __builtin_amdgcn_mfma_f32_16x16x32_f16(wl[nt], bh[r], accx[r][nt], 0, 0, 0);
+      }
+    }
+    if (chunk == 7) {
+      float* o = a.out + (size_t)(slot + (j >> 3) * S) * out_sample;
+#pragma unroll
+      for (int r = 0; r < 4; ++r)
+#pragma unroll
+        for (int nt = 0; nt < 2; ++nt) {
+          f32x4 v;
+#pragma unroll
+          for (int q = 0; q < 4; ++q) v[q] = fmaf(accx[r][nt][q], 1.0f / 2048.f, acc[r][nt][q]);
+          *reinterpret_cast<f32x4*>(o + ooff[r] + 16 * nt) = v;
+        }
+    }
+  }
+}
+
 template <int CIN, int RT, bool MASK = false>
-__global__ __launch_bounds__(256) void convT_k2s2_s16_kernel(vx_convT_args a, int ncoltiles, int nvox_in, ConvTDecode dc) {
+__global__ __launch_bounds__(CIN == 64 && RT == 4 && !MASK ? 512 : 256) void convT_k2s2_s16_kernel(vx_convT_args a, int ncoltiles, int nvox_in, ConvTDecode dc) {
+  if constexpr (CIN == 64 && RT == 4 && !MASK) {
+    if (a.up_fused) {
+      convT_upc32_body(a);
+      return;
+    }
+  }
   constexpr int Q = CIN / 32;
   const int tid = threadIdx.x, lane = tid & 63, wave = tid >> 6;
   const int m = lane & 15, g = lane >> 4;
@@ -387,6 +520,23 @@
   static const char* kname = vx_kname("convT_k2s2_s16_kernel<%d,%d,false>", CIN, RT);
   static const char* kname_m = vx_kname("convT_k2s2_s16_kernel<%d,%d,true>", CIN, RT);
   vx_note_kernel(a.drop_mode == VX_DROP_MASK ? kname_m : kname);
+  if constexpr (CIN == 64 && RT == 4) {
+    if (a.up_fused) {
+      auto kern = convT_k2s2_s16_kernel<64, 4, false>;
+      static bool attr = false;
+      if (!attr) {
+        hipError_t e = hipFuncSetAttribute(reinterpret_cast<const void*>(kern), hipFuncAttributeMaxDynamicSharedMemorySize, UPC32_LDS);
+        if (e != hipSuccess) VX_FAIL((int)e, "vx_convT_k2s2(composed): hipFuncSetAttribute(%d B LDS): %s", UPC32_LDS, hipGetErrorString(e));
+        attr = true;
+      }
+      int slots = vx_cu_count() / 8;
+      if (slots < 1) slots = 1;
+      if (slots > a.N) slots = a.N;
+      hipLaunchKernelGGL(kern, dim3((unsigned)(8 * slots)), dim3(512), UPC32_LDS, s, a, ncoltiles, (int)nvox, dc);
+      VX_CHECK_LAUNCH("vx_convT_k2s2(composed)");
+      return VX_OK;
+    }
+  }
   if (a.drop_mode == VX_DROP_MASK)
     hipLaunchKernelGGL((convT_k2s2_s16_kernel<CIN, RT, true>), dim3((unsigned)bx, (unsigned)groups), dim3(256), 0, s, a, ncoltiles,
                        (int)nvox, dc);
@@ -451,9 +601,53 @@
   return VX_OK;
 }
 
+__global__ void pack_upfused32_kernel(const float* __restrict__ w1, int w1_cin, const float* __restrict__ uw, const float* __restrict__ ub,
+                                      float* __restrict__ out) {
+  _Float16* oh = reinterpret_cast<_Float16*>(out);
+  constexpr int NWE = VX_UPC32_WHALVES / 2;
+  for (int i = blockIdx.x * blockDim.x + threadIdx.x; i < NWE + 27 * 32; i += gridDim.x * blockDim.x) {
+    if (i < NWE) {
+      const int co = i & 31, ci = (i >> 5) & 63, tap = (i >> 11) & 7, cls = i >> 14;
+      const double v = vx_upc32_weff(w1, w1_cin, uw, cls, tap, ci, co);
+      const _Float16 h = (_Float16)(float)fmin(fmax(v, -65504.0), 65504.0);
+      const _Float16 l = (_Float16)(float)((v - (double)(float)h) * 2048.0);
+      const int at = vx_upc32_index(cls, tap, ci, co);
+      oh[at] = h;
+      oh[at + 512] = l;
+    } else {
+      const int t = i - NWE, co = t & 31, bc = t >> 5;
+      out[NWE + t] = (float)vx_upc32_btab(w1, w1_cin, ub, bc / 9, (bc / 3) % 3, bc % 3, co);
+    }
+  }
+}
+extern "C" int64_t vx_convT_upfused32_packed_floats(void) { return VX_UPC32_FLOATS; }
+extern "C" int vx_pack_convT_upfused32(const float* w1_torch, int w1_cin, const float* up_w_torch, const float* up_b, float* packed,
+                                       vx_stream_t stream) {
+  if (!w1_torch || !up_w_torch || !up_b || !packed) VX_FAIL(VX_E_NULL, "vx_pack_convT_upfused32: null pointer");
+  if (w1_cin < VX_UPC32_CU) VX_FAIL(VX_E_SHAPE, "vx_pack_convT_upfused32: the conv has %d input channels, the up half is its first %d", w1_cin, VX_UPC32_CU);
+  if (!vx_aligned16(packed)) VX_FAIL(VX_E_ALIGN, "vx_pack_convT_upfused32: packed must be 16-byte aligned");
+  hipLaunchKernelGGL(pack_upfused32_kernel, dim3(516), dim3(256), 0, (hipStream_t)stream, w1_torch, w1_cin, up_w_torch, up_b, packed);
+  VX_CHECK_LAUNCH("vx_pack_convT_upfused32");
+  return VX_OK;
+}
+extern "C" int vx_convT_k2s2_upfused_ok(int D, int H, int W, int Cin, int Cout) {
+  return D == 8 && H == 8 && W == 8 && Cin == VX_UPC32_CC && Cout == VX_UPC32_CO && vx_cfg().conv_fp32 == 0 ? 1 : 0;
+}
+
 extern "C" int vx_convT_k2s2(const vx_convT_args* ap, vx_stream_t stream) {
   if (!ap) VX_FAIL(VX_E_NULL, "vx_convT_k2s2: null args");
-  const vx_convT_args& a = *ap;
+  vx_convT_args a = *ap;
+  if (a.up_fused) {
+    if (!vx_convT_k2s2_upfused_ok(a.D, a.H, a.W, a.Cin, a.Cout)) {
+      a.up_fused = nullptr;
+    } else {
+      if (a.act != VX_ACT_NONE || a.drop_mode != VX_DROP_NONE || a.out_xblk)
+        VX_FAIL(VX_E_SHAPE, "vx_convT_k2s2: composed weights (up_fused) go with no activation, no dropout and a dense output");
+      if (!vx_aligned16(a.up_fused) || !vx_aligned16(a.in) || !vx_aligned16(a.out))
+        VX_FAIL(VX_E_ALIGN, "vx_convT_k2s2: up_fused / in / out must be 16-byte aligned");
+      if (a.N <= 0 || a.N >= (1 << 19)) VX_FAIL(VX_E_SHAPE, "vx_convT_k2s2: composed launch takes 1 .. 2^19 - 1 samples");
+    }
+  }
   if (!a.in || !a.w_packed || !a.bias || !a.out) VX_FAIL(VX_E_NULL, "vx_convT_k2s2: null tensor");
   if (a.Cin <= 0 || a.Cout <= 0 || a.Cin % 4 || a.Cout % 8)
     VX_FAIL(VX_E_SHAPE, "vx_convT_k2s2: Cin=%d (mult of 4) Cout=%d (mult of 8)", a.Cin, a.Cout);
diff --git a/values_amd/csrc/lib.cpp b/values_amd/csrc/lib.cpp
--- a/values_amd/csrc/lib.cpp
+++ b/values_amd/csrc/lib.cpp
@@ -82,5 +82,5 @@
 }
 
 extern "C" const char* vx_last_kernel_name(void) { return g_last_kernel ? g_last_kernel : ""; }
-extern "C" int vx_version(void) { return 903;  }
+extern "C" int vx_version(void) { return 904;  }
 extern "C" const char* vx_last_error_string(void) { return g_err; }
diff --git a/values_amd/csrc/unet3d_forward.hip b/values_amd/csrc/unet3d_forward.hip
--- a/values_amd/csrc/unet3d_forward.hip
+++ b/values_amd/csrc/unet3d_forward.hip
@@ -114,6 +114,7 @@
   bool halves[4];
   bool fuse_up;
   bool fuse_up1;
+  bool up_acc2;
   bool split_out[4];
   bool planar1;
   bool st16;
@@ -148,6 +149,17 @@
                 w->split_family == vx_conv3d_k3_family(16, 16) && vx_conv3d_k3_acc_ok(lv[1].D, lv[1].H, lv[1].W, 16, 16);
   f.fuse_up = hashed && F == 8 && vx_conv3d_k3_upfuse_ok(lv[0].D, lv[0].H, lv[0].W, 2 * F, F);
   f.fuse_up1 = f.halves[1] && w->up3_zc16 && hashed && vx_conv3d_k3_upfuse_ok(lv[1].D, lv[1].H, lv[1].W, 16, 16) == 2;
+  if (hashed && f.inorm && !f.skip_raw[2] && cfg.conv_fp32 == 0 && !cfg.s16_no_upfuse && !cfg.s16_no_deep && w->up4_fused && w->split3_w &&
+      lv[2].C == 32 && w->split3_family == vx_conv3d_k3_family(32, 32) &&
+      vx_convT_k2s2_upfused_ok(lv[3].D, lv[3].H, lv[3].W, 64, 32) && vx_conv3d_k3_acc_ok(lv[2].D, lv[2].H, lv[2].W, 32, 32)) {
+    vx_conv3d_args a = {};
+    a.w_packed = w->split3_w; a.bias = w->conv_b[12]; a.w_family = w->split3_family;
+    a.N = r->N; a.D = lv[2].D; a.H = lv[2].H; a.W = lv[2].W; a.Cin = 32; a.Cout = 32;
+    a.in = p.CAT[2] + (size_t)r->N * lv[2].nvox * 32; a.in_pitch = 32; a.out = p.A[2]; a.out_pitch = 32; a.acc_in = p.A[2]; a.acc_pitch = 32;
+    a.act = VX_ACT_LRELU; a.drop_mode = dm; a.out_half = 1;
+    Conv3dRoute rt;
+    f.up_acc2 = conv3d_route(a, cfg, &rt) == VX_OK && rt.kernel == CONV3D_DEEP;
+  }
   f.split_out[1] = f.fuse_up;
   f.split_out[2] = f.fuse_up1;
   f.planar1 = f.fuse_up1 && !cfg.s16_no_l1dma && vx_conv3d_k3_planar_ok(lv[1].D, lv[1].H, lv[1].W, 16, 16);
@@ -220,9 +232,10 @@
     return a;
   };
   auto convT = [&](const float* in, int ui, float* out, int out_pitch, const Level& Lin, int Cin, int Cout, int act,
-                   int drop_layer, bool dense) {
+                   int drop_layer, bool dense, const float* up_fused = nullptr) {
     vx_convT_args a = {};
-    a.range_flag = r->range_flag;
+    a.up_fused = up_fused;
+    a.range_flag = up_fused ? nullptr : r->range_flag;
     a.seed_dev = r->seed_dev;
     a.out_xblk = dense ? 0 : xblk_of(2 * Lin.W); a.out_half = 0;
     a.in = in; a.in_pitch = Cin; a.w_packed = w->up_w[ui]; a.bias = w->up_b[ui];
@@ -337,6 +350,7 @@
     } else {
       vx_norm_args n = norm_args(p.B[l], C, L, 2 * l + 1, true);
       n.out = p.CAT[l]; n.out_pitch = 2 * C; n.out_coff = C; n.out_xblk = xblk_of(L.W); n.pool_out = p.P[l + 1];
+      if (l == 2 && f.up_acc2) { n.out = p.CAT[l] + (size_t)N * L.nvox * C; n.out_pitch = C; n.out_coff = 0; n.out_xblk = 0; }
       if (C <= 512) {
         n.mean = nullptr; n.rstd = nullptr;
         const vx_stat_src st = {p.stats, ntiles, 1e-5f, (int64_t)L.nvox, p.mean, p.rstd};
@@ -381,6 +395,12 @@
       }
       if (f.planar1) { b.out = p.CAT[l]; b.out_planar = 1; }
       VX_STEP(f.fuse_up1 ? "upscale3+expand_2_1(up half)" : "expand_2_1(up half)", vx_conv3d_k3(&b, stream));
+    } else if (l == 2 && f.up_acc2) {
+      vx_conv3d_args a = conv_args(wi, L, C, C, nullptr);
+      a.w_packed = w->split3_w; a.w_family = w->split3_family;
+      a.in = p.CAT[l] + (size_t)N * L.nvox * C; a.in_pitch = C; a.out = p.A[l]; a.out_pitch = C; a.acc_in = p.A[l]; a.acc_pitch = C;
+      set_drop(a, VX_ACT_LRELU, dl);
+      VX_STEP(kConv[wi], vx_conv3d_k3(&a, stream));
     } else {
       vx_conv3d_args a = conv_args(wi, L, 2 * C, C, nullptr);
       a.in = p.CAT[l]; a.in_pitch = 2 * C; a.in_xblk = xblk_of(L.W); a.out = p.A[l]; a.out_pitch = C;
@@ -405,7 +425,9 @@
       a.head_out = r->logits; a.head_w = w->final_w; a.head_b = w->final_b; a.head_C = NC; a.head_dst = r->dst; a.head_flip = r->flip;
     }
     VX_STEP(l == 0 && f.fuse_head ? "expand_1_2+final" : kConv[wi + 1], vx_conv3d_k3(&a, stream));
-    if (l > 0 && !(l == 1 && f.fuse_up) && !(l == 2 && f.fuse_up1))
+    if (l == 3 && f.up_acc2)
+      VX_STEP(kUp[1], convT(p.B[3], 1, p.A[2], C / 2, L, C, C / 2, VX_ACT_NONE, -1, true, w->up4_fused));
+    else if (l > 0 && !(l == 1 && f.fuse_up) && !(l == 2 && f.fuse_up1))
       VX_STEP(kUp[4 - l], convT(p.B[l], 4 - l, p.CAT[l - 1], f.halves[l - 1] ? C / 2 : C, L, C, C / 2, VX_ACT_NONE, -1, f.halves[l - 1]));
   }
   if (!f.fuse_head)
diff --git a/values_amd/csrc/upcompose32.h b/values_amd/csrc/upcompose32.h
--- /dev/null
+++ b/values_amd/csrc/upcompose32.h
@@ -0,0 +1,49 @@
+#pragma once
+#include "upcompose16.h"
+
+#define VX_UPC32_CC 64
+#define VX_UPC32_CU 32
+#define VX_UPC32_CO 32
+
+VX_UPC16_FN double vx_upc32_weff(const float* w1, int w1_cin, const float* uw, int cls, int tap, int ci, int co) {
+  const int pz = cls >> 2, py = (cls >> 1) & 1, px = cls & 1;
+  const int ta = tap >> 2, tb = (tap >> 1) & 1, tc = tap & 1;
+  double acc = 0.0;
+  for (int kz = 0; kz < 3; ++kz) {
+    int a, dz; vx_upc16_tap(pz, kz, &a, &dz);
+    if (a != ta) continue;
+    for (int ky = 0; ky < 3; ++ky) {
+      int b, dy; vx_upc16_tap(py, ky, &b, &dy);
+      if (b != tb) continue;
+      for (int kx = 0; kx < 3; ++kx) {
+        int c, dx; vx_upc16_tap(px, kx, &c, &dx);
+        if (c != tc) continue;
+        for (int cu = 0; cu < VX_UPC32_CU; ++cu)
+          acc += (double)w1[(co * w1_cin + cu) * 27 + kz * 9 + ky * 3 + kx] * (double)uw[(ci * VX_UPC32_CU + cu) * 8 + dz * 4 + dy * 2 + dx];
+      }
+    }
+  }
+  return acc;
+}
+
+VX_UPC16_FN double vx_upc32_btab(const float* w1, int w1_cin, const float* ub, int cz, int cy, int cx, int co) {
+  double acc = 0.0;
+  for (int kz = 0; kz < 3; ++kz) {
+    if ((cz == 0 && kz == 0) || (cz == 2 && kz == 2)) continue;
+    for (int ky = 0; ky < 3; ++ky) {
+      if ((cy == 0 && ky == 0) || (cy == 2 && ky == 2)) continue;
+      for (int kx = 0; kx < 3; ++kx) {
+        if ((cx == 0 && kx == 0) || (cx == 2 && kx == 2)) continue;
+        for (int cu = 0; cu < VX_UPC32_CU; ++cu) acc += (double)w1[(co * w1_cin + cu) * 27 + kz * 9 + ky * 3 + kx] * (double)ub[cu];
+      }
+    }
+  }
+  return acc;
+}
+
+#define VX_UPC32_WHALVES (8 * 8 * 2 * 2 * 2 * 64 * 8)
+#define VX_UPC32_FLOATS (VX_UPC32_WHALVES / 2 + 27 * 32)
+VX_UPC16_FN int vx_upc32_index(int cls, int tap, int ci, int co) {
+  const int chunk = ci >> 3, j = ci & 7, step = tap >> 2, g = tap & 3, nt = co >> 4, m = co & 15;
+  return (((((cls * 8 + chunk) * 2 + step) * 2 + nt) * 2 + 0) * 64 + (g * 16 + m)) * 8 + j;
+}
diff --git a/values_amd/unet3d.py b/values_amd/unet3d.py
--- a/values_amd/unet3d.py
+++ b/values_amd/unet3d.py
@@ -143,6 +143,19 @@
                                                            _lib.ptr(u3f), st), "vx_pack_conv3d_upfused_zc16")
                 keep.append(u3f)
                 w.up3_fused = u3f.data_ptr()
+        if (self.initial_filter_size == 8 and _lib.get_config().conv_fp32 == 0
+                and hasattr(lib, "vx_pack_convT_upfused32")):
+            w3 = sd["expand_3_1.0.weight"]
+            u4f = torch.empty(lib.vx_convT_upfused32_packed_floats(), dtype=torch.float32, device=device)
+            _lib.check(lib.vx_pack_convT_upfused32(_lib.ptr(w3), w3.shape[1], _lib.ptr(sd["upscale4.weight"]), _lib.ptr(sd["upscale4.bias"]),
+                                                   _lib.ptr(u4f), st), "vx_pack_convT_upfused32")
+            skip = w3[:, 32:64].contiguous()
+            pk = torch.empty(lib.vx_conv3d_k3_packed_floats(32, 32), dtype=torch.float32, device=device)
+            _lib.check(lib.vx_pack_conv3d_k3(_lib.ptr(skip), _lib.ptr(pk), 32, 32, st), "vx_pack_conv3d_k3 (expand_3_1 skip half)")
+            keep += [u4f, skip, pk]
+            w.up4_fused = u4f.data_ptr()
+            w.split3_w = pk.data_ptr()
+            w.split3_family = lib.vx_conv3d_k3_family(32, 32)
         fw, fb = self._head_params(sd)
         keep += [fw, fb]
         w.final_w = fw.data_ptr()
```

Result: no change. 3970 volumes/s, median of 6 (+1.0%).
